# sta105/VIORB

Measured on AMD Instinct MI355X. Metric: frames/sec ORB extract+match+pose-opt, EuRoC 752x480, 1/2/4/8 GPUs, higher is better.
Workload: dtype u8

## Files before the change

include/viorb.h:

```cpp
#ifndef VIORB_H
#define VIORB_H

#include <stddef.h>
#include <stdint.h>

#ifdef __cplusplus
extern "C" {
#endif

#define VIORB_OK                 0
#define VIORB_ERR_INVALID_ARG   -1
#define VIORB_ERR_NO_DEVICE     -2
#define VIORB_ERR_HIP           -3
#define VIORB_ERR_CAPACITY      -4
#define VIORB_ERR_UNSUPPORTED   -5

int viorb_abi_version(void);
const char* viorb_last_error(void);
int viorb_device_count(void);


typedef struct viorb_keypoint {
    float x, y;
    float size;
    float angle;
    float response;
    int32_t octave;
    int32_t class_id;
} viorb_keypoint;

typedef struct viorb_extractor_params {
    int32_t nfeatures;
    float   scale_factor;
    int32_t nlevels;
    int32_t ini_th_fast;
    int32_t min_th_fast;
} viorb_extractor_params;

typedef struct viorb_extractor viorb_extractor;

int viorb_extractor_create(const viorb_extractor_params* params, int max_batch, int device,
                           viorb_extractor** out);
int viorb_extractor_destroy(viorb_extractor* h);

int viorb_extractor_tables(const viorb_extractor* h, float* scale, float* inv_scale, float* sigma2,
                           float* inv_sigma2, int32_t* features_per_level);

int viorb_extractor_max_keypoints(const viorb_extractor* h, int* cap);
int viorb_extractor_max_keypoints_for(const viorb_extractor* h, int width, int height, int* cap);
int viorb_extractor_fast_launch_images(int batch);

int viorb_extract(viorb_extractor* h, const uint8_t* img, int width, int height, int stride,
                  viorb_keypoint* kps, uint8_t* desc, int cap, int* n);

int viorb_extract_batch_device(viorb_extractor* h, const uint8_t* d_images, int batch, int width,
                               int height, int stride, size_t image_pitch_bytes, void* stream);

int viorb_extractor_results_device(const viorb_extractor* h, const viorb_keypoint** d_kps,
                                   const uint8_t** d_desc, const int32_t** d_count,
                                   const int32_t** d_status, int* cap);

int viorb_extractor_download(viorb_extractor* h, int b, viorb_keypoint* kps, uint8_t* desc, int cap,
                             int* n);

int viorb_extractor_level_device(const viorb_extractor* h, int b, int level, int blurred,
                                 const uint8_t** d_ptr, int* width, int* height, int* stride);
int viorb_extractor_level_download(viorb_extractor* h, int b, int level, int blurred, uint8_t* dst,
                                   int* width, int* height);

int viorb_stereo_match_device(const viorb_extractor* L, int left_index, const viorb_extractor* R, int right_index, int pairs,
                              float bf, float fx, float* d_uright, float* d_depth, int32_t* d_nmatched, void* stream);
int viorb_stereo_match(viorb_extractor* L, viorb_extractor* R, float bf, float fx, float* uright, float* depth, int cap,
                       int* nmatched);

int viorb_extractor_debug_level_points(viorb_extractor* h, int b, int level, int which, int32_t* xyr,
                                       int cap, int* n);

typedef struct viorb_frontend viorb_frontend;

typedef struct viorb_frontend_config {
    float   min_x, max_x, min_y, max_y;
    float   fx, fy, cx, cy;
    double  cam[16];
    double  gravity[3];
    float   scale_factors[16];
    float   inv_level_sigma2[16];
    int32_t nlevels;
    int32_t check_orientation;
    double  gyr_meas_cov, acc_meas_cov;
    double  acc_bias_rw2;
    float   dist_coef[5];
    int32_t reserved0;
} viorb_frontend_config;

int viorb_frontend_create(const viorb_frontend_config* cfg, int max_batch, int cap, int device, viorb_frontend** out);
int viorb_frontend_search_capacity(void);
int viorb_frontend_destroy(viorb_frontend* h);

int viorb_frontend_undistort_device(viorb_frontend* h, const viorb_keypoint* kps, const int32_t* count, int batch,
                                    viorb_keypoint* kps_un, void* stream);
int viorb_undistort_points(const float* xy, int n, const float* intr4, const float* dist5, float* xy_out);
int viorb_image_bounds(int width, int height, const float* intr4, const float* dist5, float* bounds4);

int viorb_frontend_grid_device(viorb_frontend* h, const viorb_keypoint* kps, const int32_t* count, int batch,
                               int32_t* cell_start, int32_t* cell_idx, void* stream);

int viorb_frontend_imu_predict_device(viorb_frontend* h, const double* imu, int n_imu, const double* t_last,
                                      const double* t_cur, const double* last_ns, int batch, double* preint,
                                      double* cur_ns, float* pose12, void* stream);

int viorb_frontend_search_projection_device(viorb_frontend* h, const viorb_keypoint* cur_kps, const uint8_t* cur_desc,
                                            const int32_t* cur_count, const int32_t* cell_start, const int32_t* cell_idx,
                                            const float* pose12, const viorb_keypoint* last_kps, const int32_t* last_count,
                                            const uint8_t* last_flags, const float* last_Pw, const uint8_t* last_desc,
                                            float th, int batch, int32_t* cur_match, int32_t* nmatches, int32_t* status,
                                            void* stream);
int viorb_frontend_search_projection_retry_device(viorb_frontend* h, const viorb_keypoint* cur_kps, const uint8_t* cur_desc,
                                            const int32_t* cur_count, const int32_t* cell_start, const int32_t* cell_idx,
                                            const float* pose12, const viorb_keypoint* last_kps, const int32_t* last_count,
                                            const uint8_t* last_flags, const float* last_Pw, const uint8_t* last_desc,
                                            float th, int retry_below, int batch, int32_t* cur_match, int32_t* nmatches, int32_t* status,
                                            void* stream);

int viorb_frontend_search_projection_stereo_device(viorb_frontend* h, const viorb_keypoint* cur_kps, const uint8_t* cur_desc,
                                                   const int32_t* cur_count, const float* cur_uright, const int32_t* cell_start,
                                                   const int32_t* cell_idx, const float* pose12, const float* last_pose12,
                                                   const viorb_keypoint* last_kps, const int32_t* last_count, const uint8_t* last_flags,
                                                   const float* last_Pw, const uint8_t* last_desc, float th, float bf, float mb,
                                                   int retry_below, int batch, int32_t* cur_match, int32_t* nmatches, int32_t* status,
                                                   void* stream);

int viorb_frontend_search_local_points_device(viorb_frontend* h, const viorb_keypoint* cur_kps, const uint8_t* cur_desc,
                                              const int32_t* cur_count, const int32_t* cell_start, const int32_t* cell_idx,
                                              const float* pose12, const float* pts_f, const uint8_t* pts_flags,
                                              const uint8_t* pts_desc, const int32_t* pts_count, int pcap, float th,
                                              float nnratio, const uint8_t* cur_owner_obs, int batch, int32_t* match,
                                              int32_t* nmatches, float* frustum, int32_t* status, void* stream);

int viorb_frontend_search_local_points_stereo_device(viorb_frontend* h, const viorb_keypoint* cur_kps, const uint8_t* cur_desc,
                                                     const int32_t* cur_count, const float* cur_uright, float bf, const int32_t* cell_start,
                                                     const int32_t* cell_idx, const float* pose12, const float* pts_f, const uint8_t* pts_flags,
                                                     const uint8_t* pts_desc, const int32_t* pts_count, int pcap, float th, float nnratio,
                                                     const uint8_t* cur_owner_obs, int batch, int32_t* match, int32_t* nmatches, float* frustum,
                                                     float* frustum_xr, int32_t* status, void* stream);

int viorb_frontend_build_observations_device(viorb_frontend* h, const viorb_keypoint* kps, const int32_t* count,
                                             const int32_t* match, const float* match_Pw, int batch, double* obs,
                                             int32_t* obs_index, int32_t* n_obs, void* stream);

int viorb_frontend_pose_opt_device(viorb_frontend* h, int variant, int compute_marg, const double* cur_ns,
                                   const double* last_ns, const double* prior_ns, const double* marg_cov_inv,
                                   const double* preint, const double* obs_cur, const int32_t* n_cur,
                                   const double* obs_last, const int32_t* n_last, int batch, double* out_ns,
                                   double* out_last_ns, uint8_t* outlier_cur, uint8_t* outlier_last, double* marg_out,
                                   double* info, void* stream);

int viorb_frontend_set_pose_shape(int problems_per_workgroup, int wavefronts_per_problem);

int viorb_frontend_pose_opt_se3_device(viorb_frontend* h, const float* pose12, const double* obs7, const int32_t* n_obs,
                                       double bf, int batch, float* out_pose12, uint8_t* outlier, double* info, void* stream);

int viorb_frontend_discard_outliers_device(viorb_frontend* h, int32_t* match, const int32_t* obs_index, const uint8_t* outlier,
                                           const int32_t* n_obs, const uint8_t* pt_flags, int batch, uint8_t* owner_obs,
                                           int32_t* n_map, void* stream);
int viorb_frontend_pose_from_navstate_device(viorb_frontend* h, const double* ns, int batch, float* pose12, void* stream);
int viorb_frontend_build_observations2_device(viorb_frontend* h, const viorb_keypoint* kps, const int32_t* count,
                                              const int32_t* match_a, const float* Pw_a, const int32_t* match_b,
                                              const float* pts_b, int stride_b, int batch, double* obs, int32_t* obs_index,
                                              int32_t* n_obs, void* stream);

int viorb_synth_local_points_device(viorb_frontend* h, const viorb_keypoint* kps, const int32_t* count, const double* pose12,
                                    const float* Pw, int batch, float* pts_f, void* stream);

int viorb_frontend_roll_device(viorb_frontend* h, const viorb_keypoint* cur_kps, const uint8_t* cur_desc, const int32_t* cur_count,
                               viorb_keypoint* last_kps, uint8_t* last_desc, int32_t* last_count, const float* last_pts_f,
                               const uint8_t* last_flags, float* loc_pts_f, uint8_t* loc_desc, uint8_t* loc_flags,
                               int local_frames, int shift_local, const double* ns_src, double* last_ns, double* prior_ns,
                               const double* t_src, double* t_last, const double* marg_src, double* marg_dst, int batch,
                               void* stream);

int viorb_synth_plane_points_device(viorb_frontend* h, const viorb_keypoint* kps, const int32_t* count,
                                    const double* pose12, double z0, int batch, float* Pw, uint8_t* flags,
                                    int32_t* self_index , void* stream);

int viorb_frontend_pose_opt_select_device(viorb_frontend* h, const uint8_t* variant, const uint8_t* skip, int compute_marg,
                                          const double* cur_ns, const double* last_ns, const double* prior_ns, const double* marg_cov_inv,
                                          const double* preint, const double* obs_cur, const int32_t* n_cur, const double* obs_last,
                                          const int32_t* n_last, int batch, double* out_ns, double* out_last_ns, uint8_t* outlier_cur,
                                          uint8_t* outlier_last, double* marg_out, double* info, void* stream);
int viorb_frontend_self_index_device(viorb_frontend* h, const uint8_t* flags, const int32_t* count, int batch, int32_t* self_index,
                                     void* stream);

#define VIORB_TRACK_OK           0
#define VIORB_TRACK_FEW_MATCHES  1
#define VIORB_TRACK_REVERT_1     2
#define VIORB_TRACK_REVERT_2     3
#define VIORB_TRACK_RELOC_FEW    4

typedef struct viorb_tracker viorb_tracker;
typedef struct viorb_tracker_config {
    viorb_extractor_params extractor;
    viorb_frontend_config  frontend;
    int32_t width, height, batch, device;
    float   th_projection;
    int32_t track_local_map;
    int32_t local_frames;
    int32_t compute_marg;
    int32_t max_steps_ahead;
    double  synth_plane_z0;
} viorb_tracker_config;
typedef struct viorb_tracker_inputs {
    const uint8_t* d_images; int32_t image_stride; size_t image_pitch_bytes;
    const double*  d_imu; int32_t n_imu;
    const double*  d_t_cur;
    const uint8_t* d_map_updated;
    const uint8_t* d_recent_reloc;
    const double*  d_t_next_last;
    const double*  d_reset_ns;
    const double*  d_reset_marg;
    const double*  d_synth_pose12;
    const uint8_t* h_images;
} viorb_tracker_inputs;
typedef struct viorb_tracker_results {
    int32_t cap;
    const int32_t *state, *status, *nmatches, *n_map, *n_loc, *inliers, *n_obs, *n_obs2, *cur_match, *loc_match, *last_count;
    const double *info, *info2, *pred_ns, *ns_stage1, *ns_stage2, *final_ns, *final_marg, *last_ns;
    const uint8_t *outlier_cur, *outlier_cur2, *last_flags;
    const float *last_Pw, *last_pts_f;
    const viorb_extractor* extractor;
} viorb_tracker_results;
int viorb_tracker_create(const viorb_tracker_config* cfg, viorb_tracker** out);
int viorb_tracker_destroy(viorb_tracker* h);
int viorb_tracker_capacity(const viorb_tracker* h, int* cap);
int viorb_tracker_bootstrap(viorb_tracker* h, const uint8_t* d_images, int stride, size_t image_pitch_bytes, const double* d_ns0,
                            const double* d_t0, const double* d_marg_cov_inv, const double* d_synth_pose12, void* caller_stream);
int viorb_tracker_set_last_points_device(viorb_tracker* h, const float* d_Pw, const uint8_t* d_flags, const float* d_pts_f, void* caller_stream);
int viorb_tracker_step(viorb_tracker* h, const viorb_tracker_inputs* in, void* caller_stream);
int viorb_tracker_sync(viorb_tracker* h);
int viorb_tracker_results_device(const viorb_tracker* h, viorb_tracker_results* out);
int viorb_tracker_host_stats(viorb_tracker* h, double* enqueue_s, double* throttle_s, long long* steps, int reset);
int viorb_memcpy_dtoh(void* dst_host, const void* src_device, size_t bytes);
int viorb_memcpy_htod(void* dst_device, const void* src_host, size_t bytes);

int viorb_memcpy_dtod_async(void* dst, const void* src, size_t bytes, void* stream);

int viorb_profile_enable(int on);
int viorb_profile_reset(void);
int viorb_profile_select(const char* kernel_name);
int viorb_profile_read(char* names_buf, int names_cap, double* total_ms, int* calls, int cap, int* n);
int viorb_profile_timeline(double* start_ms, double* end_ms, int* slot, int cap, int* n);

int viorb_descriptor_distance(const uint8_t* a, const uint8_t* b);
int viorb_search_by_projection_frame(const viorb_keypoint* cur_kps, const uint8_t* cur_desc, int ncur, const float bounds4[4],
                                     const float pose12[12], const float intr4[4], const float* scale_factors, int nlevels,
                                     const viorb_keypoint* last_kps, int nlast, const uint8_t* last_flags, const float* last_Pw,
                                     const uint8_t* last_desc, float th, int check_orientation, int32_t* cur_match, int* nmatches);
int viorb_search_by_projection_points(const viorb_keypoint* cur_kps, const uint8_t* cur_desc, int ncur, const float bounds4[4],
                                      const float pose12[12], const float intr4[4], const float* scale_factors, int nlevels,
                                      const float* pts_f, const uint8_t* pts_flags, const uint8_t* pts_desc, int npts, float th,
                                      float nnratio, const uint8_t* cur_owner_obs, int32_t* match, int* nmatches, float* frustum5);
int viorb_search_by_projection_points_stereo(const viorb_keypoint* cur_kps, const uint8_t* cur_desc, const float* cur_uright, float bf, int ncur,
                                             const float bounds4[4], const float pose12[12], const float intr4[4], const float* scale_factors, int nlevels,
                                             const float* pts_f, const uint8_t* pts_flags, const uint8_t* pts_desc, int npts, float th, float nnratio,
                                             const uint8_t* cur_owner_obs, int32_t* match, int* nmatches, float* frustum5, float* proj_xr);
int viorb_search_by_projection_frame_stereo(const viorb_keypoint* cur_kps, const uint8_t* cur_desc, const float* cur_uright, int ncur,
                                            const float bounds4[4], const float pose12[12], const float last_pose12[12], const float intr4[4],
                                            float bf, float mb, const float* scale_factors, int nlevels, const viorb_keypoint* last_kps, int nlast,
                                            const uint8_t* last_flags, const float* last_Pw, const uint8_t* last_desc, float th,
                                            int check_orientation, int32_t* cur_match, int* nmatches);
int viorb_preintegrate(const double* imu, int n_imu, const double bg[3], const double ba[3], double t_last,
                       double t_cur, double* preint142);
int viorb_pose_opt_vi(int variant, int compute_marg, const double cur_ns[22], const double last_ns[22],
                      const double prior_ns[22], const double* marg_cov_inv144, const double preint[142],
                      const double gw[3], const double cam[16], const double* obs_cur, int n_cur, const double* obs_last,
                      int n_last, double out_ns[22], double out_last_ns[22], uint8_t* outlier_cur, uint8_t* outlier_last,
                      double* marg_out144, double info[4]);

int viorb_pose_opt_se3(const float pose12[12], const float intr5[5], const double* obs7, int n, float out_pose12[12],
                       uint8_t* outlier, double info[4]);

int viorb_local_ba_set_device(int device);
int viorb_local_ba_navstate(const double* kfs, int nk, int n_local, int prev_kf, const double* preint,
                            const double* points, int np, const int32_t* edge_idx, const double* edge_obs, int ne,
                            const double gw[3], const double cam[16], const volatile int* stop, double* kfs_out,
                            double* points_out, uint8_t* erase, double info[6]);

typedef struct viorb_lba_window {
    const double* kfs; int32_t nk, n_local, prev_kf; const double* preint; const double* points; int32_t np;
    const int32_t* edge_idx; const double* edge_obs; int32_t ne; const double* gw; const double* cam; const volatile int* stop;
    double* kfs_out; double* points_out; uint8_t* erase; double* info ; int32_t status;
} viorb_lba_window;
int viorb_local_ba_navstate_batch(viorb_lba_window* windows, int n_windows, int max_in_flight);

int viorb_local_ba_se3(const double* kfs, int nk, int n_local, const double* points, int np, const int32_t* edge_idx,
                       const double* edge_obs, int ne, const double intr5[5], const volatile int* stop, double* kfs_out,
                       double* points_out, uint8_t* erase, double info[6]);

typedef struct viorb_lba_se3_window {
    const double* kfs; int32_t nk, n_local; const double* points; int32_t np; const int32_t* edge_idx; const double* edge_obs; int32_t ne;
    const double* intr5; const volatile int* stop; double* kfs_out; double* points_out; uint8_t* erase; double* info ; int32_t status;
} viorb_lba_se3_window;
int viorb_local_ba_se3_batch(viorb_lba_se3_window* windows, int n_windows, int max_in_flight);

typedef struct viorb_vocabulary viorb_vocabulary;
int viorb_vocabulary_create(int n_nodes, int L, const int32_t* child_start, const int32_t* child_ids, const uint8_t* desc,
                            const int32_t* word_id, const double* weight, viorb_vocabulary** out);
int viorb_vocabulary_destroy(viorb_vocabulary* v);
typedef struct viorb_vocabulary_flat {
    int32_t n_nodes, k, L, n_words;
    int32_t *child_start, *child_ids, *word_id; uint8_t* desc; double* weight;
} viorb_vocabulary_flat;
int viorb_vocabulary_read_file(const char* path, int binary, viorb_vocabulary_flat* out);
void viorb_vocabulary_flat_free(viorb_vocabulary_flat* f);
int viorb_vocabulary_load_text(const char* path, viorb_vocabulary** out);
int viorb_vocabulary_load_binary(const char* path, viorb_vocabulary** out);
int viorb_vocabulary_save_text(const char* path, int n_nodes, int k, int L, const int32_t* child_start, const int32_t* child_ids,
                               const uint8_t* desc, const double* weight);
int viorb_vocabulary_save_binary(const char* path, int n_nodes, int k, int L, const int32_t* child_start, const int32_t* child_ids,
                                 const uint8_t* desc, const double* weight);

int viorb_bow_transform_device(const viorb_vocabulary* v, const uint8_t* desc, const int32_t* count, int cap, int batch,
                               int levelsup, int32_t* word, double* weight, int32_t* node, void* stream);
int viorb_bow_transform(const viorb_vocabulary* v, const uint8_t* desc, int n, int levelsup, int32_t* word,
                        double* weight, int32_t* node);

int viorb_search_by_bow_device(const viorb_keypoint* kf_kps, const uint8_t* kf_desc, const int32_t* kf_node,
                               const uint8_t* kf_has_point, const int32_t* kf_count, const viorb_keypoint* f_kps,
                               const uint8_t* f_desc, const int32_t* f_node, const int32_t* f_count, int cap, int batch,
                               float nnratio, int check_orientation, int32_t* match, int32_t* nmatches, void* stream);
int viorb_search_by_bow(const viorb_keypoint* kf_kps, const uint8_t* kf_desc, const int32_t* kf_node,
                        const uint8_t* kf_has_point, int nkf, const viorb_keypoint* f_kps, const uint8_t* f_desc,
                        const int32_t* f_node, int nf, float nnratio, int check_orientation, int32_t* match,
                        int* nmatches);

int viorb_match_bruteforce_device(const uint8_t* q_desc, const int32_t* nq, int qcap, const uint8_t* c_desc, const int32_t* nc, int ccap,
                                  int batch, int32_t* best, int32_t* second, int32_t* idx, void* stream);
int viorb_match_bruteforce(const uint8_t* q, int nq, const uint8_t* c, int nc, int32_t* best, int32_t* second, int32_t* idx);

int viorb_search_for_triangulation_device(const viorb_keypoint* k1, const uint8_t* d1, const uint8_t* has_point1,
                                          const float* uright1, const int32_t* node1, const int32_t* n1,
                                          const viorb_keypoint* k2, const uint8_t* d2, const uint8_t* has_point2,
                                          const float* uright2, const int32_t* node2, const int32_t* n2, const float* F12,
                                          const float* Cw1, const float* pose12_2, const float intr4[4],
                                          const float* scale_factors2, const float* level_sigma2_2, int nlevels, int only_stereo,
                                          int check_orientation, int cap, int batch, int32_t* match12, int32_t* nmatches,
                                          void* stream);
int viorb_search_for_triangulation(const viorb_keypoint* k1, const uint8_t* d1, const uint8_t* has_point1, const float* uright1,
                                   const int32_t* node1, int n1, const viorb_keypoint* k2, const uint8_t* d2,
                                   const uint8_t* has_point2, const float* uright2, const int32_t* node2, int n2,
                                   const float F12[9], const float Cw1[3], const float pose12_2[12], const float intr4[4],
                                   const float* scale_factors2, const float* level_sigma2_2, int nlevels, int only_stereo,
                                   int check_orientation, int32_t* match12, int* nmatches);

int viorb_frontend_fuse_device(viorb_frontend* h, const viorb_keypoint* kps, const uint8_t* desc, const float* uright,
                               const int32_t* count, const int32_t* cell_start, const int32_t* cell_idx, const float* pose12,
                               const float* pts_f, const uint8_t* pts_valid, const uint8_t* pts_desc, const int32_t* pts_count,
                               int pcap, float th, float bf, int batch, int32_t* best_idx, int32_t* nfused, void* stream);
int viorb_fuse(const viorb_keypoint* kps, const uint8_t* desc, const float* uright, int n, const float bounds4[4],
               const float pose12[12], const float intr5[5], const float* scale_factors, const float* inv_level_sigma2, int nlevels,
               const float* pts_f, const uint8_t* pts_valid, const uint8_t* pts_desc, int npts, float th, int32_t* best_idx,
               int* nfused);

typedef struct viorb_mapping_camera {
    float   fx, fy, cx, cy;
    float   mb, mbf;
    float   scale_factor;
    int32_t nlevels;
    float   scale_factors[16];
    float   level_sigma2[16];
} viorb_mapping_camera;

#define VIORB_TRI_ACCEPT     0
#define VIORB_TRI_NO_POINT   1
#define VIORB_TRI_BEHIND_1   2
#define VIORB_TRI_BEHIND_2   3
#define VIORB_TRI_REPROJ_1   4
#define VIORB_TRI_REPROJ_2   5
#define VIORB_TRI_SCALE      6
#define VIORB_TRI_NO_PAIR  255
// ... 62 lines not shown
```

viorb_amd/capi.py:

```python
import ctypes as C
import os
import numpy as np

_HERE = os.path.dirname(os.path.abspath(__file__))
SO_PATH = os.environ.get("VIORB_LIBRARY") or os.path.join(_HERE, "libviorb_hip.so")

KP_DTYPE = np.dtype([("x", "f4"), ("y", "f4"), ("size", "f4"), ("angle", "f4"),
                     ("response", "f4"), ("octave", "i4"), ("class_id", "i4")])

VIORB_OK, ERR_INVALID_ARG, ERR_NO_DEVICE, ERR_HIP, ERR_CAPACITY, ERR_UNSUPPORTED = 0, -1, -2, -3, -4, -5


class ViorbError(RuntimeError):
    def __init__(self, code, msg):
        super().__init__("viorb error %d: %s" % (code, msg))
        self.code = code


class FrontendConfig(C.Structure):
    _fields_ = [("min_x", C.c_float), ("max_x", C.c_float), ("min_y", C.c_float), ("max_y", C.c_float),
                ("fx", C.c_float), ("fy", C.c_float), ("cx", C.c_float), ("cy", C.c_float),
                ("cam", C.c_double * 16), ("gravity", C.c_double * 3),
                ("scale_factors", C.c_float * 16), ("inv_level_sigma2", C.c_float * 16),
                ("nlevels", C.c_int32), ("check_orientation", C.c_int32),
                ("gyr_meas_cov", C.c_double), ("acc_meas_cov", C.c_double), ("acc_bias_rw2", C.c_double),
                ("dist_coef", C.c_float * 5), ("reserved0", C.c_int32)]


class LbaWindow(C.Structure):
    _fields_ = [("kfs", C.c_void_p), ("nk", C.c_int32), ("n_local", C.c_int32), ("prev_kf", C.c_int32), ("preint", C.c_void_p),
                ("points", C.c_void_p), ("np", C.c_int32), ("edge_idx", C.c_void_p), ("edge_obs", C.c_void_p), ("ne", C.c_int32),
                ("gw", C.c_void_p), ("cam", C.c_void_p), ("stop", C.c_void_p), ("kfs_out", C.c_void_p), ("points_out", C.c_void_p),
                ("erase", C.c_void_p), ("info", C.c_void_p), ("status", C.c_int32)]


class LbaSe3Window(C.Structure):
    _fields_ = [("kfs", C.c_void_p), ("nk", C.c_int32), ("n_local", C.c_int32), ("points", C.c_void_p), ("np", C.c_int32),
                ("edge_idx", C.c_void_p), ("edge_obs", C.c_void_p), ("ne", C.c_int32), ("intr5", C.c_void_p), ("stop", C.c_void_p),
                ("kfs_out", C.c_void_p), ("points_out", C.c_void_p), ("erase", C.c_void_p), ("info", C.c_void_p), ("status", C.c_int32)]


class ExtractorParams(C.Structure):
    _fields_ = [("nfeatures", C.c_int32), ("scale_factor", C.c_float), ("nlevels", C.c_int32),
                ("ini_th_fast", C.c_int32), ("min_th_fast", C.c_int32)]


class VocabularyFlat(C.Structure):
    _fields_ = [("n_nodes", C.c_int32), ("k", C.c_int32), ("L", C.c_int32), ("n_words", C.c_int32), ("child_start", C.c_void_p),
                ("child_ids", C.c_void_p), ("word_id", C.c_void_p), ("desc", C.c_void_p), ("weight", C.c_void_p)]


class MappingCamera(C.Structure):
    _fields_ = [("fx", C.c_float), ("fy", C.c_float), ("cx", C.c_float), ("cy", C.c_float), ("mb", C.c_float), ("mbf", C.c_float),
                ("scale_factor", C.c_float), ("nlevels", C.c_int32), ("scale_factors", C.c_float * 16), ("level_sigma2", C.c_float * 16)]


class TrackerConfig(C.Structure):
    _fields_ = [("extractor", ExtractorParams), ("frontend", FrontendConfig), ("width", C.c_int32), ("height", C.c_int32), ("batch", C.c_int32),
                ("device", C.c_int32), ("th_projection", C.c_float), ("track_local_map", C.c_int32), ("local_frames", C.c_int32),
                ("compute_marg", C.c_int32), ("max_steps_ahead", C.c_int32), ("synth_plane_z0", C.c_double)]


class TrackerInputs(C.Structure):
    _fields_ = [("d_images", C.c_void_p), ("image_stride", C.c_int32), ("image_pitch_bytes", C.c_size_t), ("d_imu", C.c_void_p), ("n_imu", C.c_int32),
                ("d_t_cur", C.c_void_p), ("d_map_updated", C.c_void_p), ("d_recent_reloc", C.c_void_p), ("d_t_next_last", C.c_void_p),
                ("d_reset_ns", C.c_void_p), ("d_reset_marg", C.c_void_p), ("d_synth_pose12", C.c_void_p), ("h_images", C.c_void_p)]


class TrackerResults(C.Structure):
    _fields_ = [("cap", C.c_int32)] + [(n, C.c_void_p) for n in (
        "state", "status", "nmatches", "n_map", "n_loc", "inliers", "n_obs", "n_obs2", "cur_match", "loc_match", "last_count",
        "info", "info2", "pred_ns", "ns_stage1", "ns_stage2", "final_ns", "final_marg", "last_ns",
        "outlier_cur", "outlier_cur2", "last_flags", "last_Pw", "last_pts_f", "extractor")]


vp, i32, f32, sz = C.c_void_p, C.c_int, C.c_float, C.c_size_t
PP = C.POINTER
SIGNATURES = {
    "viorb_abi_version": (i32, []),
    "viorb_last_error": (C.c_char_p, []),
    "viorb_device_count": (i32, []),
    "viorb_extractor_create": (i32, [PP(ExtractorParams), i32, i32, PP(vp)]),
    "viorb_extractor_destroy": (i32, [vp]),
    "viorb_extractor_tables": (i32, [vp, vp, vp, vp, vp, vp]),
    "viorb_extractor_max_keypoints": (i32, [vp, PP(i32)]),
    "viorb_extractor_max_keypoints_for": (i32, [vp, i32, i32, PP(i32)]),
    "viorb_extractor_fast_launch_images": (i32, [i32]),
    "viorb_extract": (i32, [vp, vp, i32, i32, i32, vp, vp, i32, PP(i32)]),
    "viorb_extract_batch_device": (i32, [vp, vp, i32, i32, i32, i32, sz, vp]),
    "viorb_extractor_results_device": (i32, [vp, PP(vp), PP(vp), PP(vp), PP(vp), PP(i32)]),
    "viorb_extractor_download": (i32, [vp, i32, vp, vp, i32, PP(i32)]),
    "viorb_extractor_level_device": (i32, [vp, i32, i32, i32, PP(vp), PP(i32), PP(i32), PP(i32)]),
    "viorb_extractor_level_download": (i32, [vp, i32, i32, i32, vp, PP(i32), PP(i32)]),
    "viorb_stereo_match_device": (i32, [vp, i32, vp, i32, i32, f32, f32, vp, vp, vp, vp]),
    "viorb_stereo_match": (i32, [vp, vp, f32, f32, vp, vp, i32, PP(i32)]),
    "viorb_extractor_debug_level_points": (i32, [vp, i32, i32, i32, vp, i32, PP(i32)]),
    "viorb_frontend_create": (i32, [PP(FrontendConfig), i32, i32, i32, PP(vp)]),
    "viorb_frontend_search_capacity": (i32, []),
    "viorb_frontend_destroy": (i32, [vp]),
    "viorb_frontend_grid_device": (i32, [vp, vp, vp, i32, vp, vp, vp]),
    "viorb_frontend_undistort_device": (i32, [vp, vp, vp, i32, vp, vp]),
    "viorb_undistort_points": (i32, [vp, i32, vp, vp, vp]),
    "viorb_image_bounds": (i32, [i32, i32, vp, vp, vp]),
    "viorb_frontend_imu_predict_device": (i32, [vp, vp, i32, vp, vp, vp, i32, vp, vp, vp, vp]),
    "viorb_frontend_search_projection_device": (i32, [vp] * 12 + [f32, i32, vp, vp, vp, vp]),
    "viorb_frontend_search_projection_retry_device": (i32, [vp] * 12 + [f32, i32, i32, vp, vp, vp, vp]),
    "viorb_frontend_set_pose_shape": (i32, [i32, i32]),
    "viorb_frontend_search_local_points_device": (i32, [vp] * 11 + [i32, f32, f32, vp, i32, vp, vp, vp, vp, vp]),
    "viorb_frontend_search_local_points_stereo_device": (i32, [vp] * 5 + [f32] + [vp] * 7 + [i32, f32, f32, vp, i32, vp, vp, vp, vp, vp, vp]),
    "viorb_frontend_build_observations_device": (i32, [vp, vp, vp, vp, vp, i32, vp, vp, vp, vp]),
    "viorb_frontend_pose_opt_device": (i32, [vp, i32, i32] + [vp] * 9 + [i32] + [vp] * 7),
    "viorb_frontend_pose_opt_se3_device": (i32, [vp, vp, vp, vp, C.c_double, i32, vp, vp, vp, vp]),
    "viorb_pose_opt_se3": (i32, [vp, vp, vp, i32, vp, vp, vp]),
    "viorb_local_ba_navstate": (i32, [vp, i32, i32, i32, vp, vp, i32, vp, vp, i32] + [vp] * 7),
    "viorb_local_ba_navstate_batch": (i32, [vp, i32, i32]),
    "viorb_local_ba_set_device": (i32, [i32]),
    "viorb_local_ba_se3_batch": (i32, [vp, i32, i32]),
    "viorb_local_ba_se3": (i32, [vp, i32, i32, vp, i32, vp, vp, i32] + [vp] * 6),
    "viorb_vocabulary_create": (i32, [i32, i32, vp, vp, vp, vp, vp, PP(vp)]),
    "viorb_vocabulary_destroy": (i32, [vp]),
    "viorb_vocabulary_read_file": (i32, [C.c_char_p, i32, PP(VocabularyFlat)]),
    "viorb_vocabulary_flat_free": (None, [PP(VocabularyFlat)]),
    "viorb_vocabulary_load_text": (i32, [C.c_char_p, PP(vp)]),
    "viorb_vocabulary_load_binary": (i32, [C.c_char_p, PP(vp)]),
    "viorb_vocabulary_save_text": (i32, [C.c_char_p, i32, i32, i32, vp, vp, vp, vp]),
    "viorb_vocabulary_save_binary": (i32, [C.c_char_p, i32, i32, i32, vp, vp, vp, vp]),
    "viorb_bow_transform_device": (i32, [vp, vp, vp, i32, i32, i32, vp, vp, vp, vp]),
    "viorb_bow_transform": (i32, [vp, vp, i32, i32, vp, vp, vp]),
    "viorb_search_by_bow_device": (i32, [vp] * 9 + [i32, i32, f32, i32, vp, vp, vp]),
    "viorb_search_by_bow": (i32, [vp, vp, vp, vp, i32, vp, vp, vp, i32, f32, i32, vp, PP(i32)]),
    "viorb_match_bruteforce_device": (i32, [vp, vp, i32, vp, vp, i32, i32, vp, vp, vp, vp]),
    "viorb_match_bruteforce": (i32, [vp, i32, vp, i32, vp, vp, vp]),
    "viorb_frontend_discard_outliers_device": (i32, [vp, vp, vp, vp, vp, vp, i32, vp, vp, vp]),
    "viorb_frontend_pose_from_navstate_device": (i32, [vp, vp, i32, vp, vp]),
    "viorb_frontend_build_observations2_device": (i32, [vp, vp, vp, vp, vp, vp, vp, i32, i32, vp, vp, vp, vp]),
    "viorb_synth_local_points_device": (i32, [vp, vp, vp, vp, vp, i32, vp, vp]),
    "viorb_search_for_triangulation_device": (i32, [vp] * 18 + [i32, i32, i32, i32, i32, vp, vp, vp]),
    "viorb_search_for_triangulation": (i32, [vp] * 5 + [i32] + [vp] * 5 + [i32] + [vp] * 6 + [i32, i32, i32, vp, PP(i32)]),
    "viorb_frontend_fuse_device": (i32, [vp] * 12 + [i32, f32, f32, i32, vp, vp, vp]),
    "viorb_fuse": (i32, [vp, vp, vp, i32, vp, vp, vp, vp, vp, i32, vp, vp, vp, i32, f32, vp, PP(i32)]),
    "viorb_synth_plane_points_device": (i32, [vp, vp, vp, vp, C.c_double, i32, vp, vp, vp, vp]),
    "viorb_frontend_roll_device": (i32, [vp] * 12 + [i32, i32] + [vp] * 7 + [i32, vp]),
    "viorb_memcpy_dtod_async": (i32, [vp, vp, sz, vp]),
    "viorb_memcpy_dtoh": (i32, [vp, vp, sz]),
    "viorb_memcpy_htod": (i32, [vp, vp, sz]),
    "viorb_frontend_pose_opt_select_device": (i32, [vp, vp, vp, i32] + [vp] * 9 + [i32] + [vp] * 7),
    "viorb_frontend_self_index_device": (i32, [vp, vp, vp, i32, vp, vp]),
    "viorb_tracker_create": (i32, [PP(TrackerConfig), PP(vp)]),
    "viorb_tracker_destroy": (i32, [vp]),
    "viorb_tracker_capacity": (i32, [vp, PP(i32)]),
    "viorb_tracker_bootstrap": (i32, [vp, vp, i32, sz, vp, vp, vp, vp, vp]),
    "viorb_tracker_set_last_points_device": (i32, [vp, vp, vp, vp, vp]),
    "viorb_tracker_step": (i32, [vp, PP(TrackerInputs), vp]),
    "viorb_tracker_sync": (i32, [vp]),
    "viorb_tracker_results_device": (i32, [vp, PP(TrackerResults)]),
    "viorb_tracker_host_stats": (i32, [vp, PP(C.c_double), PP(C.c_double), PP(C.c_longlong), i32]),
    "viorb_profile_enable": (i32, [i32]),
    "viorb_profile_reset": (i32, []),
    "viorb_profile_select": (i32, [C.c_char_p]),
    "viorb_profile_read": (i32, [C.c_char_p, i32, vp, vp, i32, PP(i32)]),
    "viorb_profile_timeline": (i32, [vp, vp, vp, i32, vp]),
    "viorb_descriptor_distance": (i32, [vp, vp]),
    "viorb_search_by_projection_frame": (i32, [vp, vp, i32, vp, vp, vp, vp, i32, vp, i32, vp, vp, vp, f32, i32, vp, PP(i32)]),
    "viorb_search_by_projection_frame_stereo": (i32, [vp, vp, vp, i32, vp, vp, vp, vp, f32, f32, vp, i32, vp, i32, vp, vp, vp, f32, i32, vp, PP(i32)]),
    "viorb_frontend_search_projection_stereo_device": (i32, [vp] * 14 + [f32, f32, f32, i32, i32, vp, vp, vp, vp]),
    "viorb_search_by_projection_points": (i32, [vp, vp, i32, vp, vp, vp, vp, i32, vp, vp, vp, i32, f32, f32, vp, vp, PP(i32), vp]),
    "viorb_search_by_projection_points_stereo": (i32, [vp, vp, vp, f32, i32, vp, vp, vp, vp, i32, vp, vp, vp, i32, f32, f32, vp, vp, PP(i32), vp, vp]),
    "viorb_preintegrate": (i32, [vp, i32, vp, vp, C.c_double, C.c_double, vp]),
    "viorb_pose_opt_vi": (i32, [i32, i32] + [vp] * 8 + [i32, vp, i32] + [vp] * 6),
    "viorb_debug_pvr_edge": (None, [vp] * 7),
    "viorb_debug_proj_edge": (None, [vp] * 5),
    "viorb_debug_prior_edge": (None, [vp] * 5),
    "viorb_debug_update_ns": (None, [vp] * 6),
    "viorb_debug_preint_step": (None, [vp, vp, vp, C.c_double]),
    "viorb_debug_octree_host": (i32, [vp, i32, i32, i32, i32, vp, i32, PP(i32)]),
    "viorb_debug_fast_atan2": (f32, [f32, f32]),
    "viorb_debug_sincos": (None, [f32, PP(f32), PP(f32)]),
    "viorb_triangulate_pairs_device": (i32, [vp] * 15 + [i32, i32] + [vp] * 4),
    "viorb_triangulate_pairs": (i32, [vp] * 5 + [i32] + [vp] * 6 + [i32] + [vp] * 6),
    "viorb_map_points_update_device": (i32, [vp] * 5 + [i32, vp, vp, i32, vp, vp, C.c_int64] + [vp] * 5),
    "viorb_map_points_update": (i32, [vp] * 5 + [i32, vp, vp, i32, vp, vp, C.c_int64] + [vp] * 4),
    "viorb_create_new_map_points_workspace_bytes": (sz, [i32, i32]),
    "viorb_create_new_map_points_device": (i32, [vp, i32] + [vp] * 24 + [i32] * 6 + [vp] * 6 + [sz, vp]),
    "viorb_create_new_map_points": (i32, [vp, i32] + [vp] * 7 + [i32] + [vp] * 15 + [i32] * 3 + [vp] * 3 + [PP(i32)]),
    "viorb_debug_triangulate_pair": (i32, [vp] * 6 + [i32, vp, i32, vp]),
    "viorb_debug_map_point_update": (i32, [vp] * 5 + [i32, vp, vp, i32, vp, vp, C.c_int64] + [vp] * 4),
}

_lib = None


def lib():
    global _lib
    if _lib is None:
        if not os.path.exists(SO_PATH):
            raise ImportError("%s not built: run `python -c 'import __graft_entry__ as g; g.build()'` "
                              "(hipcc, gfx950). viorb_amd has no CPU fallback." % SO_PATH)
        try:
            import torch
        except Exception:
            pass
        L = C.CDLL(SO_PATH)
        for name, (res, args) in SIGNATURES.items():
            fn = getattr(L, name)
            fn.restype = res
            fn.argtypes = args
        _lib = L
    return _lib


def check(rc):
    if rc != VIORB_OK:
        raise ViorbError(rc, lib().viorb_last_error().decode())
    return rc


def ptr(a):
    if a is None:
        return None
    if isinstance(a, np.ndarray):
        return a.ctypes.data_as(C.c_void_p)
    return C.c_void_p(a.data_ptr())
```

viorb_amd/csrc/orb_extractor.hip:

```cpp
#include <hip/hip_runtime.h>
#include <stdarg.h>
#include <stdlib.h>
#include <math.h>
#include <vector>
#include <string>
#include <mutex>
#include <algorithm>
#include "viorb_common.h"
#include "orb_math.h"
#include "octree_arrays.h"

namespace viorb {

static thread_local char g_err[512] = "";
char* last_error_buf() { return g_err; }
void set_error(const char* fmt, ...) {
    va_list ap; va_start(ap, fmt); vsnprintf(g_err, sizeof(g_err), fmt, ap); va_end(ap);
}

namespace {
struct ProfRec { hipEvent_t a, b; int slot; };
struct Profiler {
    bool enabled = false;
    std::string only;
// ... 543 lines not shown
                    rq = surv[base + lane];
                    const int r = rq >> 8, q = rq & 0xff;
                    const int s = fast_strength(tile + __mul24(r + 3, tile_pitch) + xoff + q + 3, tile_pitch);
                    if (s >= th) { is_c = true; sc[__mul24(r + 1, sp) + q + 1] = (uint8_t)s; }
                }
                const unsigned long long m = __ballot(is_c);
                if (is_c) corn[ncorn + __popcll(m & lt)] = rq;
                ncorn += __popcll(m);
            }
            __syncthreads();
            {
                for (int base = 0; base < ncorn; base += 64) {
                    bool keep = false;
                    int r = 0, q = 0, s = 0;
                    if (base + lane < ncorn) {
                        const uint16_t rq = corn[base + lane];
                        r = rq >> 8; q = rq & 0xff;
                        const uint8_t* z = sc + __mul24(r + 1, sp) + q + 1;
                        s = z[0];
                        int nb[8];
                        nb[0] = z[-sp - 1]; nb[1] = z[-sp]; nb[2] = z[-sp + 1]; nb[3] = z[-1]; nb[4] = z[1]; nb[5] = z[sp - 1]; nb[6] = z[sp]; nb[7] = z[sp + 1];
                        int mx = 0;
    #pragma unroll
                        for (int k = 0; k < 8; k++) mx = max(mx, nb[k]);
                        keep = s > mx;
                    }
                    const unsigned long long m = __ballot(keep);
                    if (keep) {
                        const int pos = total + __popcll(m & lt);
                        if (pos < slot_cap)
                            my_slots[pos] = (uint32_t)(q + 3 + c.shx) | ((uint32_t)(r + 3 + c.shy) << 12) | ((uint32_t)s << 24);
                    }
                    total += __popcll(m);
                }
            }
            __syncthreads();
        }
    }
    if (lane == 0) cell_cnt[(size_t)img_b * ncells_total + cell] = min(total, slot_cap);
    __syncthreads();
    c = cn;
    }
}

#define F3_TPD 13
#define F3_TP (4 * F3_TPD)
#define F3_TRIPS 11
#define F3_SP 44
#define F3_SROWS 40
__device__ __forceinline__ uint32_t pk_mul16(uint32_t a, uint32_t b) {
    return __builtin_bit_cast(uint32_t, __builtin_bit_cast(short2v, a) * __builtin_bit_cast(short2v, b));
}
__device__ __forceinline__ int fast_strength_pol(const uint8_t* p, uint32_t sgn) {
    const uint32_t v = p[0], vv = v | (v << 16);
    uint32_t P[8];
    P[0] = pk_sub16(vv, (uint32_t)p[3 * F3_TP] | ((uint32_t)p[-3 * F3_TP] << 16));
    P[1] = pk_sub16(vv, (uint32_t)p[3 * F3_TP + 1] | ((uint32_t)p[-3 * F3_TP - 1] << 16));
    P[2] = pk_sub16(vv, (uint32_t)p[2 * F3_TP + 2] | ((uint32_t)p[-2 * F3_TP - 2] << 16));
    P[3] = pk_sub16(vv, (uint32_t)p[F3_TP + 3] | ((uint32_t)p[-F3_TP - 3] << 16));
    P[4] = pk_sub16(vv, (uint32_t)p[3] | ((uint32_t)p[-3] << 16));
    P[5] = pk_sub16(vv, (uint32_t)p[-F3_TP + 3] | ((uint32_t)p[F3_TP - 3] << 16));
    P[6] = pk_sub16(vv, (uint32_t)p[-2 * F3_TP + 2] | ((uint32_t)p[2 * F3_TP - 2] << 16));
    P[7] = pk_sub16(vv, (uint32_t)p[-3 * F3_TP + 1] | ((uint32_t)p[3 * F3_TP - 1] << 16));
    uint32_t S[8], lo2[8], lo4[8];
#pragma unroll
    for (int k = 0; k < 8; k++) { P[k] = pk_mul16(P[k], sgn); S[k] = swap16(P[k]); }
#pragma unroll
    for (int k = 0; k < 8; k++) lo2[k] = pk_min16(P[k], k < 7 ? P[k + 1] : S[0]);
#pragma unroll
    for (int k = 0; k < 8; k++) lo4[k] = pk_min16(lo2[k], k < 6 ? lo2[k + 2] : swap16(lo2[k - 6]));
    uint32_t A = 0x80008000u;
#pragma unroll
    for (int k = 0; k < 8; k++) A = pk_max16(A, pk_min16(pk_min16(lo4[k], k < 4 ? lo4[k + 4] : swap16(lo4[k - 4])), S[k]));
    return max((int)(short)(A & 0xffff), (int)(short)(A >> 16)) - 1;
}
__host__ __device__ __forceinline__ uint32_t spread8(uint32_t x) {
    x = (x | (x << 4)) & 0x0f0fu; x = (x | (x << 2)) & 0x3333u; x = (x | (x << 1)) & 0x5555u;
    return x;
}
#define F3_SURV_CAP (63 + 64 * 16 + 1)
#define F3_CORN_CAP 512
#ifdef VIORB_FAST_TIMING
#define FT_DECL unsigned long long ft_acc[8] = {0, 0, 0, 0, 0, 0, 0, 0}, ft_t0 = __builtin_amdgcn_s_memtime(); int ft_cells = 0, ft_surv = 0, ft_corn = 0, ft_att2 = 0
#define FT_LAP(k) do { const unsigned long long ft_now = __builtin_amdgcn_s_memtime(); ft_acc[k] += ft_now - ft_t0; ft_t0 = ft_now; } while (0)
#else
#define FT_DECL
#define FT_LAP(k)
#endif
__global__ __launch_bounds__(64) void k_fast_cells3(const uint8_t* __restrict__ planes, size_t frame_bytes,
                                                    const CellDesc* __restrict__ cells, int ini_th, int min_th,
                                                    uint32_t* __restrict__ slots, int slot_cap,
                                                    int* __restrict__ cell_cnt, int ncells_total, int tile_bytes, int score_bytes, XcdPlace PL) {
    extern __shared__ uint32_t s_mem[];
    int img_b, item;
    if (!xcd_place(PL, img_b, item)) return;
    uint8_t* tile = reinterpret_cast<uint8_t*>(s_mem);
    uint8_t* sc = tile + tile_bytes;
    uint16_t* surv = reinterpret_cast<uint16_t*>(sc + score_bytes);
    uint16_t* corn = surv + F3_SURV_CAP;
    const int lane = threadIdx.x;
    const int cell0 = item * FAST_CELLS_PER_WAVE;
    const int ncell = min((int)FAST_CELLS_PER_WAVE, ncells_total - cell0);
    const uint8_t* img = planes + (size_t)img_b * frame_bytes;
    const int lrow = lane >> 4, lq = lane & 15;
    const bool fetch_lane = lq < F3_TPD;
    uint32_t v[F3_TRIPS];
    auto request_tile = [&](const CellDesc& cd) {
        const uint8_t* src = img + cd.src_off;
        const int ntrip = (cd.ch + 3) >> 2;
        const uint32_t voff = (uint32_t)(__mul24(lrow, cd.stride) + 4 * lq);
        const uint32_t voff_last = (uint32_t)(__mul24(min(4 * (ntrip - 1) + lrow, cd.ch - 1) - 4 * (ntrip - 1), cd.stride) + 4 * lq);
        if (fetch_lane) {
#pragma unroll
            for (int k = 0; k < F3_TRIPS; k++)
                if (k < ntrip) {
                    const uint8_t* base = src + (size_t)(4 * k) * (size_t)cd.stride;
                    v[k] = *reinterpret_cast<const uint32_t*>(base + (k == ntrip - 1 ? voff_last : voff));
                }
        }
    };
    CellDesc c = cells[cell0];
    request_tile(c);
    const int lds_lane = __mul24(lrow, F3_TP) + 4 * lq;
    const unsigned long long lt = (1ull << lane) - 1ull;
    FT_DECL;
    for (int kk = 0; kk < ncell; kk++) {
    FT_LAP(7);
    const int cell = cell0 + kk;
    const int x0a = c.x0 & ~3, xoff = c.x0 - x0a;
    {
        const int ntrip = (c.ch + 3) >> 2;
        if (fetch_lane) {
#pragma unroll
            for (int k = 0; k < F3_TRIPS; k++)
                if (k < ntrip) *reinterpret_cast<uint32_t*>(tile + lds_lane + 4 * k * F3_TP) = v[k];
        }
    }
    const bool has_next = kk + 1 < ncell;
    const CellDesc cn = cells[has_next ? cell + 1 : cell];
    const int dw = c.cw - 6, dh = c.ch - 6;
    {
        const int nq = ((dh + 2) * F3_SP + 15) >> 4;
        for (int i = lane; i < nq; i += 64) reinterpret_cast<uint4*>(sc)[i] = make_uint4(0, 0, 0, 0);
    }
    __syncthreads();
    if (has_next) request_tile(cn);
    FT_LAP(0);
    uint32_t* my_slots = slots + ((size_t)img_b * ncells_total + cell) * slot_cap;
    int total = 0;
    if (dw > 0 && dh > 0) {
        const uint8_t* tile_c = tile + 3 * F3_TP + xoff + 3;
        for (int attempt = 0; attempt < 2 && total == 0; attempt++) {
            const int th = attempt ? min_th : ini_th;
            int pending = 0, ncorn = 0;
            {
                const int g0 = (xoff + 3) >> 2;
                const int G = ((xoff + 3 + dw - 1) >> 2) - g0 + 1;
                const int G2 = (G + 1) >> 1;
                const int rcpG = (int)c_rcp16[min(G2, 63)];
                const int step_r = (64 * rcpG) >> 16, step_g = 64 - step_r * G2;
                int r = __mul24(lane, rcpG) >> 16, gp = lane - __mul24(r, G2);
                const int ntrip = (dh * G2 + 63) >> 6;
                const uint32_t M = 0x00ff00ffu, Hb = 0x80008000u;
                const uint32_t K1 = Hb - (uint32_t)(th + 1) * 0x00010001u;
                const uint32_t K2 = Hb - (uint32_t)(th + 1) * 0x00010001u;
                const int sh0 = (xoff + 3) - 4 * g0;
                const int hi_last = min((G & 1) ? 4 : 8, dw - (8 * (G2 - 1) - sh0));
                const uint32_t m8_first = (0xffu << sh0) & 0xffu, m8_last = (1u << hi_last) - 1u;
                const uint32_t mask_first = spread8(m8_first) * 3u, mask_last = spread8(m8_last) * 3u;
                FT_LAP(1);
#ifdef VIORB_FAST_TIMING
                if (attempt) ft_att2++;
#endif
                for (int trip = 0; trip < ntrip; trip++) {
                    const int rc = min(r, dh - 1);
                    const int ga = 2 * gp, gb = min(ga + 1, G - 1);
                    const uint32_t* rowU = reinterpret_cast<const uint32_t*>(tile + __mul24(rc, F3_TP)) + g0;
                    const uint32_t Lf = rowU[3 * F3_TPD + ga - 1], C0 = rowU[3 * F3_TPD + ga], C1 = rowU[3 * F3_TPD + gb], Rt = rowU[3 * F3_TPD + gb + 1];
                    const uint32_t U0 = rowU[ga], U1 = rowU[gb], D0 = rowU[6 * F3_TPD + ga], D1 = rowU[6 * F3_TPD + gb];
                    const uint32_t Cl1 = gb == ga ? Lf : C0;
                    const uint32_t W0 = __builtin_amdgcn_alignbyte(C0, Lf, 1), E0 = __builtin_amdgcn_alignbyte(gb == ga ? Rt : C1, C0, 3);
                    const uint32_t W1 = __builtin_amdgcn_alignbyte(C1, Cl1, 1), E1 = __builtin_amdgcn_alignbyte(Rt, C1, 3);
                    const int q0 = 4 * (g0 + ga) - (xoff + 3);
                    uint32_t X = 0;
    #pragma unroll
                    for (int dwi = 0; dwi < 2; dwi++) {
                        const uint32_t C = dwi ? C1 : C0, U = dwi ? U1 : U0, D = dwi ? D1 : D0, W = dwi ? W1 : W0, E = dwi ? E1 : E0;
    #pragma unroll
                        for (int half = 0; half < 2; half++) {
                            auto field = [&](uint32_t x) { return half ? __builtin_amdgcn_perm(x, x, 0x0c030c01u) : (x & M); };
                            const uint32_t v2 = field(C);
                            const uint32_t p0 = field(D), p4 = field(E), p8 = field(U), p12 = field(W);
                            const uint32_t A = pk_max16(pk_min16(p0, p8), pk_min16(p4, p12));
                            const uint32_t B = pk_min16(pk_max16(p0, p8), pk_max16(p4, p12));
                            const uint32_t dk = (K1 + v2) - A, br = (K2 - v2) + B;
                            X |= (dk >> (15 - 8 * dwi - 2 * half)) & (0x00010001u << (8 * dwi + 2 * half));
                            X |= (br >> (14 - 8 * dwi - 2 * half)) & (0x00010001u << (8 * dwi + 2 * half + 1));
                        }
                    }
                    uint32_t bits = (X | (X >> 12)) & 0xffffu;
                    bits &= (gp == 0 ? mask_first : 0xffffu) & (gp == G2 - 1 ? mask_last : 0xffffu);
                    if (r >= dh) bits = 0;
                    const int cnt = __popc(bits), incl = wave_inclusive_scan(cnt);
                    const int trip_total = __builtin_amdgcn_readlane(incl, 63);
                    if (trip_total) {
                        int pos = pending + incl - cnt;
                        const uint32_t rq0 = ((uint32_t)r << 7) + (uint32_t)(2 * q0);
                        uint32_t bb = bits;
                        while (bb) {
                            const int k = __builtin_ctz(bb);
                            surv[pos++] = (uint16_t)(rq0 + k);
                            bb &= bb - 1;
                        }
                        pending += trip_total;
                    }
                    r += step_r; gp += step_g;
                    if (gp >= G2) { gp -= G2; r++; }
                    const int need = trip + 1 < ntrip ? 64 : 1;
                    FT_LAP(2);
#ifdef VIORB_FAST_TIMING
                    ft_surv += trip_total;
#endif
                    if (pending >= need) {
                        __syncthreads();
                        int done = 0;
                        while (pending - done >= need) {
                            const int n = min(64, pending - done);
                            bool is_c = false;
                            uint32_t e = 0;
                            if (lane < n) {
                                e = surv[done + lane];
                                const int er = e >> 7, eq = (e >> 1) & 63;
                                const int s = fast_strength_pol(tile_c + __mul24(er, F3_TP) + eq, (e & 1) ? 0xffffffffu : 0x00010001u);
                                if (s >= th) { is_c = true; sc[__mul24(er + 1, F3_SP) + eq + 1] = (uint8_t)s; }
                            }
                            const unsigned long long m = __ballot(is_c);
                            if (is_c) { const int cp = ncorn + __popcll(m & lt); if (cp < F3_CORN_CAP) corn[cp] = (uint16_t)(e & ~1u); }
                            ncorn += __popcll(m);
                            done += n;
                        }
                        const int left = pending - done;
                        if (left > 0) {
                            const uint16_t t = lane < left ? surv[done + lane] : (uint16_t)0;
                            __syncthreads();
                            if (lane < left) surv[lane] = t;
                        }
                        pending = left;
                        __syncthreads();
                        FT_LAP(3);
                    }
                }
            }
            __syncthreads();
            FT_LAP(4);
#ifdef VIORB_FAST_TIMING
            ft_corn += ncorn;
#endif
            const bool dense = ncorn > F3_CORN_CAP;
            const int n3 = dense ? dh * dw : ncorn;
            for (int base = 0; base < n3; base += 64) {
                bool keep = false;
                int r = 0, q = 0, s = 0;
                if (base + lane < n3) {
                    if (dense) { r = (base + lane) / dw; q = (base + lane) - r * dw; }
                    else { const uint32_t e = corn[base + lane]; r = e >> 7; q = (e >> 1) & 63; }
                    const uint8_t* z = sc + __mul24(r + 1, F3_SP) + q + 1;
                    s = z[0];
                    int nb[8];
                    nb[0] = z[-F3_SP - 1]; nb[1] = z[-F3_SP]; nb[2] = z[-F3_SP + 1]; nb[3] = z[-1]; nb[4] = z[1]; nb[5] = z[F3_SP - 1]; nb[6] = z[F3_SP]; nb[7] = z[F3_SP + 1];
                    int mx = 0;
    #pragma unroll
                    for (int k = 0; k < 8; k++) mx = max(mx, nb[k]);
                    keep = s > mx;
                }
                const unsigned long long m = __ballot(keep);
                if (keep) {
                    const int pos = total + __popcll(m & lt);
                    if (pos < slot_cap)
                        my_slots[pos] = (uint32_t)(q + 3 + c.shx) | ((uint32_t)(r + 3 + c.shy) << 12) | ((uint32_t)s << 24);
                }
                total += __popcll(m);
            }
            __syncthreads();
            FT_LAP(5);
        }
    }
    if (lane == 0) cell_cnt[(size_t)img_b * ncells_total + cell] = min(total, slot_cap);
    __syncthreads();
    c = cn;
    FT_LAP(6);
#ifdef VIORB_FAST_TIMING
    ft_cells++;
#endif
    }
#ifdef VIORB_FAST_TIMING
    if (lane == 0 && (blockIdx.x % 997) == 3)
        printf("fast3 block=%d cells=%d att2=%d surv=%d corn=%d | tile+clear=%llu setup=%llu pass1=%llu pass2=%llu tail=%llu nms=%llu end=%llu loop=%llu\n", (int)blockIdx.x, ft_cells, ft_att2, ft_surv, ft_corn,
               ft_acc[0], ft_acc[1], ft_acc[2], ft_acc[3], ft_acc[4], ft_acc[5], ft_acc[6], ft_acc[7]);
#endif
}

#define WAVE_SYNC() __syncthreads()
#define OCT_NCAP_SMALL 4096
struct OctNodeBig { int16_t x0, x1, y0, y1; uint32_t begin, count; uint16_t flags, pad; };
template <bool BIG> struct OctT;
template <> struct OctT<false> { typedef uint16_t Perm; typedef OctNode Node; typedef uint32_t SortKey; enum { KEY_SHIFT = 16 }; };
template <> struct OctT<true> { typedef uint32_t Perm; typedef OctNodeBig Node; typedef unsigned long long SortKey; enum { KEY_SHIFT = 32 }; };
template <bool BIG> struct OctLdsT {
    uint32_t* keys; typename OctT<BIG>::Perm* perm0; typename OctT<BIG>::Perm* perm1; typename OctT<BIG>::Node* nd; typename OctT<BIG>::SortKey* sortb;
};

__device__ __forceinline__ unsigned long long lanemask_lt(int lane) { return (1ull << lane) - 1ull; }

#define OCT_LANE_LIMIT 64
struct OctExpandResult { int off, nexp; };

template <bool BIG> __device__ __forceinline__ void oct_write_children(const OctLdsT<BIG>& S, const typename OctT<BIG>::Node& p, int i, int slot, int mx, int my, int sb,
                                                   const int tc[4], const int sc4[4]) {
#pragma unroll
    for (int c = 0; c < 4; c++) {
        typename OctT<BIG>::Node o;
        o.x0 = (c & 1) ? (int16_t)mx : p.x0; o.x1 = (c & 1) ? p.x1 : (int16_t)mx;
        o.y0 = (c & 2) ? (int16_t)my : p.y0; o.y1 = (c & 2) ? p.y1 : (int16_t)my;
        o.begin = (decltype(o.begin))sc4[c]; o.count = (decltype(o.count))tc[c];
        o.flags = tc[c] > 0 ? (uint16_t)((sb ^ 1) | (tc[c] == 1 ? OCT_NOMORE : 0)) : (uint16_t)OCT_DEAD; o.pad = 0;
        S.nd[slot + c] = o;
    }
    S.nd[i].flags = p.flags | OCT_DEAD;
}

#define OCT_CODE(key) (((int)((key) & 0xfff) < mx ? 0 : 1) | ((int)(((key) >> 12) & 0xfff) < my ? 0 : 2))
template <bool BIG> __device__ __forceinline__ OctExpandResult oct_expand_wave(const OctLdsT<BIG>& S, int i, int slot, int lane) {
    typedef typename OctT<BIG>::Perm Perm;
    const typename OctT<BIG>::Node p = S.nd[i];
    const int mx = p.x0 + ((p.x1 - p.x0 + 1) >> 1), my = p.y0 + ((p.y1 - p.y0 + 1) >> 1);
    const int sb = p.flags & OCT_BUF;
    const Perm* src = (sb ? S.perm1 : S.perm0) + (int)p.begin;
    Perm* dst = sb ? S.perm0 : S.perm1;
    const int cnt = (int)p.count, beg = (int)p.begin;
    const unsigned long long lt = lanemask_lt(lane);
    int t[4] = {0, 0, 0, 0};
    Perm id[4]; int c[4];
    auto load4 = [&](int o) {
#pragma unroll
        for (int u = 0; u < 4; u++) id[u] = src[min(o + 64 * u + lane, cnt - 1)];
#pragma unroll
        for (int u = 0; u < 4; u++) { const uint32_t key = S.keys[id[u]]; c[u] = o + 64 * u + lane < cnt ? OCT_CODE(key) : -1; }
    };
    int w0, w1, w2, w3;
    auto scatter4 = [&]() {
#pragma unroll
        for (int u = 0; u < 4; u++) {
            const unsigned long long m0 = __ballot(c[u] == 0), m1 = __ballot(c[u] == 1), m2 = __ballot(c[u] == 2), m3 = __ballot(c[u] == 3);
            const unsigned long long mm = c[u] == 0 ? m0 : (c[u] == 1 ? m1 : (c[u] == 2 ? m2 : m3));
            int at = w3;
            at = c[u] == 2 ? w2 : at; at = c[u] == 1 ? w1 : at; at = c[u] == 0 ? w0 : at;
            if (c[u] >= 0) dst[at + __popcll(mm & lt)] = id[u];
            w0 += __popcll(m0); w1 += __popcll(m1); w2 += __popcll(m2); w3 += __popcll(m3);
        }
    };
    auto count4 = [&]() {
#pragma unroll
        for (int u = 0; u < 4; u++) {
            t[0] += __popcll(__ballot(c[u] == 0)); t[1] += __popcll(__ballot(c[u] == 1));
            t[2] += __popcll(__ballot(c[u] == 2)); t[3] += __popcll(__ballot(c[u] == 3));
        }
    };
    if (cnt <= 256) {
        load4(0); count4();
        w0 = beg; w1 = w0 + t[0]; w2 = w1 + t[1]; w3 = w2 + t[2];
        scatter4();
    } else {
        for (int o = 0; o < cnt; o += 256) { load4(o); count4(); }
        w0 = beg; w1 = w0 + t[0]; w2 = w1 + t[1]; w3 = w2 + t[2];
        for (int o = 0; o < cnt; o += 256) { load4(o); scatter4(); }
    }
    const int sc4[4] = {beg, beg + t[0], beg + t[0] + t[1], beg + t[0] + t[1] + t[2]};
    if (lane == 0) oct_write_children(S, p, i, slot, mx, my, sb, t, sc4);
    OctExpandResult r; r.off = (t[0] > 0) + (t[1] > 0) + (t[2] > 0) + (t[3] > 0); r.nexp = (t[0] > 1) + (t[1] > 1) + (t[2] > 1) + (t[3] > 1);
    return r;
}

template <bool BIG> __device__ __forceinline__ void oct_lane_count(const OctLdsT<BIG>& S, const typename OctT<BIG>::Node& p, int mx, int my, unsigned long long& lo, unsigned long long& hi, int tc[4]) {
    const typename OctT<BIG>::Perm* src = ((p.flags & OCT_BUF) ? S.perm1 : S.perm0) + (int)p.begin;
    lo = 0; hi = 0; tc[0] = tc[1] = tc[2] = tc[3] = 0;
    const int cnt = (int)p.count;
    for (int k = 0; k < cnt; k += 4) {
        typename OctT<BIG>::Perm id[4]; uint32_t key[4];
#pragma unroll
        for (int u = 0; u < 4; u++) id[u] = src[min(k + u, cnt - 1)];
#pragma unroll
        for (int u = 0; u < 4; u++) key[u] = S.keys[id[u]];
#pragma unroll
        for (int u = 0; u < 4; u++) {
            const bool in = k + u < cnt;
            const int cx = (int)(key[u] & 0xfff) < mx ? 0 : 1, cy = (int)((key[u] >> 12) & 0xfff) < my ? 0 : 1;
            lo |= (unsigned long long)(in ? cx : 0) << ((k + u) & 63); hi |= (unsigned long long)(in ? cy : 0) << ((k + u) & 63);
            const int c = in ? (cx | (cy << 1)) : -1;
            tc[0] += c == 0; tc[1] += c == 1; tc[2] += c == 2; tc[3] += c == 3;
        }
    }
}
template <bool BIG> __device__ __forceinline__ void oct_lane_scatter(const OctLdsT<BIG>& S, const typename OctT<BIG>::Node& p, int i, int slot, int mx, int my, unsigned long long lo,
                                                 unsigned long long hi, const int tc[4]) {
    const int sb = p.flags & OCT_BUF;
    const typename OctT<BIG>::Perm* src = (sb ? S.perm1 : S.perm0) + (int)p.begin;
    typename OctT<BIG>::Perm* dst = sb ? S.perm0 : S.perm1;
    const int sc4[4] = {(int)p.begin, (int)p.begin + tc[0], (int)p.begin + tc[0] + tc[1], (int)p.begin + tc[0] + tc[1] + tc[2]};
    int w0 = sc4[0], w1 = sc4[1], w2 = sc4[2], w3 = sc4[3];
    const int cnt = (int)p.count;
    for (int k = 0; k < cnt; k += 4) {
        typename OctT<BIG>::Perm id[4];
#pragma unroll
        for (int u = 0; u < 4; u++) id[u] = src[min(k + u, cnt - 1)];
#pragma unroll
        for (int u = 0; u < 4; u++) {
            if (k + u < cnt) {
                const int c = (int)((lo >> (k + u)) & 1) | ((int)((hi >> (k + u)) & 1) << 1);
                const int pos = c == 0 ? w0 : (c == 1 ? w1 : (c == 2 ? w2 : w3));
                dst[pos] = id[u];
                w0 += c == 0; w1 += c == 1; w2 += c == 2; w3 += c == 3;
            }
        }
    }
    oct_write_children(S, p, i, slot, mx, my, sb, tc, sc4);
}

template <bool BIG> __device__ __forceinline__ int oct_compact(const OctLdsT<BIG>& S, int nn, int upto, int lane, int& first_new) {
    int w = 0;
    first_new = -1;
    for (int base = 0; base < nn; base += 64) {
        const int i = base + lane;
        typedef typename OctT<BIG>::Node Node;
        enum { NW = sizeof(Node) / 4, FW = offsetof(Node, flags) / 4, FS = 8 * (offsetof(Node, flags) % 4) };
        uint32_t wd[NW];
        const uint32_t* from = reinterpret_cast<const uint32_t*>(S.nd + min(i, nn - 1));
#pragma unroll
        for (int k = 0; k < NW; k++) wd[k] = from[k];
        const bool alive = (i < nn) && !((wd[FW] >> FS) & OCT_DEAD);
        const unsigned long long m = __ballot(alive);
        if (upto >= base && upto < base + 64) first_new = w + __popcll(m & lanemask_lt(upto - base));
        WAVE_SYNC();
        if (alive) {
            uint32_t* to = reinterpret_cast<uint32_t*>(S.nd + w + __popcll(m & lanemask_lt(lane)));
#pragma unroll
            for (int k = 0; k < NW; k++) to[k] = wd[k];
        }
        w += __popcll(m);
        WAVE_SYNC();
    }
    if (first_new < 0) first_new = w;
    return w;
}

template <class K> __device__ __forceinline__ void oct_sort(K* a, int m, int lane) {
    for (int k = 2; k <= m; k <<= 1)
        for (int j = k >> 1; j > 0; j >>= 1) {
            for (int t = lane; t < (m >> 1); t += 64) {
                const int lo = ((t & ~(j - 1)) << 1) | (t & (j - 1));
                const int hi = lo | j;
                const bool up = (lo & k) == 0;
                const K x = a[lo], y = a[hi];
                if ((x > y) == up) { a[lo] = y; a[hi] = x; }
            }
            WAVE_SYNC();
        }
}

template <bool BIG>
__global__ __launch_bounds__(64) void k_octree(const LevelDev* __restrict__ lv, const uint32_t* __restrict__ slots,
                                               int slot_cap, const int* __restrict__ cell_cnt, int ncells_total,
                                               uint32_t* __restrict__ lvl_kp, int kp_pitch, int* __restrict__ lvl_cnt,
                                               int* __restrict__ lvl_ncand, int nlevels, int* __restrict__ status,
                                               int ncap, int nodecap, int sortcap, int n_above, int n_upto,
                                               int level0, int use_tier_cap, int defer_nodes,
                                               uint32_t* __restrict__ big_scratch, int* __restrict__ big_next, int big_slots, int* __restrict__ lvl_tot,
                                               uint8_t* __restrict__ node_scratch = nullptr, size_t node_bytes = 0) {
    extern __shared__ __attribute__((aligned(16))) uint32_t s_oct[];
    typedef typename OctT<BIG>::Perm Perm; typedef typename OctT<BIG>::Node Node; typedef typename OctT<BIG>::SortKey SortKey;
    OctLdsT<BIG> S;
    if (BIG) {
        S.sortb = reinterpret_cast<SortKey*>(s_oct);
        S.nd = reinterpret_cast<Node*>(S.sortb + sortcap);
        S.keys = nullptr; S.perm0 = S.perm1 = nullptr;
    } else {
        S.keys = s_oct;
        S.perm0 = reinterpret_cast<Perm*>(s_oct + ncap);
        S.perm1 = S.perm0 + ncap;
        S.nd = reinterpret_cast<Node*>(S.perm1 + ncap);
        S.sortb = reinterpret_cast<SortKey*>(S.nd + nodecap);
    }
    const int lane = threadIdx.x, level = blockIdx.y + level0, b = blockIdx.x;
    const LevelDev L = lv[level];
    const int N = L.quota;
    if (use_tier_cap && L.oct_tier_cap > 0) n_above = L.oct_tier_cap;
    const int* cc = cell_cnt + (size_t)b * ncells_total + L.cell_base;
    {
        int tot = 0;
        if (n_above < 0) {
            for (int c0 = 0; c0 < L.ncells; c0 += 512) {
                int part[8];
#pragma unroll
                for (int j = 0; j < 8; j++) { const int ci = c0 + 64 * j + lane; part[j] = cc[min(ci, L.ncells - 1)]; if (ci >= L.ncells) part[j] = 0; }
#pragma unroll
                for (int j = 0; j < 8; j++) tot += part[j];
            }
#pragma unroll
            for (int d = 32; d > 0; d >>= 1) tot += __shfl_xor(tot, d);
            if (lane == 0) lvl_tot[b * nlevels + level] = tot;
        } else tot = lvl_tot[b * nlevels + level];
        const bool deferred = (tot & 0x40000000) != 0;
        tot &= 0x3fffffff;
        if (!(deferred && !BIG && !defer_nodes) && (tot <= n_above || tot > n_upto)) return;
        if (BIG) {
            int slot = 0;
            if (lane == 0) slot = atomicAdd(big_next, 1);
            slot = __shfl(slot, 0);
            if (slot >= big_slots) { if (lane == 0) { lvl_cnt[b * nlevels + level] = 0; lvl_ncand[b * nlevels + level] = tot; status[b] = VIORB_ERR_CAPACITY; } return; }
            uint32_t* base = big_scratch + (size_t)slot * 3 * (size_t)ncap;
            S.keys = base; S.perm0 = reinterpret_cast<Perm*>(base + ncap); S.perm1 = reinterpret_cast<Perm*>(base + 2 * (size_t)ncap);
            if (node_scratch) {
                S.sortb = reinterpret_cast<SortKey*>(node_scratch + (size_t)slot * node_bytes);
                S.nd = reinterpret_cast<Node*>(S.sortb + sortcap);
            }
        }
    }
    int n = 0;
    bool overflow = false;
    {
        const uint32_t* sl = slots + ((size_t)b * ncells_total + L.cell_base) * slot_cap;
        for (int base = 0; base < L.ncells; base += 64) {
            const int ci = base + lane;
            const int cnt = ci < L.ncells ? cc[ci] : 0;
            const int incl = wave_inclusive_scan(cnt);
            const int start = n + incl - cnt;
            const uint32_t* mine = sl + (size_t)min(ci, L.ncells - 1) * slot_cap;
            for (int k0 = 0; __any(k0 < cnt); k0 += 8) {
                uint32_t v[8];
#pragma unroll
                for (int u = 0; u < 8; u++) v[u] = mine[min(k0 + u, slot_cap - 1)];
#pragma unroll
                for (int u = 0; u < 8; u++) {
                    const int pos = start + k0 + u;
                    if (k0 + u < cnt && pos < ncap) S.keys[pos] = v[u];
                }
            }
            n += __shfl(incl, 63);
        }
        if (n > ncap) { overflow = true; n = ncap; }
    }
    if (lane == 0) lvl_ncand[b * nlevels + level] = n;
    WAVE_SYNC();
    uint32_t* out = lvl_kp + (size_t)b * kp_pitch + L.kp_off;
    if (n == 0 || L.n_ini < 1 || N < 1) {
        if (lane == 0) { lvl_cnt[b * nlevels + level] = 0; if (overflow) status[b] = VIORB_ERR_CAPACITY; }
        return;
    }
    int nn = 0, live = 0;
    {
        int begin = 0;
        for (int r = 0; r < L.n_ini; r++) {
            int cnt = 0;
            for (int o = 0; o < n; o += 64) {
                const int idx = o + lane;
                bool mine = false;
                if (idx < n) mine = ((int)((float)(S.keys[idx] & 0xfff) / L.hx)) == r;
                const unsigned long long m = __ballot(mine);
                if (mine) S.perm0[begin + cnt + __popcll(m & lanemask_lt(lane))] = (Perm)idx;
                cnt += __popcll(m);
            }
            if (cnt > 0) {
                if (lane == 0) {
                    Node o;
                    o.x0 = (int16_t)(int)(L.hx * (float)r); o.x1 = (int16_t)(int)(L.hx * (float)(r + 1));
                    o.y0 = 0; o.y1 = (int16_t)L.oct_h;
                    o.begin = (decltype(o.begin))begin; o.count = (decltype(o.count))cnt;
                    o.flags = (uint16_t)(cnt == 1 ? OCT_NOMORE : 0); o.pad = 0;
                    S.nd[nn] = o;
                }
                nn++;
            }
            begin += cnt;
        }
        WAVE_SYNC();
        for (int i = lane; i < (nn >> 1); i += 64) {
            const Node a = S.nd[i], z = S.nd[nn - 1 - i];
            S.nd[i] = z; S.nd[nn - 1 - i] = a;
        }
        WAVE_SYNC();
        live = nn;
    }
    bool finish = false;
    int guard = 0;
    while (!finish && guard++ < 64) {
        const int prev = live, nn0 = nn;
        int ne = 0;
        for (int base = 0; base < nn0; base += 64) {
            const int i = nn0 - 1 - (base + lane);
            ne += __popcll(__ballot(i >= 0 && !(S.nd[max(i, 0)].flags & (OCT_NOMORE | OCT_DEAD))));
        }
        if (nn0 + 4 * ne > nodecap) { overflow = true; break; }
        int n_to_expand = 0, e_base = 0;
        for (int base = 0; base < nn0; base += 64) {
            const int i = nn0 - 1 - (base + lane);
            Node p; p.flags = OCT_DEAD; p.count = 0;
            if (i >= 0) p = S.nd[i];
            const bool ex = i >= 0 && !(p.flags & (OCT_NOMORE | OCT_DEAD));
            const unsigned long long m = __ballot(ex);
            const int e = e_base + __popcll(m & lanemask_lt(lane));
            const bool small = ex && p.count <= OCT_LANE_LIMIT;
            int off = 0, nexp = 0;
            if (small) {
                const int mx = p.x0 + ((p.x1 - p.x0 + 1) >> 1), my = p.y0 + ((p.y1 - p.y0 + 1) >> 1);
                unsigned long long lo, hi; int tc[4];
                oct_lane_count(S, p, mx, my, lo, hi, tc);
                oct_lane_scatter(S, p, i, nn0 + 4 * e, mx, my, lo, hi, tc);
                off = (tc[0] > 0) + (tc[1] > 0) + (tc[2] > 0) + (tc[3] > 0); nexp = (tc[0] > 1) + (tc[1] > 1) + (tc[2] > 1) + (tc[3] > 1);
            }
            unsigned long long mb = __ballot(ex && !small);
            int big_off = 0, big_nexp = 0;
            while (mb) {
                const int l = __ffsll((long long)mb) - 1;
                mb &= mb - 1;
                const OctExpandResult r = oct_expand_wave(S, nn0 - 1 - (base + l), nn0 + 4 * __shfl(e, l), lane);
                big_off += r.off - 1; big_nexp += r.nexp;
            }
            int d_live = small ? off - 1 : 0, d_exp = nexp;
#pragma unroll
            for (int d = 32; d > 0; d >>= 1) { d_live += __shfl_xor(d_live, d); d_exp += __shfl_xor(d_exp, d); }
            live += d_live + big_off; n_to_expand += d_exp + big_nexp;
            e_base += __popcll(m);
        }
        nn = nn0 + 4 * ne;
        WAVE_SYNC();
        int first_new;
        nn = oct_compact(S, nn, nn0, lane, first_new);
        if (live >= N || live == prev) {
            finish = true;
        } else if (live + n_to_expand * 3 > N) {
            int guard2 = 0;
            while (!finish && guard2++ < 4096) {
                const int prev2 = live;
                int m = 0;
                for (int base = first_new; base < nn; base += 64) {
                    const int i = base + lane;
                    bool want = false; SortKey key = 0;
                    if (i < nn) { const Node o = S.nd[i]; want = o.count > 1; key = ((SortKey)o.count << OctT<BIG>::KEY_SHIFT) | (SortKey)i; }
                    const unsigned long long bm = __ballot(want);
                    if (want) { const int pos = m + __popcll(bm & lanemask_lt(lane)); if (pos < sortcap) S.sortb[pos] = key; }
                    m += __popcll(bm);
                }
                if (m > sortcap) { overflow = true; m = sortcap; }
                int mp = 1; while (mp < m) mp <<= 1;
                for (int i = m + lane; i < mp; i += 64) S.sortb[i] = 0;
                WAVE_SYNC();
                oct_sort(S.sortb, mp, lane);
                const int nn1 = nn;
                int processed = 0;
                bool reached = false;
                for (int base = 0; base < m && !reached && !finish; base += 64) {
                    const int q = base + lane;
                    const bool valid = q < m;
                    const int i = valid ? (int)(S.sortb[mp - 1 - q] & 0xffff) : 0;
                    Node p; p.flags = OCT_DEAD; p.count = 0;
                    if (valid) p = S.nd[i];
                    if (__any(valid && p.count > OCT_LANE_LIMIT)) {
                        for (int l = 0; l < 64 && base + l < m; l++) {
                            if (nn1 + 4 * (processed + 1) > nodecap) { overflow = true; finish = true; break; }
                            const OctExpandResult r = oct_expand_wave(S, (int)(S.sortb[mp - 1 - (base + l)] & 0xffff), nn1 + 4 * processed, lane);
                            processed++; live += r.off - 1;
                            if (live >= N) { reached = true; break; }
                        }
                        continue;
                    }
                    const int mx = p.x0 + ((p.x1 - p.x0 + 1) >> 1), my = p.y0 + ((p.y1 - p.y0 + 1) >> 1);
                    unsigned long long lo = 0, hi = 0; int tc[4] = {0, 0, 0, 0};
                    if (valid) oct_lane_count(S, p, mx, my, lo, hi, tc);
                    const int inc = valid ? (tc[0] > 0) + (tc[1] > 0) + (tc[2] > 0) + (tc[3] > 0) - 1 : 0;
                    const int incl = wave_inclusive_scan(inc);
                    const unsigned long long mh = __ballot(valid && live + incl >= N);
                    const int nvalid = min(64, m - base);
                    int cut = mh ? __ffsll((long long)mh) - 1 : nvalid - 1;
                    const int fit = (nodecap - nn1) / 4 - processed;
                    if (fit < cut + 1) { overflow = true; finish = true; cut = fit - 1; }
                    if (valid && lane <= cut) oct_lane_scatter(S, p, i, nn1 + 4 * (processed + lane), mx, my, lo, hi, tc);
                    if (cut >= 0) { live += __shfl(incl, cut); processed += cut + 1; }
                    if (mh) reached = true;
                }
                nn = nn1 + 4 * processed;
                WAVE_SYNC();
                nn = oct_compact(S, nn, nn1, lane, first_new);
                if (live >= N || live == prev2) finish = true;
            }
        }
    }
    if (defer_nodes && overflow) {
        if (lane == 0) lvl_tot[b * nlevels + level] |= 0x40000000;
        return;
    }
    for (int base = 0; base < nn; base += 64) {
        const int i = base + lane;
        if (i < nn) {
            const Node o = S.nd[i];
            const Perm* pm = (o.flags & OCT_BUF) ? S.perm1 : S.perm0;
            uint32_t best = S.keys[pm[o.begin]];
            for (int k = 1; k < (int)o.count; k++) {
                const uint32_t key = S.keys[pm[o.begin + k]];
                if ((key >> 24) > (best >> 24)) best = key;
            }
            out[nn - 1 - i] = (best & 0xff000000u) | ((((best >> 12) & 0xfff) + MINB) << 12) | ((best & 0xfff) + MINB);
        }
    }
    if (lane == 0) {
        lvl_cnt[b * nlevels + level] = nn;
        if (overflow) status[b] = VIORB_ERR_CAPACITY;
    }
}

#define BS_LANES 32
#define BS_PF 6
__constant__ int c_gauss[7];
__global__ __launch_bounds__(64) void k_blur(const uint8_t* __restrict__ planes, uint8_t* __restrict__ blur,
                                             size_t frame_bytes, const LevelDev* __restrict__ lv,
                                             const int4* __restrict__ items, XcdPlace PL) {
    int b, item;
    if (!xcd_place(PL, b, item)) return;
    const int4 t = items[item];
    const LevelDev L = lv[t.x];
    const uint8_t* src = planes + (size_t)b * frame_bytes + L.plane_off;
    uint8_t* dst = blur + (size_t)b * frame_bytes + L.plane_off;
    const int lane = threadIdx.x, hl = lane & (BS_LANES - 1);
    const bool upper = lane >= BS_LANES;
    const int Rb = t.w, y0A = t.z, y0B = t.z + Rb;
    const int rows = upper ? min(Rb, L.h - y0B) : min(Rb, L.h - y0A);
    const int sdw = L.stride >> 2;
    const int d = t.y + hl;
    const int dlast = (L.w - 1) >> 2, m = (L.w - 1) & 3;
    const int dc = min(d, sdw - 1);
    const bool end_lane = hl == 0 || hl == BS_LANES - 1;
    const int dn = hl == 0 ? max(dc - 1, 0) : min(dc + 1, sdw - 1);
    const uint32_t selC = m == 0 ? 0x01020304u : m == 1 ? 0x03040504u : m == 2 ? 0x05060504u : 0x07060504u;
    const uint32_t selR = m == 0 ? 0x0c0c0c0cu : m == 1 ? 0x0c000102u : m == 2 ? 0x01020304u : 0x03040506u;
    const bool has_edge = t.y == 0 || t.y + BS_LANES > dlast - 1;
    const bool is_d0 = d == 0, is_dl = d == dlast, is_dl1 = d == dlast - 1;
    const uint32_t k0 = (uint32_t)c_gauss[0], k1 = (uint32_t)c_gauss[1], k2 = (uint32_t)c_gauss[2], k3 = (uint32_t)c_gauss[3];
    const uint32_t Ka = k0 | (k1 << 8) | (k2 << 16) | (k3 << 24), Kb = k2 | (k1 << 8) | (k0 << 16);
    const uint32_t K01 = k0 | (k1 << 16), K23 = k2 | (k3 << 16), K45 = k2 | (k1 << 16);
    const int nrow = Rb + 6;
    const uint8_t* pc = src + 4u * (uint32_t)dc;
    const uint8_t* pn = src + 4u * (uint32_t)(end_lane ? dn : dc);
    uint32_t cb[BS_PF], nb[BS_PF];
    auto request = [&](int i, uint32_t& c, uint32_t& n) {
        const int ii = min(i, nrow - 1);
        int ya = y0A + ii - 3, yb = y0B + ii - 3;
        ya = ya < 0 ? -ya : ya; ya = ya >= L.h ? 2 * L.h - 2 - ya : ya; ya = min(max(ya, 0), L.h - 1);
        yb = yb < 0 ? -yb : yb; yb = yb >= L.h ? 2 * L.h - 2 - yb : yb; yb = min(max(yb, 0), L.h - 1);
        const uint32_t offA = __builtin_amdgcn_readfirstlane(ya * L.stride), offB = __builtin_amdgcn_readfirstlane(yb * L.stride);
        const uint32_t off = upper ? offB : offA;
        c = *reinterpret_cast<const uint32_t*>(pc + off);
        n = *reinterpret_cast<const uint32_t*>(pn + off);
    };
#pragma unroll
    for (int u = 0; u < BS_PF; u++) request(u, cb[u], nb[u]);
    uint32_t P[6][4], hp[4] = {0, 0, 0, 0};
#pragma unroll
    for (int u = 0; u < 6; u++) { P[u][0] = P[u][1] = P[u][2] = P[u][3] = 0; }
    uint8_t* pd = dst + 4u * (uint32_t)min(d, sdw - 1);
    const bool col_ok = d < sdw;
    for (int i0 = 0; i0 < nrow; i0 += 6) {
#pragma unroll
        for (int u = 0; u < 6; u++) {
            const int i = i0 + u;
            uint32_t c = cb[u];
            uint32_t Lr = __builtin_amdgcn_update_dpp(c, c, 0x138, 0xf, 0xf, true);
            uint32_t Rr = __builtin_amdgcn_update_dpp(c, c, 0x130, 0xf, 0xf, true);
            Lr = hl == 0 ? nb[u] : Lr; Rr = hl == BS_LANES - 1 ? nb[u] : Rr;
            request(i + BS_PF, cb[u], nb[u]);
            if (has_edge) {
                const uint32_t Lf = __builtin_amdgcn_perm(Rr, c, 0x01020304u);
                const uint32_t Cf = __builtin_amdgcn_perm(c, Lr, selC), Rf = __builtin_amdgcn_perm(c, Lr, selR);
                const uint32_t Rf1 = __builtin_amdgcn_perm(Rr, c, selC);
                Lr = is_d0 ? Lf : Lr;
                Rr = is_dl ? Rf : (is_dl1 ? Rf1 : Rr);
                c = is_dl ? Cf : c;
            }
            uint32_t h[4];
            h[0] = __builtin_amdgcn_udot4(__builtin_amdgcn_alignbyte(c, Lr, 1), Ka, __builtin_amdgcn_udot4(__builtin_amdgcn_alignbyte(Rr, c, 1), Kb, 0u, false), false);
            h[1] = __builtin_amdgcn_udot4(__builtin_amdgcn_alignbyte(c, Lr, 2), Ka, __builtin_amdgcn_udot4(__builtin_amdgcn_alignbyte(Rr, c, 2), Kb, 0u, false), false);
            h[2] = __builtin_amdgcn_udot4(__builtin_amdgcn_alignbyte(c, Lr, 3), Ka, __builtin_amdgcn_udot4(__builtin_amdgcn_alignbyte(Rr, c, 3), Kb, 0u, false), false);
            h[3] = __builtin_amdgcn_udot4(c, Ka, __builtin_amdgcn_udot4(Rr, Kb, 0u, false), false);
            uint32_t a[4];
#pragma unroll
            for (int j = 0; j < 4; j++) {
                a[j] = dot2_u16(P[(u + 1) % 6][j], K01, 1u << 15);
                a[j] = dot2_u16(P[(u + 3) % 6][j], K23, a[j]);
                a[j] = dot2_u16(P[(u + 5) % 6][j], K45, a[j]);
                a[j] = __umul24(h[j], k0) + a[j];
                a[j] = min(a[j], 0x00ffffffu);
                P[u][j] = hp[j] | (h[j] << 16);
                hp[j] = h[j];
            }
            const int o = i - 6;
            const uint32_t yoA = __builtin_amdgcn_readfirstlane((y0A + o) * L.stride), yoB = __builtin_amdgcn_readfirstlane((y0B + o) * L.stride);
            if (o >= 0 && o < rows && col_ok) {
                const uint32_t lo = __builtin_amdgcn_perm(a[1], a[0], 0x0c0c0602u), hi = __builtin_amdgcn_perm(a[3], a[2], 0x0c0c0602u);
                *reinterpret_cast<uint32_t*>(pd + (upper ? yoB : yoA)) = lo | (hi << 16);
            }
        }
    }
}

__constant__ __attribute__((aligned(16))) uint32_t c_pattern[256];
__constant__ int c_umax[16];
__constant__ uint32_t c_orient_mask[256];
typedef uint32_t u32_unaligned __attribute__((aligned(1)));
#define DESC_WIN_HALF 18
#define DESC_WIN_ROWS 37
#define DESC_WIN_DW 10
#define DESC_WIN_TRIPS 6
__global__ __launch_bounds__(256) void k_orient_describe(const uint8_t* __restrict__ planes,
                                                         const uint8_t* __restrict__ blur, size_t frame_bytes,
                                                         const LevelDev* __restrict__ lv, int nlevels,
                                                         const uint32_t* __restrict__ lvl_kp, int kp_pitch,
                                                         const int* __restrict__ lvl_cnt,
                                                         viorb_keypoint* __restrict__ out_kp,
                                                         uint8_t* __restrict__ out_desc, int out_cap,
                                                         int* __restrict__ out_cnt, int* __restrict__ status, XcdPlace PL) {
    const int lane = threadIdx.x & 63;
    int b, item;
    if (!xcd_place(PL, b, item)) return;
    const int k = item * 4 + __builtin_amdgcn_readfirstlane(threadIdx.x >> 6);
    const int* cnt = lvl_cnt + b * nlevels;
    int level = -1, local = 0, total = 0;
    for (int l = 0; l < nlevels; l++) {
        const int c = cnt[l];
        if (level < 0 && k < total + c) { level = l; local = k - total; }
        total += c;
    }
    if (k == 0 && lane == 0) { out_cnt[b] = min(total, out_cap); if (total > out_cap) status[b] = VIORB_ERR_CAPACITY; }
    if (level < 0 || k >= out_cap) return;
    const LevelDev L = lv[level];
    const uint32_t key = lvl_kp[(size_t)b * kp_pitch + L.kp_off + local];
    const int cx = (int)(key & 0xfff), cy = (int)((key >> 12) & 0xfff), score = (int)(key >> 24);
    const uint8_t* img = planes + (size_t)b * frame_bytes + L.plane_off + (size_t)cy * L.stride + cx;
    __shared__ uint32_t s_win[4][DESC_WIN_ROWS * DESC_WIN_DW];
    uint32_t* win = s_win[threadIdx.x >> 6];
    const uint8_t* bim = blur + (size_t)b * frame_bytes + L.plane_off + (size_t)cy * L.stride + cx;
    uint32_t wv[DESC_WIN_TRIPS];
#pragma unroll
    for (int it = 0; it < DESC_WIN_TRIPS; it++) {
        const int i = min(lane + 64 * it, DESC_WIN_ROWS * DESC_WIN_DW - 1);
        const int wr = i / DESC_WIN_DW, wc = i - wr * DESC_WIN_DW;
        wv[it] = *reinterpret_cast<const u32_unaligned*>(bim + __mul24(wr - DESC_WIN_HALF, L.stride) - DESC_WIN_HALF + 4 * wc);
    }
    int m10 = 0, m01 = 0;
    {
        const int j = lane & 7, r8 = lane >> 3;
        const uint32_t wu = 0x03020100u + 0x04040404u * (uint32_t)j;
        const uint8_t* col = img - HALF_PATCH + 4 * j;
        uint32_t px[4]; int vv[4];
#pragma unroll
        for (int it = 0; it < 4; it++) {
            const int row = min(it * 8 + r8, PATCH - 1);
            vv[it] = row - HALF_PATCH;
            px[it] = *reinterpret_cast<const u32_unaligned*>(col + __mul24(vv[it], L.stride));
        }
#pragma unroll
        for (int it = 0; it < 4; it++) {
            const uint32_t q = px[it] & c_orient_mask[it * 64 + lane];
            const int s1 = (int)__builtin_amdgcn_udot4(q, 0x01010101u, 0u, false);
            const int su = (int)__builtin_amdgcn_udot4(q, wu, 0u, false);
            m10 += su - __mul24(HALF_PATCH, s1);
            m01 += __mul24(vv[it], s1);
        }
    }
    m10 = __builtin_amdgcn_readlane(wave_inclusive_scan(m10), 63); m01 = __builtin_amdgcn_readlane(wave_inclusive_scan(m01), 63);
    const float angle = fast_atan2_deg((float)m01, (float)m10);
    const float factor_pi = (float)(3.14159265358979323846 / 180.f);
    float sn, cs;
    sincos_f32(angle * factor_pi, &sn, &cs);
    const float a = cs, bb = sn;
#pragma unroll
    for (int it = 0; it < DESC_WIN_TRIPS; it++) {
        const int i = lane + 64 * it;
        if (i < DESC_WIN_ROWS * DESC_WIN_DW) win[i] = wv[it];
    }
    __builtin_amdgcn_fence(__ATOMIC_RELEASE, "wavefront"); __builtin_amdgcn_wave_barrier(); __builtin_amdgcn_fence(__ATOMIC_ACQUIRE, "wavefront");
    const uint8_t* w8 = reinterpret_cast<const uint8_t*>(win) + DESC_WIN_HALF * (DESC_WIN_DW * 4) + DESC_WIN_HALF;
    uint32_t nib = 0;
    const uint4 pq = reinterpret_cast<const uint4*>(c_pattern)[lane];
    const uint32_t pqa[4] = {pq.x, pq.y, pq.z, pq.w};
#pragma unroll
    for (int t = 0; t < 4; t++) {
        const uint32_t q = pqa[t];
        const float x0 = (float)(int8_t)(q & 0xff), y0 = (float)(int8_t)((q >> 8) & 0xff);
        const float x1 = (float)(int8_t)((q >> 16) & 0xff), y1 = (float)(int8_t)(q >> 24);
        const int r0 = round_half_even(x0 * bb + y0 * a), c0 = round_half_even(x0 * a - y0 * bb);
        const int r1 = round_half_even(x1 * bb + y1 * a), c1 = round_half_even(x1 * a - y1 * bb);
        const int t0 = w8[__mul24(r0, DESC_WIN_DW * 4) + c0], t1 = w8[__mul24(r1, DESC_WIN_DW * 4) + c1];
        nib |= (uint32_t)(t0 < t1) << t;
    }
    uint32_t byte = nib | (__shfl_down(nib, 1) << 4);
    uint32_t word = byte | (__shfl_down(byte, 2) << 8) | (__shfl_down(byte, 4) << 16) | (__shfl_down(byte, 6) << 24);
    const size_t o = (size_t)b * out_cap + k;
    if ((lane & 7) == 0) reinterpret_cast<uint32_t*>(out_desc + o * 32)[lane >> 3] = word;
    if (lane == 0) {
        viorb_keypoint kp;
        kp.x = level ? (float)cx * L.scale : (float)cx;
        kp.y = level ? (float)cy * L.scale : (float)cy;
        kp.size = L.kp_size; kp.angle = angle; kp.response = (float)score;
        kp.octave = level; kp.class_id = -1;
        out_kp[o] = kp;
    }
}

struct StereoArgs {
    const viorb_keypoint *kl, *kr; const uint8_t *dl, *dr; const int *nl, *nr;
    const uint8_t *planesL, *planesR; size_t frame_bytes; const LevelDev* lv;
    int cap, sort_n, nlevels; float bf, fx;
    float scale[16], inv_scale[16];
    float* uright; float* depth; int* nmatched;
    unsigned char* work; size_t work_bytes;
};
__host__ __device__ inline size_t stereo_lds_bytes(int cap, int sort_n) { return (size_t)sort_n * (8 + 4 + 4 + 4) + (size_t)cap * 4 + 64; }

template <bool GW>
__global__ __launch_bounds__(1024) void k_stereo_match(StereoArgs A) {
    extern __shared__ __attribute__((aligned(16))) unsigned char s_st_lds[];
    unsigned char* s_st = GW ? A.work + (size_t)blockIdx.x * A.work_bytes : s_st_lds;
    const int p = blockIdx.x, t = threadIdx.x, cap = A.cap, sn = A.sort_n;
    unsigned long long* keys = reinterpret_cast<unsigned long long*>(s_st);
    float* ry = reinterpret_cast<float*>(keys + sn);
    int* rid = reinterpret_cast<int*>(ry + sn);
    uint32_t* skeys = reinterpret_cast<uint32_t*>(rid + sn);
    int* sad = reinterpret_cast<int*>(skeys + sn);
    __shared__ int s_cnt, s_removed;
    const int N = min(A.nl[p], cap), Nr = min(A.nr[p], cap);
    const viorb_keypoint* kl = A.kl + (size_t)p * cap; const viorb_keypoint* kr = A.kr + (size_t)p * cap;
    const uint8_t* dl = A.dl + (size_t)p * cap * 32; const uint8_t* dr = A.dr + (size_t)p * cap * 32;
    float* uR = A.uright + (size_t)p * cap; float* dep = A.depth + (size_t)p * cap;
    for (int i = t; i < sn; i += blockDim.x)
        keys[i] = i < Nr ? (((unsigned long long)__float_as_uint(kr[i].y) << 32) | (unsigned)i) : ~0ull;
    if (t == 0) { s_cnt = 0; s_removed = 0; }
    __syncthreads();
    for (int k = 2; k <= sn; k <<= 1)
        for (int j = k >> 1; j > 0; j >>= 1) {
            for (int q = t; q < (sn >> 1); q += blockDim.x) {
                const int lo = ((q & ~(j - 1)) << 1) | (q & (j - 1)), hi = lo | j;
                const bool up = (lo & k) == 0;
                const unsigned long long x = keys[lo], y = keys[hi];
                if ((x > y) == up) { keys[lo] = y; keys[hi] = x; }
            }
            __syncthreads();
        }
    for (int i = t; i < sn; i += blockDim.x) { ry[i] = i < Nr ? __uint_as_float((unsigned)(keys[i] >> 32)) : 3.0e38f; rid[i] = (int)(keys[i] & 0xffffffffu); }
    __syncthreads();
    const float mb = A.bf / A.fx, minD = 0.f, maxD = A.bf / mb;
    const float rmax = 2.0f * A.scale[A.nlevels - 1];
    const int nRows = A.lv[0].h;
    const int thOrbDist = (100 + 50) / 2;
    for (int iL = t; iL < cap; iL += blockDim.x) {
        float out_u = -1.f, out_d = -1.f; int out_sad = -1;
        if (iL < N) {
            const viorb_keypoint kpL = kl[iL];
            const int levelL = kpL.octave; const float vL = kpL.y, uL = kpL.x;
            const int rowi = (int)vL;
            const float minU = uL - maxD, maxU = uL - minD;
            if (rowi >= 0 && rowi < nRows && !(maxU < 0)) {
                const float ylo = (float)rowi - rmax - 1.0f, yhi = (float)rowi + rmax + 1.0f;
                int lo = 0, hi = Nr;
                while (lo < hi) { const int mid = (lo + hi) >> 1; if (ry[mid] < ylo) lo = mid + 1; else hi = mid; }
                const uint4* pl = reinterpret_cast<const uint4*>(dl + (size_t)iL * 32);
                const uint4 da = pl[0], db = pl[1];
                uint32_t best = 0xffffffffu;
                for (int k = lo; k < Nr && ry[k] <= yhi; k++) {
                    const int iR = rid[k];
                    const viorb_keypoint kpR = kr[iR];
                    const float r = 2.0f * A.scale[kpR.octave];
                    const int maxr = (int)ceilf(kpR.y + r), minr = (int)floorf(kpR.y - r);
                    if (rowi < minr || rowi > maxr) continue;
                    if (kpR.octave < levelL - 1 || kpR.octave > levelL + 1) continue;
                    if (!(kpR.x >= minU && kpR.x <= maxU)) continue;
                    const uint4* pr = reinterpret_cast<const uint4*>(dr + (size_t)iR * 32);
                    const uint4 ea = pr[0], eb = pr[1];
                    const int dist = __popc(da.x ^ ea.x) + __popc(da.y ^ ea.y) + __popc(da.z ^ ea.z) + __popc(da.w ^ ea.w) +
                                     __popc(db.x ^ eb.x) + __popc(db.y ^ eb.y) + __popc(db.z ^ eb.z) + __popc(db.w ^ eb.w);
                    if (dist < 100) best = min(best, ((uint32_t)dist << 16) | (uint32_t)iR);
                }
                if (best != 0xffffffffu && (int)(best >> 16) < thOrbDist) {
                    const int bestIdxR = (int)(best & 0xffff);
                    const float uR0 = kr[bestIdxR].x;
                    const float sfac = A.inv_scale[levelL];
                    const int cu = (int)roundf(kpL.x * sfac), cv = (int)roundf(kpL.y * sfac), cr = (int)roundf(uR0 * sfac);
                    const LevelDev Lv = A.lv[levelL];
                    const int w = 5, L = 5;
                    const float iniu = (float)cr + L - w, endu = (float)cr + L + w + 1;
                    const bool inside = !(iniu < 0 || endu >= Lv.w) && cv - w >= 0 && cv + w < Lv.h && cu - w >= 0 && cu + w < Lv.w &&
                                        cr - L - w >= 0 && cr + L + w < Lv.w;
                    if (inside) {
                        const uint8_t* IL = A.planesL + (size_t)p * A.frame_bytes + Lv.plane_off;
                        const uint8_t* IR = A.planesR + (size_t)p * A.frame_bytes + Lv.plane_off;
                        const int cL = IL[(size_t)cv * Lv.stride + cu];
                        int cRv[11], acc[11];
#pragma unroll
                        for (int sft = 0; sft < 11; sft++) { cRv[sft] = IR[(size_t)cv * Lv.stride + cr + sft - L]; acc[sft] = 0; }
                        for (int dy = -w; dy <= w; dy++) {
                            const uint8_t* rl = IL + (size_t)(cv + dy) * Lv.stride + cu - w;
                            const uint8_t* rr = IR + (size_t)(cv + dy) * Lv.stride + cr - L - w;
                            int lrow[11], rrow[21];
#pragma unroll
                            for (int x = 0; x < 11; x++) lrow[x] = (int)rl[x] - cL;
#pragma unroll
                            for (int x = 0; x < 21; x++) rrow[x] = rr[x];
#pragma unroll
                            for (int sft = 0; sft < 11; sft++)
#pragma unroll
                                for (int x = 0; x < 11; x++) acc[sft] += abs(lrow[x] - (rrow[sft + x] - cRv[sft]));
                        }
                        int bestSad = 0x7fffffff, bestinc = 0;
#pragma unroll
                        for (int sft = 0; sft < 11; sft++) if (acc[sft] < bestSad) { bestSad = acc[sft]; bestinc = sft - L; }
                        if (!(bestinc == -L || bestinc == L)) {
                            float d1 = 0, d2 = 0, d3 = 0;
#pragma unroll
                            for (int sft = 1; sft < 10; sft++) if (sft - L == bestinc) { d1 = (float)acc[sft - 1]; d2 = (float)acc[sft]; d3 = (float)acc[sft + 1]; }
                            const float deltaR = (d1 - d3) / (2.0f * (d1 + d3 - 2.0f * d2));
                            if (!(deltaR < -1 || deltaR > 1)) {
                                float bestuR = A.scale[levelL] * ((float)cr + (float)bestinc + deltaR);
                                float disparity = uL - bestuR;
                                if (disparity >= minD && disparity < maxD) {
                                    if (disparity <= 0) { disparity = 0.01f; bestuR = (float)((double)uL - 0.01); }
                                    out_d = A.bf / disparity; out_u = bestuR; out_sad = bestSad;
                                }
                            }
                        }
                    }
                }
            }
        }
        uR[iL] = out_u; dep[iL] = out_d; sad[iL] = out_sad;
    }
    __syncthreads();
    for (int i = t; i < sn; i += blockDim.x) skeys[i] = (i < cap && sad[i] >= 0) ? (((uint32_t)sad[i] << 16) | (uint32_t)i) : 0xffffffffu;
    for (int i = t; i < cap; i += blockDim.x) if (sad[i] >= 0) atomicAdd(&s_cnt, 1);
    __syncthreads();
    for (int k = 2; k <= sn; k <<= 1)
        for (int j = k >> 1; j > 0; j >>= 1) {
            for (int q = t; q < (sn >> 1); q += blockDim.x) {
                const int lo = ((q & ~(j - 1)) << 1) | (q & (j - 1)), hi = lo | j;
                const bool up = (lo & k) == 0;
                const uint32_t x = skeys[lo], y = skeys[hi];
                if ((x > y) == up) { skeys[lo] = y; skeys[hi] = x; }
            }
            __syncthreads();
        }
    const int cnt = s_cnt;
    if (cnt > 0) {
        const float median = (float)(skeys[cnt / 2] >> 16);
        const float thDist = 1.5f * 1.4f * median;
        for (int i = t; i < cnt; i += blockDim.x) {
            const uint32_t e = skeys[i];
            if (!((float)(e >> 16) < thDist)) { const int iL = (int)(e & 0xffff); uR[iL] = -1.f; dep[iL] = -1.f; atomicAdd(&s_removed, 1); }
        }
    }
    __syncthreads();
    if (t == 0) A.nmatched[p] = cnt - s_removed;
}

}

using namespace viorb;

struct viorb_extractor {
    viorb_extractor_params p;
    int max_batch = 1, device = 0;
    std::vector<float> scale, inv_scale, sigma2, inv_sigma2;
    std::vector<int> quota;
    int umax[16];
    int img_w = 0, img_h = 0;
    std::vector<LevelDev> lv;
    std::vector<CellDesc> cells;
    std::vector<int4> blur_tiles;
    size_t frame_bytes = 0;
    int slot_cap = 0, kp_pitch = 0, out_cap = 0;
    int fast_tile_pitch = 0, fast_tile_rows = 0, fast_tile_bytes = 0, fast_score_bytes = 0, fast_list_cap = 0;
    bool fast_v3 = false;
    int fast3_tile_bytes = 0, fast3_score_bytes = 0;
    int oct_ncap = 0, oct_nodecap = 0, oct_sortcap = 0;
    std::vector<std::pair<int, int>> oct_tiers;
    int oct_first_cap = 0, oct_node_x10 = 50;
    int oct_big_cap = 0, oct_big_slots = 0; uint32_t* d_oct_big = nullptr; int* d_oct_big_next = nullptr; int* d_lvl_tot = nullptr;
    unsigned char* d_stereo_work = nullptr; size_t stereo_work_bytes = 0;
    bool oct_huge = false; uint8_t* d_oct_nodes = nullptr; size_t oct_node_bytes = 0;
    std::vector<int> rs_pitch_dw, rs_rows;
    std::vector<int4> rs2_tiles; std::vector<int> rs2_off, rs2_pitch_dw, rs2_ok; bool rs2_copy_ok = false;
    int4* d_rs2_tiles = nullptr;
    std::vector<int4> rss_items; std::vector<uint2> rss_etab; std::vector<int> rss_item_off, rss_etab_off, rss_ok;
    int4* d_rss_items = nullptr; uint2* d_rss_etab = nullptr;
    uint8_t *d_planes = nullptr, *d_blur = nullptr, *d_desc = nullptr, *d_stage = nullptr;
    LevelDev* d_lv = nullptr; CellDesc* d_cells = nullptr; int4* d_blur_tiles = nullptr;
    int2 *d_xtab = nullptr, *d_ytab = nullptr;
    uint32_t *d_slots = nullptr, *d_lvl_kp = nullptr;
    int *d_cell_cnt = nullptr, *d_lvl_cnt = nullptr, *d_lvl_ncand = nullptr, *d_count = nullptr, *d_status = nullptr;
    viorb_keypoint* d_kps = nullptr;
    size_t stage_bytes = 0;
    hipStream_t own_stream = nullptr;
    hipStream_t aux_stream = nullptr; hipEvent_t ev_fork = nullptr, ev_join = nullptr;
    hipStream_t last_stream = nullptr;
    int last_batch = 0;
    unsigned fast_prof_rot = 0;
    bool tables_uploaded = false;
};

static void free_device(viorb_extractor* h) {
    void* ptrs[] = {h->d_planes, h->d_blur, h->d_desc, h->d_stage, h->d_lv, h->d_cells, h->d_blur_tiles, h->d_xtab,
                    h->d_ytab, h->d_slots, h->d_lvl_kp, h->d_cell_cnt, h->d_lvl_cnt, h->d_lvl_ncand, h->d_count,
                    h->d_status, h->d_kps, h->d_rs2_tiles, h->d_rss_items, h->d_rss_etab, h->d_oct_big, h->d_oct_big_next, h->d_lvl_tot, h->d_oct_nodes};
    for (void* p : ptrs) if (p) (void)hipFree(p);
    h->d_rs2_tiles = nullptr; h->d_rss_items = nullptr; h->d_rss_etab = nullptr; h->d_oct_big = nullptr; h->d_oct_big_next = nullptr; h->d_lvl_tot = nullptr; h->d_oct_nodes = nullptr;
    h->d_planes = h->d_blur = h->d_desc = h->d_stage = nullptr; h->d_lv = nullptr; h->d_cells = nullptr;
    h->d_blur_tiles = nullptr; h->d_xtab = h->d_ytab = nullptr; h->d_slots = h->d_lvl_kp = nullptr;
    h->d_cell_cnt = h->d_lvl_cnt = h->d_lvl_ncand = h->d_count = h->d_status = nullptr; h->d_kps = nullptr;
    h->stage_bytes = 0;
}

static int max_keypoints_for_size(const viorb_extractor* h, int w, int hgt) {
    int cap = 0;
    for (int l = 0; l < h->p.nlevels; l++) {
        const float s = h->inv_scale[l];
        const int lw = host_cv_round((double)((float)w * s)), lh = host_cv_round((double)((float)hgt * s));
        const int ow = lw - 2 * MINB, oh = lh - 2 * MINB;
        const int n_ini = (oh > 0 && ow > 0) ? (int)roundf((float)ow / (float)oh) : 0;
        cap += std::max(h->quota[l] + 2, 4 * n_ini);
    }
    return cap;
}

static int configure(viorb_extractor* h, int w, int hgt) {
    const int nl = h->p.nlevels;
    free_device(h);
    h->lv.assign(nl, LevelDev());
    h->cells.clear(); h->blur_tiles.clear();
    std::vector<int2> xtab, ytab;
    h->rs_pitch_dw.assign(nl, 0); h->rs_rows.assign(nl, 0);
    h->rs2_tiles.clear(); h->rs2_off.assign(nl, 0); h->rs2_pitch_dw.assign(nl, 1); h->rs2_ok.assign(nl, 0); h->rs2_copy_ok = false;
    h->rss_items.clear(); h->rss_etab.clear(); h->rss_item_off.assign(nl + 1, 0); h->rss_etab_off.assign(nl, 0); h->rss_ok.assign(nl, 0);
    size_t off = 0;
    int kp_off = 0, max_cw = 0, max_ch = 0;
    for (int l = 0; l < nl; l++) {
        LevelDev& L = h->lv[l];
        const float s = h->inv_scale[l];
        L.w = host_cv_round((double)((float)w * s));
        L.h = host_cv_round((double)((float)hgt * s));
        if (L.w < 1 || L.h < 1 || L.w > 4095 || L.h > 4095) { set_error("level %d size %dx%d unsupported", l, L.w, L.h); return VIORB_ERR_UNSUPPORTED; }
        L.stride = (int)align_up(L.w, 64);
        L.plane_off = (uint32_t)off;
        off += align_up((size_t)L.stride * L.h, 256);
        L.quota = h->quota[l];
        L.scale = h->scale[l];
        L.kp_size = (float)(int)(PATCH * h->scale[l]);
        const int maxBX = L.w - MINB, maxBY = L.h - MINB;
        const float width = (float)(maxBX - MINB), height = (float)(maxBY - MINB);
        L.oct_w = maxBX - MINB; L.oct_h = maxBY - MINB;
        L.cell_base = (int)h->cells.size();
        const int nCols = (int)(width / 30.f), nRows = (int)(height / 30.f);
        if (nCols >= 1 && nRows >= 1) {
            const int wCell = (int)ceilf(width / nCols), hCell = (int)ceilf(height / nRows);
            for (int i = 0; i < nRows; i++) {
                const float iniY = (float)(MINB + i * hCell);
                float maxY = iniY + hCell + 6;
                if (iniY >= maxBY - 3) continue;
                if (maxY > maxBY) maxY = (float)maxBY;
                for (int j = 0; j < nCols; j++) {
                    const float iniX = (float)(MINB + j * wCell);
                    float maxX = iniX + wCell + 6;
                    if (iniX >= maxBX - 6) continue;
                    if (maxX > maxBX) maxX = (float)maxBX;
                    CellDesc c;
                    c.level = l; c.x0 = (int)iniX; c.y0 = (int)iniY;
                    c.cw = (int)maxX - (int)iniX; c.ch = (int)maxY - (int)iniY;
                    c.shx = j * wCell; c.shy = i * hCell; c.pitch = (int)align_up(c.cw + 3, 4) + 4;
                    c.src_off = (uint32_t)(L.plane_off + (size_t)c.y0 * L.stride + (size_t)(c.x0 & ~3)); c.stride = L.stride;
                    if (c.cw < 7 || c.ch < 7) continue;
                    h->cells.push_back(c);
                    max_cw = std::max(max_cw, (int)c.cw); max_ch = std::max(max_ch, (int)c.ch);
                }
            }
        }
        L.ncells = (int)h->cells.size() - L.cell_base;
        L.n_ini = (L.oct_h > 0 && L.oct_w > 0) ? (int)roundf((float)L.oct_w / (float)L.oct_h) : 0;
        L.hx = L.n_ini > 0 ? (float)L.oct_w / (float)L.n_ini : 1.f;
        L.kp_off = kp_off;
        kp_off += std::max(L.quota, 4 * L.n_ini) + 4;
        L.xtab_off = (int)xtab.size(); L.ytab_off = (int)ytab.size();
        if (l > 0) {
            const int sw = h->lv[l - 1].w, sh = h->lv[l - 1].h;
            const double inv_sx = (double)L.w / sw, inv_sy = (double)L.h / sh;
            const double scale_x = 1. / inv_sx, scale_y = 1. / inv_sy;
            for (int dx = 0; dx < L.w; dx++) {
                float fx = (float)((dx + 0.5) * scale_x - 0.5);
                int sx = host_cv_floor(fx);
                fx -= sx;
                if (sx < 0) { fx = 0; sx = 0; }
                if (sx + 1 >= sw && sx >= sw - 1) { fx = 0; sx = sw - 1; }
                const int a0 = clampi(host_cv_round((double)((1.f - fx) * 2048)), -32768, 32767);
                const int a1 = clampi(host_cv_round((double)(fx * 2048)), -32768, 32767);
                const int sx1 = std::min(sx + 1, sw - 1);
                xtab.push_back(make_int2(sx | (sx1 << 16), (a0 & 0xffff) | (a1 << 16)));
            }
            for (int dy = 0; dy < L.h; dy++) {
                float fy = (float)((dy + 0.5) * scale_y - 0.5);
                int sy = host_cv_floor(fy);
                fy -= sy;
                const int b0 = clampi(host_cv_round((double)((1.f - fy) * 2048)), -32768, 32767);
                const int b1 = clampi(host_cv_round((double)(fy * 2048)), -32768, 32767);
                const int sy0 = clampi(sy, 0, sh - 1), sy1 = clampi(sy + 1, 0, sh - 1);
                ytab.push_back(make_int2(sy0 | (sy1 << 16), (b0 & 0xffff) | (b1 << 16)));
            }
            int maxdw = 1, maxrows = 1;
            const int2* xt = xtab.data() + L.xtab_off; const int2* yt = ytab.data() + L.ytab_off;
            for (int tx = 0; tx < L.w; tx += RS_TW) {
                const int x1 = std::min(tx + RS_TW, L.w) - 1;
                const int xs0 = (xt[tx].x & 0xffff) & ~3, xs1 = xt[x1].x >> 16;
                maxdw = std::max(maxdw, ((xs1 - xs0) >> 2) + 1);
            }
            for (int ty = 0; ty < L.h; ty += RS_TH) {
                const int y1 = std::min(ty + RS_TH, L.h) - 1;
                maxrows = std::max(maxrows, (yt[y1].x >> 16) - (yt[ty].x & 0xffff) + 1);
            }
            h->rs_pitch_dw[l] = maxdw; h->rs_rows[l] = maxrows;
            if ((size_t)maxdw * maxrows * 4 > 60000) { set_error("resize tile does not fit LDS (scale factor too large)"); return VIORB_ERR_UNSUPPORTED; }
            {
                h->rs2_off[l] = (int)h->rs2_tiles.size();
                int pdw = 1, prow = 1; bool cover = true; int next_x = 0, next_y = 0;
                const int gx2 = (L.w + RS2_TW - 1) / RS2_TW, gy2 = (L.h + RS2_TH - 1) / RS2_TH;
                for (int ty = 0; ty < gy2; ty++) {
                    const int y0t = ty * RS2_TH, y1t = std::min(y0t + RS2_TH, L.h) - 1;
                    const int ys0 = yt[y0t].x & 0xffff, ys1 = yt[y1t].x >> 16;
                    if (ys0 > next_y) cover = false;
                    next_y = std::max(next_y, ys1 + 1);
                    next_x = 0;
                    for (int tx = 0; tx < gx2; tx++) {
                        const int x0t = tx * RS2_TW, x1t = std::min(x0t + RS2_TW, L.w) - 1;
                        const int xs0 = (xt[x0t].x & 0xffff) & ~3, xs1 = xt[x1t].x >> 16;
                        if (xs0 > next_x) cover = false;
                        next_x = std::max(next_x, (xs1 | 3) + 1);
                        const int ndw = ((xs1 - xs0) >> 2) + 1, nrows = ys1 - ys0 + 1;
                        pdw = std::max(pdw, ndw); prow = std::max(prow, nrows);
                        h->rs2_tiles.push_back(make_int4(xs0, ndw, ys0, nrows));
                    }
                    if (next_x < sw) cover = false;
                }
                if (next_y < sh) cover = false;
                h->rs2_pitch_dw[l] = pdw;
                h->rs2_ok[l] = (prow <= 48 && pdw * prow <= 256 * RS2_TRIPS) ? 1 : 0;
                if (l == 1) h->rs2_copy_ok = cover && h->rs2_ok[1];
            }
            {
                static const bool no_stream = getenv("VIORB_RESIZE_TILES") != nullptr;
                bool ok = !no_stream && sw >= 8;
                h->rss_etab_off[l] = (int)h->rss_etab.size();
                std::vector<uint2> et(sh, make_uint2(0x7fffu, 0u));
                for (int dy = 0; dy < L.h && ok; dy++) {
                    const int sy0 = yt[dy].x & 0xffff, sy1 = yt[dy].x >> 16;
                    if ((sy1 != sy0 && sy1 != sy0 + 1) || et[sy1].x != 0x7fffu || dy >= 0x7fff) { ok = false; break; }
                    const int b0 = yt[dy].y & 0xffff, b1 = (yt[dy].y >> 16) & 0xffff;
                    if (b0 > 2048 || b1 > 2048) { ok = false; break; }
                    et[sy1] = make_uint2((uint32_t)dy | (sy1 == sy0 ? 0x8000u : 0u), (uint32_t)b0 | ((uint32_t)b1 << 16));
                }
                const int ndw = (L.w + 3) / 4;
                for (int dcol = 0; dcol < ndw && ok; dcol++) {
                    const int first = xt[std::min(4 * dcol, L.w - 1)].x & 0xffff;
                    for (int j = 0; j < 4; j++) {
                        const int2 e = xt[std::min(4 * dcol + j, L.w - 1)];
                        if ((e.x >> 16) - first > 7 || (e.x & 0xffff) < first || (e.y & 0xffff) > 2048 || ((e.y >> 16) & 0xffff) > 2048) ok = false;
                    }
                }
                h->rss_item_off[l] = (int)h->rss_items.size();
                if (ok) {
                    const double sy = (double)sh / L.h;
                    const int rbmax = std::max(1, std::min(100, (int)((RSS_MAX_SRC_ROWS - 2) / sy)));
                    const int nb = 2 * ((L.h + 2 * rbmax - 1) / (2 * rbmax)), rb = (L.h + nb - 1) / nb;
                    for (int k = 0; k < nb && ok; k++) {
                        const int ya = k * rb, yb = std::min(ya + rb, L.h) - 1;
                        if (ya <= yb && (yt[yb].x >> 16) - (yt[ya].x & 0xffff) + 1 > RSS_MAX_SRC_ROWS) ok = false;
                    }
                    for (int sx = 0; sx < ndw && ok; sx += RSS_LANES)
                        for (int k = 0; k < nb; k += 2)
                            if (k * rb < L.h) h->rss_items.push_back(make_int4(sx, k * rb, rb, 0));
                }
                if (!ok) h->rss_items.resize(h->rss_item_off[l]);
                h->rss_ok[l] = ok ? 1 : 0;
                h->rss_etab.insert(h->rss_etab.end(), et.begin(), et.end());
            }
        }
        {
            const int nb = 2 * ((L.h + 127) / 128), rb = (L.h + nb - 1) / nb, ndw = (L.w + 3) / 4;
            for (int sx = 0; sx < ndw; sx += BS_LANES)
                for (int k = 0; k < nb; k += 2) h->blur_tiles.push_back(make_int4(l, sx, k * rb, rb));
            if (L.w < 12 || L.h < 4) { set_error("level %d (%dx%d) too small for the blur", l, L.w, L.h); return VIORB_ERR_UNSUPPORTED; }
        }
    }
    h->frame_bytes = align_up(off, 256);
    h->kp_pitch = kp_off;
    h->out_cap = max_keypoints_for_size(h, w, hgt);
    const int ncells = (int)h->cells.size();
    if (ncells == 0) { set_error("image %dx%d too small for a FAST cell grid", w, hgt); return VIORB_ERR_UNSUPPORTED; }
    h->fast_tile_pitch = (int)align_up(max_cw + 3, 4) + 4;
    h->fast_tile_rows = max_ch;
    {
        int tb = 64 * FAST_FETCH_TRIPS * 4;
        for (const CellDesc& c : h->cells) tb = std::max(tb, c.pitch * c.ch);
        h->fast_tile_bytes = (int)align_up((size_t)tb, 16);
    }
    h->fast_score_bytes = (int)align_up((size_t)(max_cw - 6 + 2) * (max_ch - 6 + 2), 4);
    h->slot_cap = ((max_cw - 6 + 1) / 2) * ((max_ch - 6 + 1) / 2);
    h->fast_list_cap = (int)align_up((size_t)(max_cw - 6) * (max_ch - 6), 2);
    if (max_cw - 6 > 255 || max_ch - 6 > 255) { set_error("FAST cell larger than 255 px"); return VIORB_ERR_UNSUPPORTED; }
    {
        bool ok = true;
        for (const CellDesc& c : h->cells) ok = ok && ((c.x0 & 3) + c.cw <= 4 * F3_TPD - 4) && c.ch <= 4 * F3_TRIPS && c.cw - 6 + 2 <= F3_SP && c.ch - 6 + 2 <= F3_SROWS;
        static const bool force_v2 = getenv("VIORB_FAST_V2") != nullptr;
        h->fast_v3 = ok && !force_v2;
        h->fast3_tile_bytes = (int)align_up((size_t)(4 * ((max_ch + 3) / 4)) * F3_TP, 16);
        h->fast3_score_bytes = (int)align_up((size_t)(max_ch - 6 + 2) * F3_SP + 16, 16);
    }
    int maxq = 1; for (int l = 0; l < nl; l++) maxq = std::max(maxq, h->quota[l]);
    h->oct_ncap = 8192;
    h->oct_nodecap = 5 * maxq + 64;
    int sc = 1; while (sc < maxq + 8) sc <<= 1;
    h->oct_sortcap = sc;
    size_t oct_lds = (size_t)h->oct_ncap * 8 + (size_t)h->oct_nodecap * sizeof(OctNode) + (size_t)sc * 4;
    if (h->oct_nodecap > 65535) { set_error("per-level quota %d too large for the quadtree's 16-bit node indices", maxq); return VIORB_ERR_UNSUPPORTED; }
    h->oct_huge = oct_lds > 160 * 1024;
    if (!h->oct_huge && oct_lds > 64 * 1024 &&
        raise_dynamic_lds(reinterpret_cast<const void*>(k_octree<false>), oct_lds) != hipSuccess) {
        (void)hipGetLastError();
        h->oct_ncap = 4096;
        oct_lds = (size_t)h->oct_ncap * 8 + (size_t)h->oct_nodecap * sizeof(OctNode) + (size_t)sc * 4;
        if (oct_lds > 64 * 1024) { set_error("quadtree LDS (%zu B) exceeds the dynamic-LDS limit", oct_lds); return VIORB_ERR_UNSUPPORTED; }
    }

    if (!h->oct_huge) {
        const size_t lds_big = (size_t)h->oct_sortcap * 8 + (size_t)h->oct_nodecap * sizeof(OctNodeBig);
        if (lds_big > 160 * 1024) h->oct_huge = true;
        else if (lds_big > 64 * 1024) VIORB_HIP_TRY(raise_dynamic_lds(reinterpret_cast<const void*>(k_octree<true>), lds_big));
    }
    {
        const char* e = getenv("VIORB_OCT_TIERS");
        std::string spec = e ? e : "3:2048";
        h->oct_tiers.clear();
        for (int l = 0; l < nl; l++) h->lv[l].oct_tier_cap = 0;
        int prev_l = 0, prev_c = std::min(h->oct_ncap, (int)OCT_NCAP_SMALL);
        h->oct_first_cap = prev_c;
        { const char* e2 = getenv("VIORB_OCT_NODE_X10"); h->oct_node_x10 = e2 ? atoi(e2) : 25; if (h->oct_node_x10 < 10 || h->oct_node_x10 > 50) h->oct_node_x10 = 50; }
        size_t pos = 0;
        while (!h->oct_huge && pos < spec.size()) {
            int l = 0, c = 0, used = 0;
            if (sscanf(spec.c_str() + pos, "%d:%d%n", &l, &c, &used) != 2) break;
            if (l == 0 && h->oct_tiers.empty() && c >= 64 && c <= prev_c) { h->oct_first_cap = c; prev_c = c + 1; }
            else if (l <= prev_l || l >= nl || c < 64 || c >= prev_c) break;
            else { h->oct_tiers.push_back(std::make_pair(l, c)); prev_l = l; prev_c = c; }
            pos += (size_t)used; if (pos < spec.size() && spec[pos] == ',') pos++;
        }
        for (size_t ti = 0; ti < h->oct_tiers.size(); ti++) {
            const int l1 = ti + 1 < h->oct_tiers.size() ? h->oct_tiers[ti + 1].first : nl;
            for (int l = h->oct_tiers[ti].first; l < l1; l++) h->lv[l].oct_tier_cap = h->oct_tiers[ti].second;
        }
    }
    const size_t B = (size_t)h->max_batch;
    VIORB_HIP_TRY(hipMalloc(&h->d_planes, B * h->frame_bytes));
    VIORB_HIP_TRY(hipMalloc(&h->d_blur, B * h->frame_bytes));
    VIORB_HIP_TRY(hipMalloc(&h->d_lv, sizeof(LevelDev) * nl));
    VIORB_HIP_TRY(hipMalloc(&h->d_cells, sizeof(CellDesc) * ncells));
    VIORB_HIP_TRY(hipMalloc(&h->d_blur_tiles, sizeof(int4) * h->blur_tiles.size()));
    VIORB_HIP_TRY(hipMalloc(&h->d_rs2_tiles, sizeof(int4) * std::max<size_t>(h->rs2_tiles.size(), 1)));
    VIORB_HIP_TRY(hipMalloc(&h->d_rss_items, sizeof(int4) * std::max<size_t>(h->rss_items.size(), 1)));
    VIORB_HIP_TRY(hipMalloc(&h->d_rss_etab, sizeof(uint2) * std::max<size_t>(h->rss_etab.size(), 1)));
    VIORB_HIP_TRY(hipMalloc(&h->d_xtab, sizeof(int2) * std::max<size_t>(xtab.size(), 1)));
    VIORB_HIP_TRY(hipMalloc(&h->d_ytab, sizeof(int2) * std::max<size_t>(ytab.size(), 1)));
    VIORB_HIP_TRY(hipMalloc(&h->d_slots, B * ncells * h->slot_cap * sizeof(uint32_t)));
    VIORB_HIP_TRY(hipMalloc(&h->d_cell_cnt, B * ncells * sizeof(int)));
    VIORB_HIP_TRY(hipMalloc(&h->d_lvl_kp, B * h->kp_pitch * sizeof(uint32_t)));
    VIORB_HIP_TRY(hipMalloc(&h->d_lvl_cnt, B * nl * sizeof(int)));
    VIORB_HIP_TRY(hipMalloc(&h->d_lvl_ncand, B * nl * sizeof(int)));
    VIORB_HIP_TRY(hipMalloc(&h->d_lvl_tot, B * nl * sizeof(int)));
    {
        int big = 1;
        for (int l = 0; l < nl; l++) big = std::max(big, h->lv[l].ncells * h->slot_cap);
        h->oct_big_cap = (int)align_up((size_t)big, 64);
        h->oct_big_slots = h->oct_huge ? (int)(B * nl) : (int)std::min<size_t>(B * nl, 64);
        VIORB_HIP_TRY(hipMalloc(&h->d_oct_big, (size_t)h->oct_big_slots * 3 * h->oct_big_cap * sizeof(uint32_t)));
        VIORB_HIP_TRY(hipMalloc(&h->d_oct_big_next, sizeof(int)));
        if (h->oct_huge) {
            h->oct_node_bytes = align_up((size_t)h->oct_sortcap * 8 + (size_t)h->oct_nodecap * sizeof(OctNodeBig), 256);
            VIORB_HIP_TRY(hipMalloc(&h->d_oct_nodes, (size_t)h->oct_big_slots * h->oct_node_bytes));
        }
    }
    VIORB_HIP_TRY(hipMalloc(&h->d_kps, B * h->out_cap * sizeof(viorb_keypoint)));
    VIORB_HIP_TRY(hipMalloc(&h->d_desc, B * h->out_cap * 32));
    VIORB_HIP_TRY(hipMalloc(&h->d_count, B * sizeof(int)));
    VIORB_HIP_TRY(hipMalloc(&h->d_status, B * sizeof(int)));
    VIORB_HIP_TRY(hipMemset(h->d_planes, 0, B * h->frame_bytes));
    VIORB_HIP_TRY(hipMemset(h->d_blur, 0, B * h->frame_bytes));
    VIORB_HIP_TRY(hipMemset(h->d_count, 0, B * sizeof(int)));
    VIORB_HIP_TRY(hipMemset(h->d_status, 0, B * sizeof(int)));
    VIORB_HIP_TRY(hipMemset(h->d_lvl_cnt, 0, B * nl * sizeof(int)));
    VIORB_HIP_TRY(hipMemcpy(h->d_lv, h->lv.data(), sizeof(LevelDev) * nl, hipMemcpyHostToDevice));
    VIORB_HIP_TRY(hipMemcpy(h->d_cells, h->cells.data(), sizeof(CellDesc) * ncells, hipMemcpyHostToDevice));
    VIORB_HIP_TRY(hipMemcpy(h->d_blur_tiles, h->blur_tiles.data(), sizeof(int4) * h->blur_tiles.size(), hipMemcpyHostToDevice));
    if (!h->rs2_tiles.empty()) VIORB_HIP_TRY(hipMemcpy(h->d_rs2_tiles, h->rs2_tiles.data(), sizeof(int4) * h->rs2_tiles.size(), hipMemcpyHostToDevice));
    if (!h->rss_items.empty()) VIORB_HIP_TRY(hipMemcpy(h->d_rss_items, h->rss_items.data(), sizeof(int4) * h->rss_items.size(), hipMemcpyHostToDevice));
    if (!h->rss_etab.empty()) VIORB_HIP_TRY(hipMemcpy(h->d_rss_etab, h->rss_etab.data(), sizeof(uint2) * h->rss_etab.size(), hipMemcpyHostToDevice));
    if (!xtab.empty()) VIORB_HIP_TRY(hipMemcpy(h->d_xtab, xtab.data(), sizeof(int2) * xtab.size(), hipMemcpyHostToDevice));
    if (!ytab.empty()) VIORB_HIP_TRY(hipMemcpy(h->d_ytab, ytab.data(), sizeof(int2) * ytab.size(), hipMemcpyHostToDevice));
    if (!h->tables_uploaded) {
        int g[7];
        {
            float cf[7]; double sum = 0; const double s2 = -0.5 / (2.0 * 2.0);
            for (int i = 0; i < 7; i++) { double x = i - 3.0; cf[i] = (float)exp(s2 * x * x); sum += cf[i]; }
            sum = 1. / sum;
            for (int i = 0; i < 7; i++) { cf[i] = (float)(cf[i] * sum); g[i] = host_cv_round((double)(cf[i] * 256.f)); }
        }
        uint32_t pat[256];
        for (int i = 0; i < 256; i++)
            pat[i] = (uint32_t)(uint8_t)kPatternHost[4 * i] | ((uint32_t)(uint8_t)kPatternHost[4 * i + 1] << 8) |
                     ((uint32_t)(uint8_t)kPatternHost[4 * i + 2] << 16) | ((uint32_t)(uint8_t)kPatternHost[4 * i + 3] << 24);
        VIORB_HIP_TRY(hipMemcpyToSymbol(HIP_SYMBOL(c_gauss), g, sizeof(g)));
        {
            uint32_t rc[64]; rc[0] = 0;
            for (int d = 1; d < 64; d++) rc[d] = (65536u + d - 1) / d;
            VIORB_HIP_TRY(hipMemcpyToSymbol(HIP_SYMBOL(c_rcp16), rc, sizeof(rc)));
        }
        VIORB_HIP_TRY(hipMemcpyToSymbol(HIP_SYMBOL(c_pattern), pat, sizeof(pat)));
        VIORB_HIP_TRY(hipMemcpyToSymbol(HIP_SYMBOL(c_umax), h->umax, sizeof(int) * 16));
        uint32_t om[256];
        for (int row = 0; row < 32; row++)
            for (int j = 0; j < 8; j++) {
                uint32_t m = 0;
                for (int k2 = 0; k2 < 4; k2++) {
                    const int u = -HALF_PATCH + 4 * j + k2, v = row - HALF_PATCH;
                    if (row < PATCH && u <= HALF_PATCH && std::abs(u) <= h->umax[std::abs(v)]) m |= 0xffu << (8 * k2);
                }
                om[row * 8 + j] = m;
            }
        VIORB_HIP_TRY(hipMemcpyToSymbol(HIP_SYMBOL(c_orient_mask), om, sizeof(om)));
        h->tables_uploaded = true;
    }
    h->img_w = w; h->img_h = hgt;
    return VIORB_OK;
}

static int fast_launch_images(int batch) {
    static const int nlaunch = getenv("VIORB_FAST_LAUNCHES") ? std::max(1, atoi(getenv("VIORB_FAST_LAUNCHES"))) : FAST_LAUNCHES;
    return std::min(std::max(batch, 1), std::max(8, ((batch + nlaunch - 1) / nlaunch + 7) & ~7));
}

static int launch_all(viorb_extractor* h, const uint8_t* d_images, int batch, int stride, size_t pitch, hipStream_t st) {
    const int nl = h->p.nlevels;
    const int ncells = (int)h->cells.size();
    const LevelDev& L0 = h->lv[0];
    const bool fuse_copy = batch < 16 && nl > 1 && h->rs2_copy_ok && (stride & 3) == 0 && (pitch & 3) == 0 && (((uintptr_t)d_images) & 3) == 0 && (L0.w & 3) == 0;
    if (!fuse_copy) {
        const int gx = (L0.stride / 16 + 63) / 64;
        const XcdPlace PL = make_place(gx * L0.h, batch);
        ProfScope ps("k_copy_level0", st);
        hipLaunchKernelGGL(k_copy_level0, dim3(place_blocks(PL)), dim3(64), 0, st, d_images, L0.w, L0.h, stride, pitch, h->d_planes, h->frame_bytes, L0.stride, h->d_status, PL, gx);
    }
    for (int l = 1; l < nl; l++) {
        const LevelDev& L = h->lv[l];
        if (h->rss_ok[l] && !(l == 1 && fuse_copy)) {
            const LevelDev& P = h->lv[l - 1];
            ResizeStreamArgs A;
            A.planes = h->d_planes; A.frame_bytes = h->frame_bytes; A.src_off = P.plane_off; A.dst_off = L.plane_off;
            A.src_stride = P.stride; A.src_h = P.h; A.dst_stride = L.stride; A.dst_w = L.w; A.dst_h = L.h;
            A.xtab = h->d_xtab + L.xtab_off; A.ytab = h->d_ytab + L.ytab_off; A.etab = h->d_rss_etab + h->rss_etab_off[l];
            A.items = h->d_rss_items + h->rss_item_off[l];
            const int nitems = (l + 1 < nl ? h->rss_item_off[l + 1] : (int)h->rss_items.size()) - h->rss_item_off[l];
            const XcdPlace PL = make_place(nitems, batch);
            ProfScope ps("k_resize", st);
            hipLaunchKernelGGL(k_resize_stream, dim3(place_blocks(PL)), dim3(64), 0, st, A, PL);
            continue;
        }
        if (h->rs2_ok[l]) {
            const LevelDev& P = h->lv[l - 1];
            Resize2Args A;
            const bool from_image = (l == 1 && fuse_copy);
            A.src = from_image ? d_images : h->d_planes + P.plane_off; A.src_pitch = from_image ? pitch : h->frame_bytes; A.src_stride = from_image ? stride : P.stride;
            A.dst = h->d_planes + L.plane_off; A.dst_pitch = h->frame_bytes; A.dst_stride = L.stride; A.dst_w = L.w; A.dst_h = L.h;
            A.copy_dst = from_image ? h->d_planes + L0.plane_off : nullptr; A.copy_pitch = h->frame_bytes; A.copy_stride = L0.stride;
            A.xtab = h->d_xtab + L.xtab_off; A.ytab = h->d_ytab + L.ytab_off; A.tiles = h->d_rs2_tiles + h->rs2_off[l];
            A.gx = (L.w + RS2_TW - 1) / RS2_TW; A.lds_pitch_dw = h->rs2_pitch_dw[l]; A.status = from_image ? h->d_status : nullptr;
            const int gy = (L.h + RS2_TH - 1) / RS2_TH;
            const XcdPlace PL = make_place(A.gx * gy, batch);
            const size_t lds = (size_t)A.lds_pitch_dw * 48 * 4 + (RS2_TW + RS2_TH) * sizeof(int2);
            ProfScope ps("k_resize", st);
            hipLaunchKernelGGL(k_resize2, dim3(place_blocks(PL)), dim3(256), lds, st, A, PL);
            continue;
        }
        const int gx = (L.w + RS_TW - 1) / RS_TW, gy = (L.h + RS_TH - 1) / RS_TH;
        const XcdPlace PL = make_place(gx * gy, batch);
        const size_t lds = (size_t)h->rs_pitch_dw[l] * h->rs_rows[l] * 4;
        ProfScope ps("k_resize", st);
        hipLaunchKernelGGL(k_resize, dim3(place_blocks(PL)), dim3(256), lds, st, h->d_planes, h->frame_bytes, h->d_lv, l, h->d_xtab, h->d_ytab,
                           h->rs_pitch_dw[l], h->rs_rows[l], PL, gx);
    }
    {
        const size_t lds = h->fast_v3 ? (size_t)h->fast3_tile_bytes + h->fast3_score_bytes + (size_t)(F3_SURV_CAP + F3_CORN_CAP) * 2
                                      : (size_t)h->fast_tile_bytes + h->fast_score_bytes + (size_t)h->fast_list_cap * 4;
        const int step = fast_launch_images(batch);
        h->fast_prof_rot++;
        for (int i0 = 0; i0 < batch; i0 += step) {
            ProfScope ps(prof_times_everything() || (i0 / step) == (int)(h->fast_prof_rot % (unsigned)((batch + step - 1) / step)) ? "k_fast_cells" : nullptr, st);
            const XcdPlace PL = make_place((ncells + FAST_CELLS_PER_WAVE - 1) / FAST_CELLS_PER_WAVE, batch, i0, std::min(batch, i0 + step));
            if (h->fast_v3)
                hipLaunchKernelGGL(k_fast_cells3, dim3(place_blocks(PL)), dim3(64), lds, st, h->d_planes, h->frame_bytes, h->d_cells,
                                   h->p.ini_th_fast, h->p.min_th_fast, h->d_slots, h->slot_cap, h->d_cell_cnt, ncells, h->fast3_tile_bytes, h->fast3_score_bytes, PL);
            else
                hipLaunchKernelGGL(k_fast_cells, dim3(place_blocks(PL)), dim3(64), lds, st, h->d_planes, h->frame_bytes, h->d_lv, h->d_cells,
                                   h->p.ini_th_fast, h->p.min_th_fast, h->d_slots, h->slot_cap, h->d_cell_cnt, ncells,
                                   h->fast_tile_bytes, h->fast_score_bytes, h->fast_list_cap, PL);
        }
    }
    static const bool fork_blur = !(getenv("VIORB_BLUR_FORK") && atoi(getenv("VIORB_BLUR_FORK")) == 0);
    hipStream_t bst = st;
    if (fork_blur && batch >= 16) {
        if (!h->aux_stream) {
            VIORB_HIP_TRY(hipStreamCreateWithFlags(&h->aux_stream, hipStreamNonBlocking));
            VIORB_HIP_TRY(hipEventCreateWithFlags(&h->ev_fork, hipEventDisableTiming));
            VIORB_HIP_TRY(hipEventCreateWithFlags(&h->ev_join, hipEventDisableTiming));
        }
        bst = h->aux_stream;
        VIORB_HIP_TRY(hipEventRecord(h->ev_fork, st));
        VIORB_HIP_TRY(hipStreamWaitEvent(bst, h->ev_fork, 0));
    }
    {
        ProfScope ps("k_blur", bst);
        const XcdPlace PL = make_place((int)h->blur_tiles.size(), batch);
        hipLaunchKernelGGL(k_blur, dim3(place_blocks(PL)), dim3(64), 0, bst, h->d_planes, h->d_blur, h->frame_bytes,
                           h->d_lv, h->d_blur_tiles, PL);
    }
    if (bst != st) VIORB_HIP_TRY(hipEventRecord(h->ev_join, bst));
    {
        const size_t fixed = (size_t)h->oct_nodecap * sizeof(OctNode) + (size_t)h->oct_sortcap * 4;
        const int small = h->oct_first_cap > 0 ? h->oct_first_cap : std::min(h->oct_ncap, (int)OCT_NCAP_SMALL);
        const int ntier = h->oct_huge ? 0 : (int)h->oct_tiers.size();
        const bool defer = h->oct_node_x10 < 50;
        auto first_nodes = [&](int mq) { return std::min(5 * mq + 64, (h->oct_node_x10 * mq) / 10 + 64); };
        if (!h->oct_huge) {
            ProfScope ps("k_octree", st);
            const int l_end0 = ntier ? h->oct_tiers[0].first : nl;
            int mq0 = 1; for (int l = 0; l < l_end0; l++) mq0 = std::max(mq0, h->quota[l]);
            const int ndc0 = defer ? first_nodes(mq0) : h->oct_nodecap;
            hipLaunchKernelGGL(k_octree<false>, dim3(batch, l_end0), dim3(64), (size_t)small * 8 + (size_t)ndc0 * sizeof(OctNode) + (size_t)h->oct_sortcap * 4, st,
                               h->d_lv, h->d_slots, h->slot_cap, h->d_cell_cnt,
                               ncells, h->d_lvl_kp, h->kp_pitch, h->d_lvl_cnt, h->d_lvl_ncand, nl, h->d_status, small, ndc0,
                               h->oct_sortcap, -1, small, 0, 0, defer ? 1 : 0, nullptr, nullptr, 0, h->d_lvl_tot);
            for (int ti = 0; ti < ntier; ti++) {
                const int l0 = h->oct_tiers[ti].first, l1 = ti + 1 < ntier ? h->oct_tiers[ti + 1].first : nl, nc = h->oct_tiers[ti].second;
                int mq = 1; for (int l = l0; l < l1; l++) mq = std::max(mq, h->quota[l]);
                const int ndc = defer ? first_nodes(mq) : 5 * mq + 64;
                hipLaunchKernelGGL(k_octree<false>, dim3(batch, l1 - l0), dim3(64), (size_t)nc * 8 + (size_t)ndc * sizeof(OctNode) + (size_t)h->oct_sortcap * 4,
                                   st, h->d_lv, h->d_slots, h->slot_cap, h->d_cell_cnt, ncells, h->d_lvl_kp, h->kp_pitch, h->d_lvl_cnt, h->d_lvl_ncand, nl, h->d_status,
                                   nc, ndc, h->oct_sortcap, -1, nc, l0, 0, defer ? 1 : 0, nullptr, nullptr, 0, h->d_lvl_tot);
            }
        }
        if (!h->oct_huge && (small < h->oct_ncap || ntier || defer)) {
            ProfScope ps("k_octree_large", st);
            hipLaunchKernelGGL(k_octree<false>, dim3(batch, nl), dim3(64), (size_t)h->oct_ncap * 8 + fixed, st, h->d_lv, h->d_slots, h->slot_cap,
                               h->d_cell_cnt, ncells, h->d_lvl_kp, h->kp_pitch, h->d_lvl_cnt, h->d_lvl_ncand, nl, h->d_status, h->oct_ncap,
                               h->oct_nodecap, h->oct_sortcap, small, h->oct_ncap, 0, ntier ? 1 : 0, 0, nullptr, nullptr, 0, h->d_lvl_tot);
        }
        {
            const size_t lds_big = h->oct_huge ? 0 : (size_t)h->oct_sortcap * 8 + (size_t)h->oct_nodecap * sizeof(OctNodeBig);
            VIORB_HIP_TRY(hipMemsetAsync(h->d_oct_big_next, 0, sizeof(int), st));
            ProfScope ps("k_octree_big", st);
            hipLaunchKernelGGL(k_octree<true>, dim3(batch, nl), dim3(64), lds_big, st, h->d_lv, h->d_slots, h->slot_cap, h->d_cell_cnt, ncells, h->d_lvl_kp,
                               h->kp_pitch, h->d_lvl_cnt, h->d_lvl_ncand, nl, h->d_status, h->oct_big_cap, h->oct_nodecap, h->oct_sortcap,
                               h->oct_huge ? -1 : std::max(h->oct_ncap, (int)small), 0x7fffffff, 0, 0, 0, h->d_oct_big, h->d_oct_big_next, h->oct_big_slots, h->d_lvl_tot,
                               h->oct_huge ? h->d_oct_nodes : (uint8_t*)nullptr, h->oct_node_bytes);
        }
    }
    if (bst != st) VIORB_HIP_TRY(hipStreamWaitEvent(st, h->ev_join, 0));
    {
        ProfScope ps("k_orient_describe", st);
        const XcdPlace PL = make_place((h->out_cap + 3) / 4, batch);
        hipLaunchKernelGGL(k_orient_describe, dim3(place_blocks(PL)), dim3(256), 0, st, h->d_planes, h->d_blur, h->frame_bytes,
                           h->d_lv, nl, h->d_lvl_kp, h->kp_pitch, h->d_lvl_cnt, h->d_kps, h->d_desc, h->out_cap, h->d_count, h->d_status, PL);
    }
    VIORB_HIP_TRY(hipGetLastError());
    h->last_stream = st; h->last_batch = batch;
    return VIORB_OK;
}

extern "C" {

int viorb_abi_version(void) { return 2; }

int viorb_memcpy_dtod_async(void* dst, const void* src, size_t bytes, void* stream) {
    VIORB_REQUIRE(dst && src, "null pointer");
    VIORB_HIP_TRY(hipMemcpyAsync(dst, src, bytes, hipMemcpyDeviceToDevice, (hipStream_t)stream));
    return VIORB_OK;
}

int viorb_profile_enable(int on) {
    g_prof.enabled = on != 0;
    return VIORB_OK;
}
int viorb_profile_reset(void) {
    g_prof.used = 0;
    return VIORB_OK;
}
int viorb_profile_select(const char* kernel_name) {
    g_prof.only = kernel_name ? kernel_name : "";
    return VIORB_OK;
}
int viorb_profile_read(char* names_buf, int names_cap, double* total_ms, int* calls, int cap, int* n) {
    VIORB_REQUIRE(names_buf && total_ms && calls && n, "null argument");
    VIORB_HIP_TRY(hipDeviceSynchronize());
    const int k = (int)g_prof.names.size();
    *n = k;
    std::string all;
    for (int i = 0; i < k; i++) { all += g_prof.names[i]; all += '\n'; }
    snprintf(names_buf, names_cap, "%s", all.c_str());
    for (int i = 0; i < k && i < cap; i++) { total_ms[i] = 0; calls[i] = 0; }
    for (size_t r = 0; r < g_prof.used; r++) {
        float ms = 0;
        if (hipEventElapsedTime(&ms, g_prof.recs[r].a, g_prof.recs[r].b) != hipSuccess) continue;
        const int slot = g_prof.recs[r].slot;
        if (slot >= 0 && slot < cap) { total_ms[slot] += ms; calls[slot]++; }
    }
    return VIORB_OK;
}
int viorb_profile_timeline(double* start_ms, double* end_ms, int* slot, int cap, int* n) {
    VIORB_REQUIRE(start_ms && end_ms && slot && n, "null argument");
    VIORB_HIP_TRY(hipDeviceSynchronize());
    *n = (int)g_prof.used;
    for (size_t r = 0; r < g_prof.used && (int)r < cap; r++) {
        float a = 0, b = 0;
        (void)hipEventElapsedTime(&a, g_prof.recs[0].a, g_prof.recs[r].a);
        (void)hipEventElapsedTime(&b, g_prof.recs[0].a, g_prof.recs[r].b);
        start_ms[r] = a; end_ms[r] = b; slot[r] = g_prof.recs[r].slot;
    }
    return VIORB_OK;
}
const char* viorb_last_error(void) { return viorb::last_error_buf(); }
int viorb_device_count(void) {
    int n = 0;
    if (hipGetDeviceCount(&n) != hipSuccess) return 0;
    return n;
}

int viorb_extractor_create(const viorb_extractor_params* params, int max_batch, int device, viorb_extractor** out) {
    VIORB_REQUIRE(params && out, "null params/out");
    VIORB_REQUIRE(params->nlevels >= 1 && params->nlevels <= MAX_LEVELS, "nlevels must be 1..16");
    VIORB_REQUIRE(params->nfeatures >= 1 && params->scale_factor > 1.0f, "nfeatures >= 1, scale_factor > 1");
    VIORB_REQUIRE(max_batch >= 1, "max_batch >= 1");
    viorb_extractor* h = new viorb_extractor();
    h->p = *params; h->max_batch = max_batch; h->device = device;
    const int nl = params->nlevels;
    const double sf = (double)params->scale_factor;
    h->scale.resize(nl); h->sigma2.resize(nl); h->inv_scale.resize(nl); h->inv_sigma2.resize(nl); h->quota.resize(nl);
    h->scale[0] = 1.f; h->sigma2[0] = 1.f;
    for (int i = 1; i < nl; i++) { h->scale[i] = (float)(h->scale[i - 1] * sf); h->sigma2[i] = h->scale[i] * h->scale[i]; }
    for (int i = 0; i < nl; i++) { h->inv_scale[i] = 1.0f / h->scale[i]; h->inv_sigma2[i] = 1.0f / h->sigma2[i]; }
    const float factor = (float)(1.0f / sf);
    float nd = params->nfeatures * (1 - factor) / (1 - (float)pow((double)factor, (double)nl));
    int sum = 0;
    for (int l = 0; l < nl - 1; l++) { h->quota[l] = host_cv_round(nd); sum += h->quota[l]; nd *= factor; }
    h->quota[nl - 1] = std::max(params->nfeatures - sum, 0);
    {
        int v, v0, vmax = host_cv_floor(HALF_PATCH * sqrtf(2.f) / 2 + 1), vmin = host_cv_ceil(HALF_PATCH * sqrtf(2.f) / 2);
        const double hp2 = HALF_PATCH * HALF_PATCH;
        for (v = 0; v < 16; v++) h->umax[v] = 0;
        for (v = 0; v <= vmax; ++v) h->umax[v] = host_cv_round(sqrt(hp2 - v * v));
        for (v = HALF_PATCH, v0 = 0; v >= vmin; --v) { while (h->umax[v0] == h->umax[v0 + 1]) ++v0; h->umax[v] = v0; ++v0; }
    }
    *out = h;
    return VIORB_OK;
}

int viorb_extractor_destroy(viorb_extractor* h) {
    if (!h) return VIORB_OK;
    if (h->d_planes) { (void)hipSetDevice(h->device); free_device(h); }
    if (h->d_stereo_work) (void)hipFree(h->d_stereo_work);
    if (h->own_stream) (void)hipStreamDestroy(h->own_stream);
    if (h->aux_stream) (void)hipStreamDestroy(h->aux_stream);
    if (h->ev_fork) (void)hipEventDestroy(h->ev_fork);
    if (h->ev_join) (void)hipEventDestroy(h->ev_join);
    delete h;
    return VIORB_OK;
}

int viorb_extractor_tables(const viorb_extractor* h, float* scale, float* inv_scale, float* sigma2, float* inv_sigma2,
                           int32_t* fpl) {
    VIORB_REQUIRE(h, "null handle");
    for (int i = 0; i < h->p.nlevels; i++) {
        if (scale) scale[i] = h->scale[i];
        if (inv_scale) inv_scale[i] = h->inv_scale[i];
        if (sigma2) sigma2[i] = h->sigma2[i];
        if (inv_sigma2) inv_sigma2[i] = h->inv_sigma2[i];
        if (fpl) fpl[i] = h->quota[i];
    }
    return VIORB_OK;
}

int viorb_extractor_fast_launch_images(int batch) { return fast_launch_images(batch); }

int viorb_extractor_max_keypoints(const viorb_extractor* h, int* cap) {
    VIORB_REQUIRE(h && cap, "null handle/cap");
    int c = 0; for (int l = 0; l < h->p.nlevels; l++) c += h->quota[l] + 2;
    *cap = c;
    return VIORB_OK;
}

int viorb_extractor_max_keypoints_for(const viorb_extractor* h, int width, int height, int* cap) {
    VIORB_REQUIRE(h && cap && width > 0 && height > 0, "null handle/cap or empty size");
    *cap = max_keypoints_for_size(h, width, height);
    return VIORB_OK;
}

static int ensure_device(viorb_extractor* h, int w, int hgt) {
    if (viorb_device_count() < 1) { set_error("no HIP device: libviorb_hip has no CPU fallback"); return VIORB_ERR_NO_DEVICE; }
    VIORB_HIP_TRY(hipSetDevice(h->device));
    if (w != h->img_w || hgt != h->img_h || !h->d_planes) {
        int rc = configure(h, w, hgt);
        if (rc != VIORB_OK) { h->img_w = h->img_h = 0; return rc; }
    }
    return VIORB_OK;
}

int viorb_extract_batch_device(viorb_extractor* h, const uint8_t* d_images, int batch, int width, int height, int stride,
                               size_t pitch, void* stream) {
    VIORB_REQUIRE(h && d_images, "null handle/images");
    VIORB_REQUIRE(batch >= 1 && batch <= h->max_batch, "batch out of range");
    VIORB_REQUIRE(width > 0 && height > 0 && stride >= width, "bad image geometry");
    int rc = ensure_device(h, width, height);
    if (rc != VIORB_OK) return rc;
    return launch_all(h, d_images, batch, stride, pitch, (hipStream_t)stream);
}

int viorb_extractor_results_device(const viorb_extractor* h, const viorb_keypoint** d_kps, const uint8_t** d_desc,
                                   const int32_t** d_count, const int32_t** d_status, int* cap) {
    VIORB_REQUIRE(h && h->d_kps, "no results yet");
    if (d_kps) *d_kps = h->d_kps;
    if (d_desc) *d_desc = h->d_desc;
    if (d_count) *d_count = h->d_count;
    if (d_status) *d_status = h->d_status;
    if (cap) *cap = h->out_cap;
    return VIORB_OK;
}

int viorb_extractor_download(viorb_extractor* h, int b, viorb_keypoint* kps, uint8_t* desc, int cap, int* n) {
    VIORB_REQUIRE(h && h->d_kps && n, "no results yet");
    VIORB_REQUIRE(b >= 0 && b < h->last_batch, "image index out of range");
    VIORB_HIP_TRY(hipSetDevice(h->device));
    VIORB_HIP_TRY(hipStreamSynchronize(h->last_stream));
    int cnt = 0, st = 0;
    VIORB_HIP_TRY(hipMemcpy(&cnt, h->d_count + b, sizeof(int), hipMemcpyDeviceToHost));
    VIORB_HIP_TRY(hipMemcpy(&st, h->d_status + b, sizeof(int), hipMemcpyDeviceToHost));
    *n = cnt;
    const int m = std::min(cnt, cap);
    if (m > 0 && kps) VIORB_HIP_TRY(hipMemcpy(kps, h->d_kps + (size_t)b * h->out_cap, sizeof(viorb_keypoint) * m, hipMemcpyDeviceToHost));
    if (m > 0 && desc) VIORB_HIP_TRY(hipMemcpy(desc, h->d_desc + (size_t)b * h->out_cap * 32, (size_t)32 * m, hipMemcpyDeviceToHost));
    if (st != VIORB_OK) { set_error("image %d: a capacity of the extractor was exceeded (quadtree nodes / scratch slots, or more keypoints kept than viorb_extractor_max_keypoints: a level whose quadtree roots outnumber a quarter of its quota)", b); return st; }
    if (cnt > cap) { set_error("caller capacity %d < %d keypoints", cap, cnt); return VIORB_ERR_CAPACITY; }
    return VIORB_OK;
}

int viorb_extract(viorb_extractor* h, const uint8_t* img, int width, int height, int stride, viorb_keypoint* kps,
                  uint8_t* desc, int cap, int* n) {
    VIORB_REQUIRE(h && n, "null handle/n");
    *n = 0;
    if (!img || width <= 0 || height <= 0) return VIORB_OK;
    VIORB_REQUIRE(stride >= width, "stride < width");
    int rc = ensure_device(h, width, height);
    if (rc != VIORB_OK) return rc;
    if (!h->own_stream) VIORB_HIP_TRY(hipStreamCreateWithFlags(&h->own_stream, hipStreamNonBlocking));
    const size_t bytes = (size_t)stride * height;
    if (h->stage_bytes < bytes) {
        if (h->d_stage) (void)hipFree(h->d_stage);
        h->d_stage = nullptr; h->stage_bytes = 0;
        VIORB_HIP_TRY(hipMalloc(&h->d_stage, bytes));
        h->stage_bytes = bytes;
    }
    VIORB_HIP_TRY(hipMemcpyAsync(h->d_stage, img, bytes, hipMemcpyHostToDevice, h->own_stream));
    rc = launch_all(h, h->d_stage, 1, stride, bytes, h->own_stream);
    if (rc != VIORB_OK) return rc;
    return viorb_extractor_download(h, 0, kps, desc, cap, n);
}

int viorb_extractor_level_device(const viorb_extractor* h, int b, int level, int blurred, const uint8_t** d_ptr, int* width,
                                 int* height, int* stride) {
    VIORB_REQUIRE(h && h->d_planes, "no pyramid yet");
    VIORB_REQUIRE(level >= 0 && level < h->p.nlevels && b >= 0 && b < h->max_batch, "level/image out of range");
    const LevelDev& L = h->lv[level];
    if (d_ptr) *d_ptr = (blurred ? h->d_blur : h->d_planes) + (size_t)b * h->frame_bytes + L.plane_off;
    if (width) *width = L.w;
    if (height) *height = L.h;
    if (stride) *stride = L.stride;
    return VIORB_OK;
}

int viorb_extractor_level_download(viorb_extractor* h, int b, int level, int blurred, uint8_t* dst, int* width, int* height) {
    const uint8_t* p = nullptr; int w = 0, hh = 0, s = 0;
    int rc = viorb_extractor_level_device(h, b, level, blurred, &p, &w, &hh, &s);
    if (rc != VIORB_OK) return rc;
    VIORB_HIP_TRY(hipSetDevice(h->device));
    VIORB_HIP_TRY(hipStreamSynchronize(h->last_stream));
    if (dst) VIORB_HIP_TRY(hipMemcpy2D(dst, w, p, s, w, hh, hipMemcpyDeviceToHost));
    if (width) *width = w;
    if (height) *height = hh;
    return VIORB_OK;
}

int viorb_stereo_match_device(const viorb_extractor* L, int left_index, const viorb_extractor* R, int right_index, int pairs, float bf, float fx,
                              float* d_uright, float* d_depth, int32_t* d_nmatched, void* stream) {
    VIORB_REQUIRE(L && R && L->d_kps && R->d_kps && d_uright && d_depth && d_nmatched, "extract both images first");
    VIORB_REQUIRE(pairs >= 1 && left_index >= 0 && right_index >= 0 && left_index + pairs <= L->max_batch && right_index + pairs <= R->max_batch,
                  "image indices out of range");
    VIORB_REQUIRE(L->img_w == R->img_w && L->img_h == R->img_h && L->out_cap == R->out_cap && L->p.nlevels == R->p.nlevels && L->device == R->device,
                  "left and right extractors must have the same geometry and parameters");
    VIORB_HIP_TRY(hipSetDevice(L->device));
    StereoArgs A;
    const int cap = L->out_cap;
    A.kl = L->d_kps + (size_t)left_index * cap; A.kr = R->d_kps + (size_t)right_index * cap;
    A.dl = L->d_desc + (size_t)left_index * cap * 32; A.dr = R->d_desc + (size_t)right_index * cap * 32;
    A.nl = L->d_count + left_index; A.nr = R->d_count + right_index;
    A.planesL = L->d_planes + (size_t)left_index * L->frame_bytes; A.planesR = R->d_planes + (size_t)right_index * R->frame_bytes;
    A.frame_bytes = L->frame_bytes; A.lv = L->d_lv; A.cap = cap; A.nlevels = L->p.nlevels; A.bf = bf; A.fx = fx;
    int sn = 64; while (sn < cap) sn <<= 1;
    A.sort_n = sn;
    for (int i = 0; i < 16; i++) { A.scale[i] = L->scale[i < L->p.nlevels ? i : L->p.nlevels - 1]; A.inv_scale[i] = L->inv_scale[i < L->p.nlevels ? i : L->p.nlevels - 1]; }
    A.uright = d_uright; A.depth = d_depth; A.nmatched = d_nmatched;
    const size_t lds = stereo_lds_bytes(cap, sn);
    A.work = nullptr; A.work_bytes = 0;
    ProfScope ps("k_stereo_match", (hipStream_t)stream);
    if (lds > 160 * 1024) {
        viorb_extractor* Lm = const_cast<viorb_extractor*>(L);
        const size_t per = (lds + 255) & ~(size_t)255;
        if (Lm->stereo_work_bytes < per * pairs) {
            VIORB_HIP_TRY(hipSetDevice(L->device));
            VIORB_HIP_TRY(hipDeviceSynchronize());
            if (Lm->d_stereo_work) (void)hipFree(Lm->d_stereo_work);
            Lm->d_stereo_work = nullptr; Lm->stereo_work_bytes = 0;
            VIORB_HIP_TRY(hipMalloc(&Lm->d_stereo_work, per * pairs));
            Lm->stereo_work_bytes = per * pairs;
        }
        A.work = Lm->d_stereo_work; A.work_bytes = per;
        hipLaunchKernelGGL(k_stereo_match<true>, dim3(pairs), dim3(1024), 0, (hipStream_t)stream, A);
    } else {
        if (lds > 64 * 1024) VIORB_HIP_TRY(raise_dynamic_lds(reinterpret_cast<const void*>(k_stereo_match<false>), lds));
        hipLaunchKernelGGL(k_stereo_match<false>, dim3(pairs), dim3(1024), lds, (hipStream_t)stream, A);
    }
    VIORB_HIP_TRY(hipGetLastError());
    return VIORB_OK;
}

int viorb_stereo_match(viorb_extractor* L, viorb_extractor* R, float bf, float fx, float* uright, float* depth, int cap, int* nmatched) {
    VIORB_REQUIRE(L && R && uright && depth && nmatched, "null argument");
    VIORB_REQUIRE(L->d_kps && R->d_kps, "extract both images first");
    VIORB_HIP_TRY(hipSetDevice(L->device));
    VIORB_HIP_TRY(hipStreamSynchronize(L->last_stream));
    VIORB_HIP_TRY(hipStreamSynchronize(R->last_stream));
    float *d_u = nullptr, *d_d = nullptr; int* d_n = nullptr;
    const int oc = L->out_cap;
    VIORB_HIP_TRY(hipMalloc(&d_u, sizeof(float) * oc)); VIORB_HIP_TRY(hipMalloc(&d_d, sizeof(float) * oc)); VIORB_HIP_TRY(hipMalloc(&d_n, sizeof(int)));
    int rc = viorb_stereo_match_device(L, 0, R, 0, 1, bf, fx, d_u, d_d, d_n, nullptr);
    if (rc == VIORB_OK && hipDeviceSynchronize() != hipSuccess) { set_error("stereo kernel failed"); rc = VIORB_ERR_HIP; }
    if (rc == VIORB_OK) {
        const int m = std::min(cap, oc);
        (void)hipMemcpy(uright, d_u, sizeof(float) * m, hipMemcpyDeviceToHost);
        (void)hipMemcpy(depth, d_d, sizeof(float) * m, hipMemcpyDeviceToHost);
        (void)hipMemcpy(nmatched, d_n, sizeof(int), hipMemcpyDeviceToHost);
    }
    (void)hipFree(d_u); (void)hipFree(d_d); (void)hipFree(d_n);
    return rc;
}

int viorb_extractor_debug_level_points(viorb_extractor* h, int b, int level, int which, int32_t* xyr, int cap, int* n) {
    VIORB_REQUIRE(h && h->d_planes && n, "no results yet");
    VIORB_REQUIRE(level >= 0 && level < h->p.nlevels && b >= 0 && b < h->last_batch, "level/image out of range");
    VIORB_HIP_TRY(hipSetDevice(h->device));
    VIORB_HIP_TRY(hipStreamSynchronize(h->last_stream));
    const LevelDev& L = h->lv[level];
    const int ncells = (int)h->cells.size();
    std::vector<uint32_t> keys;
    if (which == 0) {
        std::vector<int> cc(L.ncells);
        std::vector<uint32_t> sl((size_t)L.ncells * h->slot_cap);
        if (L.ncells > 0) {
            VIORB_HIP_TRY(hipMemcpy(cc.data(), h->d_cell_cnt + (size_t)b * ncells + L.cell_base, sizeof(int) * L.ncells, hipMemcpyDeviceToHost));
            VIORB_HIP_TRY(hipMemcpy(sl.data(), h->d_slots + ((size_t)b * ncells + L.cell_base) * h->slot_cap, sl.size() * 4, hipMemcpyDeviceToHost));
        }
        for (int c = 0; c < L.ncells; c++)
            for (int k = 0; k < cc[c]; k++) keys.push_back(sl[(size_t)c * h->slot_cap + k]);
    } else {
        int cnt = 0;
        VIORB_HIP_TRY(hipMemcpy(&cnt, h->d_lvl_cnt + b * h->p.nlevels + level, sizeof(int), hipMemcpyDeviceToHost));
        keys.resize(cnt);
        if (cnt > 0) VIORB_HIP_TRY(hipMemcpy(keys.data(), h->d_lvl_kp + (size_t)b * h->kp_pitch + L.kp_off, sizeof(uint32_t) * cnt, hipMemcpyDeviceToHost));
    }
    *n = (int)keys.size();
    for (int i = 0; i < (int)keys.size() && i < cap; i++) {
        xyr[3 * i] = (int)(keys[i] & 0xfff); xyr[3 * i + 1] = (int)((keys[i] >> 12) & 0xfff); xyr[3 * i + 2] = (int)(keys[i] >> 24);
    }
    return VIORB_OK;
}

int viorb_debug_octree_host(const uint32_t* keys, int n, int width, int height, int N, uint32_t* out, int cap, int* nout) {
    VIORB_REQUIRE(keys && out && nout && n >= 0 && n <= 65535, "bad arguments");
    std::vector<uint32_t> k(keys, keys + n);
    std::vector<uint32_t> r = distribute_octree_arrays(k, width, height, N);
    *nout = (int)r.size();
    for (int i = 0; i < (int)r.size() && i < cap; i++) out[i] = r[i];
    return VIORB_OK;
}
float viorb_debug_fast_atan2(float y, float x) { return fast_atan2_deg(y, x); }
void viorb_debug_sincos(float r, float* s, float* c) { sincos_f32(r, s, c); }

}
```

viorb_amd/extractor.py:

```python
import ctypes as C
import numpy as np
from . import capi
from .capi import lib, check, ptr, KP_DTYPE


class ORBextractor:
    def __init__(self, nfeatures=1000, scaleFactor=1.2, nlevels=8, iniThFAST=20, minThFAST=7,
                 max_batch=1, device=0):
        self.L = lib()
        self.params = capi.ExtractorParams(nfeatures, scaleFactor, nlevels, iniThFAST, minThFAST)
        self.nlevels = nlevels
        self.max_batch = max_batch
        h = C.c_void_p()
        check(self.L.viorb_extractor_create(C.byref(self.params), max_batch, device, C.byref(h)))
        self.h = h
        cap = C.c_int()
        check(self.L.viorb_extractor_max_keypoints(self.h, C.byref(cap)))
        self.cap = cap.value

    def __del__(self):
        if getattr(self, "h", None):
            self.L.viorb_extractor_destroy(self.h)
            self.h = None

    def GetLevels(self):
        return self.nlevels

    def GetScaleFactor(self):
        return self.params.scale_factor

    def tables(self):
        n = self.nlevels
        sf, isf, s2, is2 = (np.zeros(n, np.float32) for _ in range(4))
        q = np.zeros(n, np.int32)
        check(self.L.viorb_extractor_tables(self.h, ptr(sf), ptr(isf), ptr(s2), ptr(is2), ptr(q)))
        return dict(scale=sf, inv_scale=isf, sigma2=s2, inv_sigma2=is2, quota=q)

    def GetScaleFactors(self):
        return self.tables()["scale"]

    def GetInverseScaleFactors(self):
        return self.tables()["inv_scale"]

    def GetScaleSigmaSquares(self):
        return self.tables()["sigma2"]

    def GetInverseScaleSigmaSquares(self):
        return self.tables()["inv_sigma2"]

    def __call__(self, image, mask=None):
        if image is None or image.size == 0:
            return np.zeros(0, KP_DTYPE), np.zeros((0, 32), np.uint8)
        assert image.dtype == np.uint8 and image.ndim == 2
        image = np.ascontiguousarray(image)
        h, w = image.shape
        cap = self.capacity_for(w, h)
        kps = np.zeros(cap, KP_DTYPE)
        desc = np.zeros((cap, 32), np.uint8)
        n = C.c_int()
        check(self.L.viorb_extract(self.h, ptr(image), w, h, image.strides[0], ptr(kps), ptr(desc), cap, C.byref(n)))
        return kps[:n.value].copy(), desc[:n.value].copy()

    def capacity_for(self, width, height):
        cap = C.c_int()
        check(self.L.viorb_extractor_max_keypoints_for(self.h, int(width), int(height), C.byref(cap)))
        self.cap = cap.value
        return cap.value

    def extract_batch_device(self, images, stream=None):
        import torch
        assert images.is_cuda and images.dtype == torch.uint8 and images.dim() == 3
        B, h, w = images.shape
        assert images.stride(2) == 1
        st = stream if stream is not None else torch.cuda.current_stream(images.device)
        check(self.L.viorb_extract_batch_device(self.h, ptr(images), B, w, h, images.stride(1), images.stride(0),
                                                C.c_void_p(st.cuda_stream)))
        self._last_batch = B
        self.capacity_for(w, h)

    def download(self, b):
        kps = np.zeros(self.cap, KP_DTYPE)
        desc = np.zeros((self.cap, 32), np.uint8)
        n = C.c_int()
        check(self.L.viorb_extractor_download(self.h, b, ptr(kps), ptr(desc), self.cap, C.byref(n)))
        return kps[:n.value].copy(), desc[:n.value].copy()

    def results_device(self):
        a, b, c, d = C.c_void_p(), C.c_void_p(), C.c_void_p(), C.c_void_p()
        cap = C.c_int()
        check(self.L.viorb_extractor_results_device(self.h, C.byref(a), C.byref(b), C.byref(c), C.byref(d), C.byref(cap)))
        return a.value, b.value, c.value, d.value, cap.value

    def level(self, l, b=0, blurred=False):
        w, h = C.c_int(), C.c_int()
        check(self.L.viorb_extractor_level_download(self.h, b, l, int(blurred), None, C.byref(w), C.byref(h)))
        out = np.zeros((h.value, w.value), np.uint8)
        check(self.L.viorb_extractor_level_download(self.h, b, l, int(blurred), ptr(out), C.byref(w), C.byref(h)))
        return out

    def debug_level_points(self, l, b=0, kept=False):
        buf = np.zeros((131072, 3), np.int32)
        n = C.c_int()
        check(self.L.viorb_extractor_debug_level_points(self.h, b, l, int(kept), ptr(buf), len(buf), C.byref(n)))
        return buf[:min(n.value, len(buf))].copy()


def ComputeStereoMatches(ex_left, ex_right, bf, fx):
    u, d = np.zeros(ex_left.cap, np.float32), np.zeros(ex_left.cap, np.float32)
    n = C.c_int()
    check(lib().viorb_stereo_match(ex_left.h, ex_right.h, float(bf), float(fx), ptr(u), ptr(d), ex_left.cap, C.byref(n)))
    return u, d, n.value


def octree_host(keys_xyr, width, height, N):
    k = np.asarray(keys_xyr, np.int64).reshape(-1, 3)
    packed = (k[:, 0] | (k[:, 1] << 12) | (k[:, 2] << 24)).astype(np.uint32)
    out = np.zeros(len(packed) + 16, np.uint32)
    n = C.c_int()
    check(lib().viorb_debug_octree_host(ptr(packed), len(packed), width, height, N, ptr(out), len(out), C.byref(n)))
    o = out[:n.value].astype(np.int64)
    return np.stack([o & 0xfff, (o >> 12) & 0xfff, o >> 24], axis=1).astype(np.int32)
```

Measured before the change: 191,500.

## Partition quadtree keys directly in LDS with in-place register-resident splits

```diff
diff --git a/include/viorb.h b/include/viorb.h
--- a/include/viorb.h
+++ b/include/viorb.h
@@ -75,6 +75,11 @@
 
 int viorb_extractor_debug_level_points(viorb_extractor* h, int b, int level, int which, int32_t* xyr,
                                        int cap, int* n);
+
+typedef struct viorb_quadtree_plan {
+    int32_t level_begin, level_end, candidates, nodes, lds_bytes, in_place;
+} viorb_quadtree_plan;
+int viorb_extractor_quadtree_plans(const viorb_extractor* h, viorb_quadtree_plan* plans, int cap, int* n);
 
 typedef struct viorb_frontend viorb_frontend;
 
diff --git a/viorb_amd/capi.py b/viorb_amd/capi.py
--- a/viorb_amd/capi.py
+++ b/viorb_amd/capi.py
@@ -95,6 +95,7 @@
     "viorb_stereo_match_device": (i32, [vp, i32, vp, i32, i32, f32, f32, vp, vp, vp, vp]),
     "viorb_stereo_match": (i32, [vp, vp, f32, f32, vp, vp, i32, PP(i32)]),
     "viorb_extractor_debug_level_points": (i32, [vp, i32, i32, i32, vp, i32, PP(i32)]),
+    "viorb_extractor_quadtree_plans": (i32, [vp, vp, i32, PP(i32)]),
     "viorb_frontend_create": (i32, [PP(FrontendConfig), i32, i32, i32, PP(vp)]),
     "viorb_frontend_search_capacity": (i32, []),
     "viorb_frontend_destroy": (i32, [vp]),
diff --git a/viorb_amd/csrc/orb_extractor.hip b/viorb_amd/csrc/orb_extractor.hip
--- a/viorb_amd/csrc/orb_extractor.hip
+++ b/viorb_amd/csrc/orb_extractor.hip
@@ -869,128 +869,206 @@
 
 #define WAVE_SYNC() __syncthreads()
 #define OCT_NCAP_SMALL 4096
+#ifndef OCT_INPLACE_MAX
+#define OCT_INPLACE_MAX 3072
+#endif
 struct OctNodeBig { int16_t x0, x1, y0, y1; uint32_t begin, count; uint16_t flags, pad; };
+static inline size_t oct_lds_bytes(int ncap, int nodecap, int sortcap, bool inplace) {
+    return (size_t)((ncap + 3) & ~3) * 4 * (inplace ? 1 : 2) + (size_t)nodecap * sizeof(OctNode) + (size_t)sortcap * 4;
+}
 template <bool BIG> struct OctT;
-template <> struct OctT<false> { typedef uint16_t Perm; typedef OctNode Node; typedef uint32_t SortKey; enum { KEY_SHIFT = 16 }; };
-template <> struct OctT<true> { typedef uint32_t Perm; typedef OctNodeBig Node; typedef unsigned long long SortKey; enum { KEY_SHIFT = 32 }; };
+template <> struct OctT<false> { typedef OctNode Node; typedef uint32_t SortKey; enum { KEY_SHIFT = 16 }; };
+template <> struct OctT<true> { typedef OctNodeBig Node; typedef unsigned long long SortKey; enum { KEY_SHIFT = 32 }; };
 template <bool BIG> struct OctLdsT {
-    uint32_t* keys; typename OctT<BIG>::Perm* perm0; typename OctT<BIG>::Perm* perm1; typename OctT<BIG>::Node* nd; typename OctT<BIG>::SortKey* sortb;
+    uint32_t* k0; int kd; typename OctT<BIG>::Node* nd; typename OctT<BIG>::SortKey* sortb;
+    __device__ __forceinline__ uint32_t* buf(int b) const { return k0 + (b ? kd : 0); }
+    __device__ __forceinline__ uint32_t* other(int b) const { return k0 + (b ? 0 : kd); }
 };
 
 __device__ __forceinline__ unsigned long long lanemask_lt(int lane) { return (1ull << lane) - 1ull; }
+__device__ __forceinline__ int oct_nth_set(unsigned long long m, int n) {
+    int pos = 0;
+#pragma unroll
+    for (int s = 32; s > 0; s >>= 1) {
+        const int c = __popcll((m >> pos) & ((1ull << s) - 1ull));
+        if (n >= c) { n -= c; pos += s; }
+    }
+    return pos;
+}
 
 #define OCT_LANE_LIMIT 64
 struct OctExpandResult { int off, nexp; };
 
-template <bool BIG> __device__ __forceinline__ void oct_write_children(const OctLdsT<BIG>& S, const typename OctT<BIG>::Node& p, int i, int slot, int mx, int my, int sb,
-                                                   const int tc[4], const int sc4[4]) {
+template <bool BIG> __device__ __forceinline__ void oct_write_boxes(const OctLdsT<BIG>& S, const typename OctT<BIG>::Node& p, int i, int slot, int mx, int my) {
+    typedef typename OctT<BIG>::Node Node;
 #pragma unroll
     for (int c = 0; c < 4; c++) {
-        typename OctT<BIG>::Node o;
-        o.x0 = (c & 1) ? (int16_t)mx : p.x0; o.x1 = (c & 1) ? p.x1 : (int16_t)mx;
-        o.y0 = (c & 2) ? (int16_t)my : p.y0; o.y1 = (c & 2) ? p.y1 : (int16_t)my;
-        o.begin = (decltype(o.begin))sc4[c]; o.count = (decltype(o.count))tc[c];
+        const int x0 = (c & 1) ? mx : (int)p.x0, x1 = (c & 1) ? (int)p.x1 : mx, y0 = (c & 2) ? my : (int)p.y0, y1 = (c & 2) ? (int)p.y1 : my;
+        uint32_t* to = reinterpret_cast<uint32_t*>(S.nd + slot + c);
+        to[0] = (uint32_t)(x0 & 0xffff) | ((uint32_t)x1 << 16);
+        to[1] = (uint32_t)(y0 & 0xffff) | ((uint32_t)y1 << 16);
+    }
+    S.nd[i].flags = p.flags | OCT_DEAD;
+}
+template <bool BIG> __device__ __forceinline__ void oct_write_ranges(const OctLdsT<BIG>& S, int slot, int sb, int beg, const int tc[4]) {
+    int s = beg;
+#pragma unroll
+    for (int c = 0; c < 4; c++) {
+        typename OctT<BIG>::Node& o = S.nd[slot + c];
+        o.begin = (decltype(o.begin))s; o.count = (decltype(o.count))tc[c];
         o.flags = tc[c] > 0 ? (uint16_t)((sb ^ 1) | (tc[c] == 1 ? OCT_NOMORE : 0)) : (uint16_t)OCT_DEAD; o.pad = 0;
-        S.nd[slot + c] = o;
-    }
-    S.nd[i].flags = p.flags | OCT_DEAD;
+        s += tc[c];
+    }
 }
 
 #define OCT_CODE(key) (((int)((key) & 0xfff) < mx ? 0 : 1) | ((int)(((key) >> 12) & 0xfff) < my ? 0 : 2))
-template <bool BIG> __device__ __forceinline__ OctExpandResult oct_expand_wave(const OctLdsT<BIG>& S, int i, int slot, int lane) {
-    typedef typename OctT<BIG>::Perm Perm;
+template <int R> __device__ __forceinline__ void oct_partition_regs(const uint32_t* src, uint32_t* dst, int cnt, int mx, int my, int lane, int t[4]) {
+    const unsigned long long lt = lanemask_lt(lane);
+    enum { NCD = (R + 9) / 10 };
+    uint32_t k[R], cd[NCD];
+#pragma unroll
+    for (int u = 0; u < R; u++) if (64 * u < cnt) k[u] = src[64 * u + lane];
+#pragma unroll
+    for (int u = 0; u < NCD; u++) cd[u] = 0;
+    t[0] = t[1] = t[2] = t[3] = 0;
+#pragma unroll
+    for (int u = 0; u < R; u++)
+        if (64 * u < cnt) {
+            const int c = 64 * u + lane < cnt ? OCT_CODE(k[u]) : -1;
+            cd[u / 10] |= (uint32_t)(c + 1) << (3 * (u % 10));
+            t[0] += __popcll(__ballot(c == 0)); t[1] += __popcll(__ballot(c == 1));
+            t[2] += __popcll(__ballot(c == 2)); t[3] += __popcll(__ballot(c == 3));
+            if (R > 16) __builtin_amdgcn_sched_barrier(0);
+        }
+    WAVE_SYNC();
+    int w0 = 0, w1 = t[0], w2 = w1 + t[1], w3 = w2 + t[2];
+#pragma unroll
+    for (int u = 0; u < R; u++)
+        if (64 * u < cnt) {
+            const int c = (int)((cd[u / 10] >> (3 * (u % 10))) & 7) - 1;
+            const unsigned long long m0 = __ballot(c == 0), m1 = __ballot(c == 1), m2 = __ballot(c == 2), m3 = __ballot(c == 3);
+            const unsigned long long mm = c == 0 ? m0 : (c == 1 ? m1 : (c == 2 ? m2 : m3));
+            int at = w3;
+            at = c == 2 ? w2 : at; at = c == 1 ? w1 : at; at = c == 0 ? w0 : at;
+            if (c >= 0) dst[at + __popcll(mm & lt)] = k[u];
+            w0 += __popcll(m0); w1 += __popcll(m1); w2 += __popcll(m2); w3 += __popcll(m3);
+            if (R > 16) __builtin_amdgcn_sched_barrier(0);
+        }
+}
+
+template <bool BIG> __device__ __forceinline__ OctExpandResult oct_expand_wave(const OctLdsT<BIG>& S, int i, int slot, int lane, bool inplace) {
     const typename OctT<BIG>::Node p = S.nd[i];
     const int mx = p.x0 + ((p.x1 - p.x0 + 1) >> 1), my = p.y0 + ((p.y1 - p.y0 + 1) >> 1);
     const int sb = p.flags & OCT_BUF;
-    const Perm* src = (sb ? S.perm1 : S.perm0) + (int)p.begin;
-    Perm* dst = sb ? S.perm0 : S.perm1;
     const int cnt = (int)p.count, beg = (int)p.begin;
-    const unsigned long long lt = lanemask_lt(lane);
+    const uint32_t* src = S.buf(sb) + beg;
+    uint32_t* dst = S.other(sb) + beg;
     int t[4] = {0, 0, 0, 0};
-    Perm id[4]; int c[4];
-    auto load4 = [&](int o) {
-#pragma unroll
-        for (int u = 0; u < 4; u++) id[u] = src[min(o + 64 * u + lane, cnt - 1)];
-#pragma unroll
-        for (int u = 0; u < 4; u++) { const uint32_t key = S.keys[id[u]]; c[u] = o + 64 * u + lane < cnt ? OCT_CODE(key) : -1; }
-    };
-    int w0, w1, w2, w3;
-    auto scatter4 = [&]() {
-#pragma unroll
-        for (int u = 0; u < 4; u++) {
-            const unsigned long long m0 = __ballot(c[u] == 0), m1 = __ballot(c[u] == 1), m2 = __ballot(c[u] == 2), m3 = __ballot(c[u] == 3);
-            const unsigned long long mm = c[u] == 0 ? m0 : (c[u] == 1 ? m1 : (c[u] == 2 ? m2 : m3));
-            int at = w3;
-            at = c[u] == 2 ? w2 : at; at = c[u] == 1 ? w1 : at; at = c[u] == 0 ? w0 : at;
-            if (c[u] >= 0) dst[at + __popcll(mm & lt)] = id[u];
-            w0 += __popcll(m0); w1 += __popcll(m1); w2 += __popcll(m2); w3 += __popcll(m3);
-        }
-    };
-    auto count4 = [&]() {
-#pragma unroll
-        for (int u = 0; u < 4; u++) {
-            t[0] += __popcll(__ballot(c[u] == 0)); t[1] += __popcll(__ballot(c[u] == 1));
-            t[2] += __popcll(__ballot(c[u] == 2)); t[3] += __popcll(__ballot(c[u] == 3));
-        }
-    };
-    if (cnt <= 256) {
-        load4(0); count4();
-        w0 = beg; w1 = w0 + t[0]; w2 = w1 + t[1]; w3 = w2 + t[2];
-        scatter4();
-    } else {
-        for (int o = 0; o < cnt; o += 256) { load4(o); count4(); }
-        w0 = beg; w1 = w0 + t[0]; w2 = w1 + t[1]; w3 = w2 + t[2];
-        for (int o = 0; o < cnt; o += 256) { load4(o); scatter4(); }
-    }
-    const int sc4[4] = {beg, beg + t[0], beg + t[0] + t[1], beg + t[0] + t[1] + t[2]};
-    if (lane == 0) oct_write_children(S, p, i, slot, mx, my, sb, t, sc4);
+    if (cnt <= 256) oct_partition_regs<4>(src, dst, cnt, mx, my, lane, t);
+    else if (cnt <= 1024) oct_partition_regs<16>(src, dst, cnt, mx, my, lane, t);
+    else if (!BIG && inplace) oct_partition_regs<OCT_INPLACE_MAX / 64>(src, dst, cnt, mx, my, lane, t);
+    else {
+        const unsigned long long lt = lanemask_lt(lane);
+        uint32_t k[4]; int c[4];
+        auto load4 = [&](int o) {
+#pragma unroll
+            for (int u = 0; u < 4; u++) k[u] = src[min(o + 64 * u + lane, cnt - 1)];
+#pragma unroll
+            for (int u = 0; u < 4; u++) c[u] = o + 64 * u + lane < cnt ? OCT_CODE(k[u]) : -1;
+        };
+        for (int o = 0; o < cnt; o += 256) {
+            load4(o);
+#pragma unroll
+            for (int u = 0; u < 4; u++) {
+                t[0] += __popcll(__ballot(c[u] == 0)); t[1] += __popcll(__ballot(c[u] == 1));
+                t[2] += __popcll(__ballot(c[u] == 2)); t[3] += __popcll(__ballot(c[u] == 3));
+            }
+        }
+        int w0 = 0, w1 = t[0], w2 = w1 + t[1], w3 = w2 + t[2];
+        for (int o = 0; o < cnt; o += 256) {
+            load4(o);
+#pragma unroll
+            for (int u = 0; u < 4; u++) {
+                const unsigned long long m0 = __ballot(c[u] == 0), m1 = __ballot(c[u] == 1), m2 = __ballot(c[u] == 2), m3 = __ballot(c[u] == 3);
+                const unsigned long long mm = c[u] == 0 ? m0 : (c[u] == 1 ? m1 : (c[u] == 2 ? m2 : m3));
+                int at = w3;
+                at = c[u] == 2 ? w2 : at; at = c[u] == 1 ? w1 : at; at = c[u] == 0 ? w0 : at;
+                if (c[u] >= 0) dst[at + __popcll(mm & lt)] = k[u];
+                w0 += __popcll(m0); w1 += __popcll(m1); w2 += __popcll(m2); w3 += __popcll(m3);
+            }
+        }
+    }
+    if (lane == 0) { oct_write_boxes<BIG>(S, p, i, slot, mx, my); oct_write_ranges<BIG>(S, slot, sb, beg, t); }
     OctExpandResult r; r.off = (t[0] > 0) + (t[1] > 0) + (t[2] > 0) + (t[3] > 0); r.nexp = (t[0] > 1) + (t[1] > 1) + (t[2] > 1) + (t[3] > 1);
     return r;
 }
 
-template <bool BIG> __device__ __forceinline__ void oct_lane_count(const OctLdsT<BIG>& S, const typename OctT<BIG>::Node& p, int mx, int my, unsigned long long& lo, unsigned long long& hi, int tc[4]) {
-    const typename OctT<BIG>::Perm* src = ((p.flags & OCT_BUF) ? S.perm1 : S.perm0) + (int)p.begin;
-    lo = 0; hi = 0; tc[0] = tc[1] = tc[2] = tc[3] = 0;
+#define OCT_SMALL_U 4
+template <bool BIG> __device__ __forceinline__ void oct_expand_small(const OctLdsT<BIG>& S, bool act, const typename OctT<BIG>::Node& p, int i, int slot, int lane,
+                                                                     int& d_live, int& d_exp) {
+    const int pcnt = (int)p.count, pbeg = (int)p.begin;
+    const int pmx = p.x0 + ((p.x1 - p.x0 + 1) >> 1), pmy = p.y0 + ((p.y1 - p.y0 + 1) >> 1);
+    if (act) oct_write_boxes<BIG>(S, p, i, slot, pmx, pmy);
+    const int lw = act ? 32 - __clz(max(pcnt - 1, 1)) : 0;
+    const uint32_t pk_cnt = (uint32_t)(pcnt & 0x7f) | ((uint32_t)(p.flags & OCT_BUF) << 8);
+    const uint32_t pk_mid = (uint32_t)(pmx & 0xffff) | ((uint32_t)pmy << 16);
+    const unsigned long long lt = lanemask_lt(lane);
+    for (int l = 6; l >= 1; l--) {
+        const unsigned long long mw = __ballot(act && lw == l);
+        if (!mw) continue;
+        const int w = 1 << l, nw = __popcll(mw), G = 64 >> l;
+        const int sub = lane >> l, kk = lane & (w - 1);
+        const unsigned long long gm = (l == 6 ? ~0ull : ((1ull << w) - 1ull)) << (lane & ~(w - 1));
+        for (int g0 = 0; g0 < nw; g0 += G * OCT_SMALL_U) {
+            uint32_t key[OCT_SMALL_U]; int nbeg[OCT_SMALL_U], nslot[OCT_SMALL_U]; uint32_t c2[OCT_SMALL_U], m2[OCT_SMALL_U];
+#pragma unroll
+            for (int u = 0; u < OCT_SMALL_U; u++) {
+                if (g0 + u * G >= nw) break;
+                const int g = g0 + u * G + sub;
+                const int sl = oct_nth_set(mw, min(g, nw - 1));
+                nbeg[u] = __shfl(pbeg, sl); c2[u] = (uint32_t)__shfl((int)pk_cnt, sl); m2[u] = (uint32_t)__shfl((int)pk_mid, sl); nslot[u] = __shfl(slot, sl);
+                const bool pv = g < nw && kk < (int)(c2[u] & 0x7f);
+                key[u] = S.buf((int)((c2[u] >> 8) & 1))[nbeg[u] + (pv ? kk : 0)];
+            }
+            WAVE_SYNC();
+#pragma unroll
+            for (int u = 0; u < OCT_SMALL_U; u++) {
+                if (g0 + u * G >= nw) break;
+                const int g = g0 + u * G + sub;
+                const int ncnt = (int)(c2[u] & 0x7f), nsb = (int)((c2[u] >> 8) & 1), mx = (int)(m2[u] & 0xffff), my = (int)(m2[u] >> 16);
+                const bool gv = g < nw, pv = gv && kk < ncnt;
+                const int c = pv ? OCT_CODE(key[u]) : -1;
+                const unsigned long long m0 = __ballot(c == 0) & gm, m1 = __ballot(c == 1) & gm, m2b = __ballot(c == 2) & gm, m3 = __ballot(c == 3) & gm;
+                const int tc[4] = {(int)__popcll(m0), (int)__popcll(m1), (int)__popcll(m2b), (int)__popcll(m3)};
+                const unsigned long long mm = c == 0 ? m0 : (c == 1 ? m1 : (c == 2 ? m2b : m3));
+                int at = tc[0] + tc[1] + tc[2];
+                at = c == 2 ? tc[0] + tc[1] : at; at = c == 1 ? tc[0] : at; at = c == 0 ? 0 : at;
+                uint32_t* dst = S.other(nsb) + nbeg[u];
+                if (pv) dst[at + __popcll(mm & lt)] = key[u];
+                if (gv && kk == 0) {
+                    oct_write_ranges<BIG>(S, nslot[u], nsb, nbeg[u], tc);
+                    d_live += (tc[0] > 0) + (tc[1] > 0) + (tc[2] > 0) + (tc[3] > 0) - 1;
+                    d_exp += (tc[0] > 1) + (tc[1] > 1) + (tc[2] > 1) + (tc[3] > 1);
+                }
+            }
+        }
+    }
+}
+
+template <bool BIG> __device__ __forceinline__ void oct_lane_count(const OctLdsT<BIG>& S, const typename OctT<BIG>::Node& p, int mx, int my, int tc[4]) {
+    const uint32_t* src = S.buf(p.flags & OCT_BUF) + (int)p.begin;
+    tc[0] = tc[1] = tc[2] = tc[3] = 0;
     const int cnt = (int)p.count;
     for (int k = 0; k < cnt; k += 4) {
-        typename OctT<BIG>::Perm id[4]; uint32_t key[4];
-#pragma unroll
-        for (int u = 0; u < 4; u++) id[u] = src[min(k + u, cnt - 1)];
-#pragma unroll
-        for (int u = 0; u < 4; u++) key[u] = S.keys[id[u]];
+        uint32_t key[4];
+#pragma unroll
+        for (int u = 0; u < 4; u++) key[u] = src[min(k + u, cnt - 1)];
 #pragma unroll
         for (int u = 0; u < 4; u++) {
-            const bool in = k + u < cnt;
-            const int cx = (int)(key[u] & 0xfff) < mx ? 0 : 1, cy = (int)((key[u] >> 12) & 0xfff) < my ? 0 : 1;
-            lo |= (unsigned long long)(in ? cx : 0) << ((k + u) & 63); hi |= (unsigned long long)(in ? cy : 0) << ((k + u) & 63);
-            const int c = in ? (cx | (cy << 1)) : -1;
+            const int c = k + u < cnt ? OCT_CODE(key[u]) : -1;
             tc[0] += c == 0; tc[1] += c == 1; tc[2] += c == 2; tc[3] += c == 3;
         }
     }
-}
-template <bool BIG> __device__ __forceinline__ void oct_lane_scatter(const OctLdsT<BIG>& S, const typename OctT<BIG>::Node& p, int i, int slot, int mx, int my, unsigned long long lo,
-                                                 unsigned long long hi, const int tc[4]) {
-    const int sb = p.flags & OCT_BUF;
-    const typename OctT<BIG>::Perm* src = (sb ? S.perm1 : S.perm0) + (int)p.begin;
-    typename OctT<BIG>::Perm* dst = sb ? S.perm0 : S.perm1;
-    const int sc4[4] = {(int)p.begin, (int)p.begin + tc[0], (int)p.begin + tc[0] + tc[1], (int)p.begin + tc[0] + tc[1] + tc[2]};
-    int w0 = sc4[0], w1 = sc4[1], w2 = sc4[2], w3 = sc4[3];
-    const int cnt = (int)p.count;
-    for (int k = 0; k < cnt; k += 4) {
-        typename OctT<BIG>::Perm id[4];
-#pragma unroll
-        for (int u = 0; u < 4; u++) id[u] = src[min(k + u, cnt - 1)];
-#pragma unroll
-        for (int u = 0; u < 4; u++) {
-            if (k + u < cnt) {
-                const int c = (int)((lo >> (k + u)) & 1) | ((int)((hi >> (k + u)) & 1) << 1);
-                const int pos = c == 0 ? w0 : (c == 1 ? w1 : (c == 2 ? w2 : w3));
-                dst[pos] = id[u];
-                w0 += c == 0; w1 += c == 1; w2 += c == 2; w3 += c == 3;
-            }
-        }
-    }
-    oct_write_children(S, p, i, slot, mx, my, sb, tc, sc4);
 }
 
 template <bool BIG> __device__ __forceinline__ int oct_compact(const OctLdsT<BIG>& S, int nn, int upto, int lane, int& first_new) {
@@ -1040,21 +1118,21 @@
                                                uint32_t* __restrict__ lvl_kp, int kp_pitch, int* __restrict__ lvl_cnt,
                                                int* __restrict__ lvl_ncand, int nlevels, int* __restrict__ status,
                                                int ncap, int nodecap, int sortcap, int n_above, int n_upto,
-                                               int level0, int use_tier_cap, int defer_nodes,
+                                               int level0, int use_tier_cap, int defer_nodes, int inplace,
                                                uint32_t* __restrict__ big_scratch, int* __restrict__ big_next, int big_slots, int* __restrict__ lvl_tot,
                                                uint8_t* __restrict__ node_scratch = nullptr, size_t node_bytes = 0) {
     extern __shared__ __attribute__((aligned(16))) uint32_t s_oct[];
-    typedef typename OctT<BIG>::Perm Perm; typedef typename OctT<BIG>::Node Node; typedef typename OctT<BIG>::SortKey SortKey;
+    typedef typename OctT<BIG>::Node Node; typedef typename OctT<BIG>::SortKey SortKey;
     OctLdsT<BIG> S;
     if (BIG) {
         S.sortb = reinterpret_cast<SortKey*>(s_oct);
         S.nd = reinterpret_cast<Node*>(S.sortb + sortcap);
-        S.keys = nullptr; S.perm0 = S.perm1 = nullptr;
+        S.k0 = nullptr; S.kd = 0;
     } else {
-        S.keys = s_oct;
-        S.perm0 = reinterpret_cast<Perm*>(s_oct + ncap);
-        S.perm1 = S.perm0 + ncap;
-        S.nd = reinterpret_cast<Node*>(S.perm1 + ncap);
+        const int kstride = (ncap + 3) & ~3;
+        S.k0 = s_oct;
+        S.kd = inplace ? 0 : kstride;
+        S.nd = reinterpret_cast<Node*>(s_oct + S.kd + kstride);
         S.sortb = reinterpret_cast<SortKey*>(S.nd + nodecap);
     }
     const int lane = threadIdx.x, level = blockIdx.y + level0, b = blockIdx.x;
@@ -1085,7 +1163,7 @@
             slot = __shfl(slot, 0);
             if (slot >= big_slots) { if (lane == 0) { lvl_cnt[b * nlevels + level] = 0; lvl_ncand[b * nlevels + level] = tot; status[b] = VIORB_ERR_CAPACITY; } return; }
             uint32_t* base = big_scratch + (size_t)slot * 3 * (size_t)ncap;
-            S.keys = base; S.perm0 = reinterpret_cast<Perm*>(base + ncap); S.perm1 = reinterpret_cast<Perm*>(base + 2 * (size_t)ncap);
+            S.k0 = base; S.kd = ncap;
             if (node_scratch) {
                 S.sortb = reinterpret_cast<SortKey*>(node_scratch + (size_t)slot * node_bytes);
                 S.nd = reinterpret_cast<Node*>(S.sortb + sortcap);
@@ -1109,7 +1187,7 @@
 #pragma unroll
                 for (int u = 0; u < 8; u++) {
                     const int pos = start + k0 + u;
-                    if (k0 + u < cnt && pos < ncap) S.keys[pos] = v[u];
+                    if (k0 + u < cnt && pos < ncap) S.k0[pos] = v[u];
                 }
             }
             n += __shfl(incl, 63);
@@ -1126,28 +1204,59 @@
     int nn = 0, live = 0;
     {
         int begin = 0;
-        for (int r = 0; r < L.n_ini; r++) {
-            int cnt = 0;
-            for (int o = 0; o < n; o += 64) {
-                const int idx = o + lane;
-                bool mine = false;
-                if (idx < n) mine = ((int)((float)(S.keys[idx] & 0xfff) / L.hx)) == r;
-                const unsigned long long m = __ballot(mine);
-                if (mine) S.perm0[begin + cnt + __popcll(m & lanemask_lt(lane))] = (Perm)idx;
-                cnt += __popcll(m);
-            }
+        auto root_node = [&](int r, int cnt) {
             if (cnt > 0) {
                 if (lane == 0) {
                     Node o;
                     o.x0 = (int16_t)(int)(L.hx * (float)r); o.x1 = (int16_t)(int)(L.hx * (float)(r + 1));
                     o.y0 = 0; o.y1 = (int16_t)L.oct_h;
                     o.begin = (decltype(o.begin))begin; o.count = (decltype(o.count))cnt;
-                    o.flags = (uint16_t)(cnt == 1 ? OCT_NOMORE : 0); o.pad = 0;
+                    o.flags = (uint16_t)(OCT_BUF | (cnt == 1 ? OCT_NOMORE : 0)); o.pad = 0;
                     S.nd[nn] = o;
                 }
                 nn++;
             }
             begin += cnt;
+        };
+        if (!BIG && inplace) {
+            uint32_t k[OCT_INPLACE_MAX / 64], rt[OCT_INPLACE_MAX / 256];
+#pragma unroll
+            for (int u = 0; u < OCT_INPLACE_MAX / 64; u++) if (64 * u < n) k[u] = S.k0[64 * u + lane];
+#pragma unroll
+            for (int u = 0; u < OCT_INPLACE_MAX / 256; u++) rt[u] = 0;
+#pragma unroll
+            for (int u = 0; u < OCT_INPLACE_MAX / 64; u++) {
+                if (64 * u >= n) continue;
+                const int root = 64 * u + lane < n ? (int)((float)(k[u] & 0xfff) / L.hx) : 255;
+                rt[u >> 2] |= (uint32_t)(root & 0xff) << (8 * (u & 3));
+            }
+            WAVE_SYNC();
+            for (int r = 0; r < L.n_ini; r++) {
+                int cnt = 0;
+#pragma unroll
+                for (int u = 0; u < OCT_INPLACE_MAX / 64; u++) {
+                    if (64 * u >= n) continue;
+                    const bool mine = (int)((rt[u >> 2] >> (8 * (u & 3))) & 0xff) == r;
+                    const unsigned long long m = __ballot(mine);
+                    if (mine) S.k0[S.kd + begin + cnt + __popcll(m & lanemask_lt(lane))] = k[u];
+                    cnt += __popcll(m);
+                    __builtin_amdgcn_sched_barrier(0);
+                }
+                root_node(r, cnt);
+            }
+        } else {
+            for (int r = 0; r < L.n_ini; r++) {
+                int cnt = 0;
+                for (int o = 0; o < n; o += 64) {
+                    const int idx = o + lane;
+                    bool mine = false; uint32_t key = 0;
+                    if (idx < n) { key = S.k0[idx]; mine = ((int)((float)(key & 0xfff) / L.hx)) == r; }
+                    const unsigned long long m = __ballot(mine);
+                    if (mine) S.k0[S.kd + begin + cnt + __popcll(m & lanemask_lt(lane))] = key;
+                    cnt += __popcll(m);
+                }
+                root_node(r, cnt);
+            }
         }
         WAVE_SYNC();
         for (int i = lane; i < (nn >> 1); i += 64) {
@@ -1176,23 +1285,16 @@
             const unsigned long long m = __ballot(ex);
             const int e = e_base + __popcll(m & lanemask_lt(lane));
             const bool small = ex && p.count <= OCT_LANE_LIMIT;
-            int off = 0, nexp = 0;
-            if (small) {
-                const int mx = p.x0 + ((p.x1 - p.x0 + 1) >> 1), my = p.y0 + ((p.y1 - p.y0 + 1) >> 1);
-                unsigned long long lo, hi; int tc[4];
-                oct_lane_count(S, p, mx, my, lo, hi, tc);
-                oct_lane_scatter(S, p, i, nn0 + 4 * e, mx, my, lo, hi, tc);
-                off = (tc[0] > 0) + (tc[1] > 0) + (tc[2] > 0) + (tc[3] > 0); nexp = (tc[0] > 1) + (tc[1] > 1) + (tc[2] > 1) + (tc[3] > 1);
-            }
+            int d_live = 0, d_exp = 0;
+            oct_expand_small<BIG>(S, small, p, i, nn0 + 4 * e, lane, d_live, d_exp);
             unsigned long long mb = __ballot(ex && !small);
             int big_off = 0, big_nexp = 0;
             while (mb) {
                 const int l = __ffsll((long long)mb) - 1;
                 mb &= mb - 1;
-                const OctExpandResult r = oct_expand_wave(S, nn0 - 1 - (base + l), nn0 + 4 * __shfl(e, l), lane);
+                const OctExpandResult r = oct_expand_wave<BIG>(S, nn0 - 1 - (base + l), nn0 + 4 * __shfl(e, l), lane, inplace != 0);
                 big_off += r.off - 1; big_nexp += r.nexp;
             }
-            int d_live = small ? off - 1 : 0, d_exp = nexp;
 #pragma unroll
             for (int d = 32; d > 0; d >>= 1) { d_live += __shfl_xor(d_live, d); d_exp += __shfl_xor(d_exp, d); }
             live += d_live + big_off; n_to_expand += d_exp + big_nexp;
@@ -1234,15 +1336,15 @@
                     if (__any(valid && p.count > OCT_LANE_LIMIT)) {
                         for (int l = 0; l < 64 && base + l < m; l++) {
                             if (nn1 + 4 * (processed + 1) > nodecap) { overflow = true; finish = true; break; }
-                            const OctExpandResult r = oct_expand_wave(S, (int)(S.sortb[mp - 1 - (base + l)] & 0xffff), nn1 + 4 * processed, lane);
+                            const OctExpandResult r = oct_expand_wave<BIG>(S, (int)(S.sortb[mp - 1 - (base + l)] & 0xffff), nn1 + 4 * processed, lane, inplace != 0);
                             processed++; live += r.off - 1;
                             if (live >= N) { reached = true; break; }
                         }
                         continue;
                     }
                     const int mx = p.x0 + ((p.x1 - p.x0 + 1) >> 1), my = p.y0 + ((p.y1 - p.y0 + 1) >> 1);
-                    unsigned long long lo = 0, hi = 0; int tc[4] = {0, 0, 0, 0};
-                    if (valid) oct_lane_count(S, p, mx, my, lo, hi, tc);
+                    int tc[4] = {0, 0, 0, 0};
+                    if (valid) oct_lane_count<BIG>(S, p, mx, my, tc);
                     const int inc = valid ? (tc[0] > 0) + (tc[1] > 0) + (tc[2] > 0) + (tc[3] > 0) - 1 : 0;
                     const int incl = wave_inclusive_scan(inc);
                     const unsigned long long mh = __ballot(valid && live + incl >= N);
@@ -1250,7 +1352,7 @@
                     int cut = mh ? __ffsll((long long)mh) - 1 : nvalid - 1;
                     const int fit = (nodecap - nn1) / 4 - processed;
                     if (fit < cut + 1) { overflow = true; finish = true; cut = fit - 1; }
-                    if (valid && lane <= cut) oct_lane_scatter(S, p, i, nn1 + 4 * (processed + lane), mx, my, lo, hi, tc);
+                    { int dl = 0, de = 0; oct_expand_small<BIG>(S, valid && lane <= cut, p, i, nn1 + 4 * (processed + lane), lane, dl, de); }
                     if (cut >= 0) { live += __shfl(incl, cut); processed += cut + 1; }
                     if (mh) reached = true;
                 }
@@ -1269,10 +1371,10 @@
         const int i = base + lane;
         if (i < nn) {
             const Node o = S.nd[i];
-            const Perm* pm = (o.flags & OCT_BUF) ? S.perm1 : S.perm0;
-            uint32_t best = S.keys[pm[o.begin]];
+            const uint32_t* pm = S.buf(o.flags & OCT_BUF) + o.begin;
+            uint32_t best = pm[0];
             for (int k = 1; k < (int)o.count; k++) {
-                const uint32_t key = S.keys[pm[o.begin + k]];
+                const uint32_t key = pm[k];
                 if ((key >> 24) > (best >> 24)) best = key;
             }
             out[nn - 1 - i] = (best & 0xff000000u) | ((((best >> 12) & 0xfff) + MINB) << 12) | ((best & 0xfff) + MINB);
@@ -1655,6 +1757,8 @@
     int fast3_tile_bytes = 0, fast3_score_bytes = 0;
     int oct_ncap = 0, oct_nodecap = 0, oct_sortcap = 0;
     std::vector<std::pair<int, int>> oct_tiers;
+    struct OctPlan { int l0, l1, ncap, nodecap; size_t lds; bool inplace; };
+    std::vector<OctPlan> oct_plans;
     int oct_first_cap = 0, oct_node_x10 = 50;
     int oct_big_cap = 0, oct_big_slots = 0; uint32_t* d_oct_big = nullptr; int* d_oct_big_next = nullptr; int* d_lvl_tot = nullptr;
     unsigned char* d_stereo_work = nullptr; size_t stereo_work_bytes = 0;
@@ -1897,14 +2001,14 @@
     h->oct_nodecap = 5 * maxq + 64;
     int sc = 1; while (sc < maxq + 8) sc <<= 1;
     h->oct_sortcap = sc;
-    size_t oct_lds = (size_t)h->oct_ncap * 8 + (size_t)h->oct_nodecap * sizeof(OctNode) + (size_t)sc * 4;
+    size_t oct_lds = oct_lds_bytes(h->oct_ncap, h->oct_nodecap, sc, false);
     if (h->oct_nodecap > 65535) { set_error("per-level quota %d too large for the quadtree's 16-bit node indices", maxq); return VIORB_ERR_UNSUPPORTED; }
     h->oct_huge = oct_lds > 160 * 1024;
     if (!h->oct_huge && oct_lds > 64 * 1024 &&
         raise_dynamic_lds(reinterpret_cast<const void*>(k_octree<false>), oct_lds) != hipSuccess) {
         (void)hipGetLastError();
         h->oct_ncap = 4096;
-        oct_lds = (size_t)h->oct_ncap * 8 + (size_t)h->oct_nodecap * sizeof(OctNode) + (size_t)sc * 4;
+        oct_lds = oct_lds_bytes(h->oct_ncap, h->oct_nodecap, sc, false);
         if (oct_lds > 64 * 1024) { set_error("quadtree LDS (%zu B) exceeds the dynamic-LDS limit", oct_lds); return VIORB_ERR_UNSUPPORTED; }
     }
 
@@ -1915,7 +2019,7 @@
     }
     {
         const char* e = getenv("VIORB_OCT_TIERS");
-        std::string spec = e ? e : "3:2048";
+        std::string spec = e ? e : "0:3072,3:1792";
         h->oct_tiers.clear();
         for (int l = 0; l < nl; l++) h->lv[l].oct_tier_cap = 0;
         int prev_l = 0, prev_c = std::min(h->oct_ncap, (int)OCT_NCAP_SMALL);
@@ -1933,6 +2037,20 @@
         for (size_t ti = 0; ti < h->oct_tiers.size(); ti++) {
             const int l1 = ti + 1 < h->oct_tiers.size() ? h->oct_tiers[ti + 1].first : nl;
             for (int l = h->oct_tiers[ti].first; l < l1; l++) h->lv[l].oct_tier_cap = h->oct_tiers[ti].second;
+        }
+        h->oct_plans.clear();
+        const int ntier = h->oct_huge ? 0 : (int)h->oct_tiers.size();
+        for (int ti = -1; ti < ntier && !h->oct_huge; ti++) {
+            viorb_extractor::OctPlan P;
+            P.l0 = ti < 0 ? 0 : h->oct_tiers[ti].first;
+            P.l1 = ti + 1 < ntier ? h->oct_tiers[ti + 1].first : nl;
+            P.ncap = ti < 0 ? h->oct_first_cap : h->oct_tiers[ti].second;
+            int mq = 1; for (int l = P.l0; l < P.l1; l++) mq = std::max(mq, h->quota[l]);
+            P.nodecap = h->oct_node_x10 < 50 ? std::min(5 * mq + 64, (h->oct_node_x10 * mq) / 10 + 64) : (ti < 0 ? h->oct_nodecap : 5 * mq + 64);
+            P.inplace = P.ncap <= OCT_INPLACE_MAX;
+            for (int l = P.l0; l < P.l1; l++) P.inplace = P.inplace && h->lv[l].n_ini <= 255;
+            P.lds = oct_lds_bytes(P.ncap, P.nodecap, h->oct_sortcap, P.inplace);
+            h->oct_plans.push_back(P);
         }
     }
     const size_t B = (size_t)h->max_batch;
@@ -2109,34 +2227,21 @@
     }
     if (bst != st) VIORB_HIP_TRY(hipEventRecord(h->ev_join, bst));
     {
-        const size_t fixed = (size_t)h->oct_nodecap * sizeof(OctNode) + (size_t)h->oct_sortcap * 4;
         const int small = h->oct_first_cap > 0 ? h->oct_first_cap : std::min(h->oct_ncap, (int)OCT_NCAP_SMALL);
         const int ntier = h->oct_huge ? 0 : (int)h->oct_tiers.size();
         const bool defer = h->oct_node_x10 < 50;
-        auto first_nodes = [&](int mq) { return std::min(5 * mq + 64, (h->oct_node_x10 * mq) / 10 + 64); };
         if (!h->oct_huge) {
             ProfScope ps("k_octree", st);
-            const int l_end0 = ntier ? h->oct_tiers[0].first : nl;
-            int mq0 = 1; for (int l = 0; l < l_end0; l++) mq0 = std::max(mq0, h->quota[l]);
-            const int ndc0 = defer ? first_nodes(mq0) : h->oct_nodecap;
-            hipLaunchKernelGGL(k_octree<false>, dim3(batch, l_end0), dim3(64), (size_t)small * 8 + (size_t)ndc0 * sizeof(OctNode) + (size_t)h->oct_sortcap * 4, st,
-                               h->d_lv, h->d_slots, h->slot_cap, h->d_cell_cnt,
-                               ncells, h->d_lvl_kp, h->kp_pitch, h->d_lvl_cnt, h->d_lvl_ncand, nl, h->d_status, small, ndc0,
-                               h->oct_sortcap, -1, small, 0, 0, defer ? 1 : 0, nullptr, nullptr, 0, h->d_lvl_tot);
-            for (int ti = 0; ti < ntier; ti++) {
-                const int l0 = h->oct_tiers[ti].first, l1 = ti + 1 < ntier ? h->oct_tiers[ti + 1].first : nl, nc = h->oct_tiers[ti].second;
-                int mq = 1; for (int l = l0; l < l1; l++) mq = std::max(mq, h->quota[l]);
-                const int ndc = defer ? first_nodes(mq) : 5 * mq + 64;
-                hipLaunchKernelGGL(k_octree<false>, dim3(batch, l1 - l0), dim3(64), (size_t)nc * 8 + (size_t)ndc * sizeof(OctNode) + (size_t)h->oct_sortcap * 4,
-                                   st, h->d_lv, h->d_slots, h->slot_cap, h->d_cell_cnt, ncells, h->d_lvl_kp, h->kp_pitch, h->d_lvl_cnt, h->d_lvl_ncand, nl, h->d_status,
-                                   nc, ndc, h->oct_sortcap, -1, nc, l0, 0, defer ? 1 : 0, nullptr, nullptr, 0, h->d_lvl_tot);
-            }
+            for (const viorb_extractor::OctPlan& P : h->oct_plans)
+                hipLaunchKernelGGL(k_octree<false>, dim3(batch, P.l1 - P.l0), dim3(64), P.lds, st, h->d_lv, h->d_slots, h->slot_cap, h->d_cell_cnt,
+                                   ncells, h->d_lvl_kp, h->kp_pitch, h->d_lvl_cnt, h->d_lvl_ncand, nl, h->d_status, P.ncap, P.nodecap,
+                                   h->oct_sortcap, -1, P.ncap, P.l0, 0, defer ? 1 : 0, P.inplace ? 1 : 0, nullptr, nullptr, 0, h->d_lvl_tot);
         }
         if (!h->oct_huge && (small < h->oct_ncap || ntier || defer)) {
             ProfScope ps("k_octree_large", st);
-            hipLaunchKernelGGL(k_octree<false>, dim3(batch, nl), dim3(64), (size_t)h->oct_ncap * 8 + fixed, st, h->d_lv, h->d_slots, h->slot_cap,
+            hipLaunchKernelGGL(k_octree<false>, dim3(batch, nl), dim3(64), oct_lds_bytes(h->oct_ncap, h->oct_nodecap, h->oct_sortcap, false), st, h->d_lv, h->d_slots, h->slot_cap,
                                h->d_cell_cnt, ncells, h->d_lvl_kp, h->kp_pitch, h->d_lvl_cnt, h->d_lvl_ncand, nl, h->d_status, h->oct_ncap,
-                               h->oct_nodecap, h->oct_sortcap, small, h->oct_ncap, 0, ntier ? 1 : 0, 0, nullptr, nullptr, 0, h->d_lvl_tot);
+                               h->oct_nodecap, h->oct_sortcap, small, h->oct_ncap, 0, ntier ? 1 : 0, 0, 0, nullptr, nullptr, 0, h->d_lvl_tot);
         }
         {
             const size_t lds_big = h->oct_huge ? 0 : (size_t)h->oct_sortcap * 8 + (size_t)h->oct_nodecap * sizeof(OctNodeBig);
@@ -2144,7 +2249,7 @@
             ProfScope ps("k_octree_big", st);
             hipLaunchKernelGGL(k_octree<true>, dim3(batch, nl), dim3(64), lds_big, st, h->d_lv, h->d_slots, h->slot_cap, h->d_cell_cnt, ncells, h->d_lvl_kp,
                                h->kp_pitch, h->d_lvl_cnt, h->d_lvl_ncand, nl, h->d_status, h->oct_big_cap, h->oct_nodecap, h->oct_sortcap,
-                               h->oct_huge ? -1 : std::max(h->oct_ncap, (int)small), 0x7fffffff, 0, 0, 0, h->d_oct_big, h->d_oct_big_next, h->oct_big_slots, h->d_lvl_tot,
+                               h->oct_huge ? -1 : std::max(h->oct_ncap, (int)small), 0x7fffffff, 0, 0, 0, 0, h->d_oct_big, h->d_oct_big_next, h->oct_big_slots, h->d_lvl_tot,
                                h->oct_huge ? h->d_oct_nodes : (uint8_t*)nullptr, h->oct_node_bytes);
         }
     }
@@ -2445,6 +2550,17 @@
     return rc;
 }
 
+int viorb_extractor_quadtree_plans(const viorb_extractor* h, viorb_quadtree_plan* plans, int cap, int* n) {
+    if (!h || !n || (cap > 0 && !plans)) { set_error("quadtree_plans: null argument"); return VIORB_ERR_INVALID_ARG; }
+    *n = (int)h->oct_plans.size();
+    for (int i = 0; i < *n && i < cap; i++) {
+        const viorb_extractor::OctPlan& P = h->oct_plans[i];
+        plans[i].level_begin = P.l0; plans[i].level_end = P.l1; plans[i].candidates = P.ncap; plans[i].nodes = P.nodecap;
+        plans[i].lds_bytes = (int32_t)P.lds; plans[i].in_place = P.inplace ? 1 : 0;
+    }
+    return VIORB_OK;
+}
+
 int viorb_extractor_debug_level_points(viorb_extractor* h, int b, int level, int which, int32_t* xyr, int cap, int* n) {
     VIORB_REQUIRE(h && h->d_planes && n, "no results yet");
     VIORB_REQUIRE(level >= 0 && level < h->p.nlevels && b >= 0 && b < h->last_batch, "level/image out of range");
diff --git a/viorb_amd/extractor.py b/viorb_amd/extractor.py
--- a/viorb_amd/extractor.py
+++ b/viorb_amd/extractor.py
@@ -104,6 +104,13 @@
         check(self.L.viorb_extractor_debug_level_points(self.h, b, l, int(kept), ptr(buf), len(buf), C.byref(n)))
         return buf[:min(n.value, len(buf))].copy()
 
+    def quadtree_plans(self):
+        buf = np.zeros((16, 6), np.int32)
+        n = C.c_int()
+        check(self.L.viorb_extractor_quadtree_plans(self.h, ptr(buf), len(buf), C.byref(n)))
+        names = ("level_begin", "level_end", "candidates", "nodes", "lds_bytes", "in_place")
+        return [dict(zip(names, (int(v) for v in row))) for row in buf[:min(n.value, len(buf))]]
+
 
 def ComputeStereoMatches(ex_left, ex_right, bf, fx):
     u, d = np.zeros(ex_left.cap, np.float32), np.zeros(ex_left.cap, np.float32)
```

New measurement: 191,200. No clear change (-0.2%).
